# RobinBruneau/RNb-NeuS2

Hardware: AMD Instinct MI355X
Metric: training rays/s + ms/step, normals-only SDF 64x800^2 (higher is better)
Workload: dtype f16 storage / f32 accumulate

## Files before the change

include/rnb_neus2.h:

```cpp
#ifndef RNB_NEUS2_H
#define RNB_NEUS2_H

#include <stdint.h>

#ifdef __cplusplus
extern "C" {
#endif

#define RNB_ABI_VERSION 5

typedef enum rnb_status {
	RNB_OK = 0,
	RNB_ERR_INVALID = -1,
	RNB_ERR_DEVICE = -2,
	RNB_ERR_NOMEM = -3,
	RNB_ERR_NO_SAMPLES = -4
} rnb_status;

#define RNB_N_POS_DIMS 3
#define RNB_COORD_FLOATS 7
#define RNB_OUT_WIDTH 16
#define RNB_SDF_IN 32
#define RNB_SDF_HID 64
#define RNB_SDF_OUT 16
// ... 84 lines not shown
	RNB_BUF_DENSITY_BITFIELD = 8,
	RNB_BUF_DENSITY_MEAN = 9,
	RNB_BUF_RAY_INDICES = 10,
	RNB_BUF_RAYS = 11,
	RNB_BUF_NUMSTEPS = 12,
	RNB_BUF_COORDS = 13,
	RNB_BUF_MLP_OUT = 14,
	RNB_BUF_DLOSS_DOUT = 15,
	RNB_BUF_COORDS_COMPACTED = 16,
	RNB_BUF_LOSS = 17,
	RNB_BUF_EK_LOSS = 18,
	RNB_BUF_MASK_LOSS = 19,
	RNB_BUF_COUNTERS = 20,
	RNB_BUF_DENSITY_GRID_TMP = 21,
	RNB_BUF_GRID_SAMPLE_POS = 22,
	RNB_BUF_GRID_SAMPLE_IDX = 23,
	RNB_BUF_STEP_VECTOR = 24,
	RNB_BUF_GRID_SAMPLE_POS_EVAL = 25,
	RNB_BUF_GRID_SAMPLE_IDX_EVAL = 26,
	RNB_BUF_GRADS_FP16 = 27,
	RNB_BUF_COUNT
} rnb_buffer_id;
#define RNB_BUF_READONLY 0x100

typedef enum rnb_memcpy_kind { RNB_H2D = 0, RNB_D2H = 1, RNB_D2D = 2 } rnb_memcpy_kind;

const char* rnb_last_error(void);
uint32_t rnb_abi_version(void);
int rnb_default_config(rnb_config* cfg);
int rnb_create(const rnb_config* cfg, rnb_ctx** out);
int rnb_destroy(rnb_ctx* ctx);
int rnb_update_config(rnb_ctx* ctx, const rnb_config* cfg);

uint64_t rnb_n_params(const rnb_ctx* ctx);
int rnb_param_layout(const rnb_ctx* ctx, uint64_t offsets[5]);
int rnb_grid_tables(const rnb_ctx* ctx, uint32_t* offsets, uint32_t* resolution, float* scale);
int rnb_init_params(rnb_ctx* ctx, const float* sdf_mlp_weights_host);
int rnb_set_params(rnb_ctx* ctx, const float* params_host);
int rnb_buffer(rnb_ctx* ctx, int buffer_id, void** ptr, uint64_t* n_bytes);
int rnb_params_changed(rnb_ctx* ctx);
int rnb_bitfield_changed(rnb_ctx* ctx);
int rnb_device_malloc(rnb_ctx* ctx, uint64_t n_bytes, void** ptr);
int rnb_device_free(rnb_ctx* ctx, void* ptr);
int rnb_memcpy(rnb_ctx* ctx, void* dst, const void* src, uint64_t n_bytes, int kind);

int rnb_set_dataset(rnb_ctx* ctx, uint32_t n_views, const rnb_view* views,
                    const uint16_t* const* normals_host, const uint16_t* const* albedos_host);

int rnb_set_training_step(rnb_ctx* ctx, uint32_t step);
uint32_t rnb_valid_level(const rnb_ctx* ctx);
int rnb_update_density_grid(rnb_ctx* ctx, void* stream);
typedef int (*rnb_grid_exchange_fn)(void* user, void* grid_tmp, uint64_t n_elements, void* stream);
int rnb_set_grid_exchange(rnb_ctx* ctx, rnb_grid_exchange_fn fn, void* user);
int rnb_update_density_grid_begin(rnb_ctx* ctx, void* stream);
int rnb_update_density_grid_end(rnb_ctx* ctx, void* stream);
int rnb_update_density_bitfield(rnb_ctx* ctx, void* stream);
int rnb_density(rnb_ctx* ctx, void* stream, const float* xyz_dev, uint32_t n, uint16_t* out_dev, int use_inference_params);
int rnb_sdf(rnb_ctx* ctx, void* stream, const float* xyz_dev, uint32_t n, uint16_t* out_dev, int use_inference_params);
int rnb_forward_infer(rnb_ctx* ctx, void* stream, const float* coords_dev, uint32_t n, uint16_t* out_dev, int use_inference_params);
int rnb_sdf_lattice(rnb_ctx* ctx, void* stream, const uint32_t res[3], float lattice_min, float lattice_max, float* out, int inference);
int rnb_marching_cubes(rnb_ctx* ctx, void* stream, const float* density, const uint32_t res[3], const float aabb_min[3], const float aabb_max[3], float thresh,
                       float** verts, uint32_t** indices, uint32_t* n_verts, uint32_t* n_indices);
int rnb_generate_training_samples(rnb_ctx* ctx, void* stream, uint32_t n_rays, uint32_t n_rays_total, uint32_t max_samples);
int rnb_compute_loss(rnb_ctx* ctx, void* stream, uint32_t n_rays, uint32_t n_rays_total);
int rnb_forward_backward(rnb_ctx* ctx, void* stream);
int rnb_optimizer_step(rnb_ctx* ctx, void* stream);

int rnb_train_step(rnb_ctx* ctx, void* stream, rnb_step_stats* stats);
int rnb_train_step_begin(rnb_ctx* ctx, void* stream);
int rnb_train_step_end(rnb_ctx* ctx, void* stream, rnb_step_stats* stats);
int rnb_train_step_apply(rnb_ctx* ctx, void* stream);
int rnb_train_step_local(rnb_ctx* ctx, void* stream, uint64_t counters[4], double loss_sums[3]);
int rnb_train_step_finish(rnb_ctx* ctx, const uint64_t counters[4], const double loss_sums[3], rnb_step_stats* stats);
int rnb_profile_enable(rnb_ctx* ctx, int on);
int rnb_profile_count(const rnb_ctx* ctx);
int rnb_profile_get(const rnb_ctx* ctx, int idx, const char** name, double* total_ms, uint64_t* launches, double* units);
uint32_t rnb_training_step(const rnb_ctx* ctx);
uint32_t rnb_rays_per_batch(const rnb_ctx* ctx);
int rnb_set_optimizer_step(rnb_ctx* ctx, uint32_t step);
int rnb_set_controller(rnb_ctx* ctx, uint32_t training_step, uint32_t rays_per_batch,
                       uint32_t measured_batch_size_before_compaction, uint32_t n_rays_total);

typedef enum rnb_primitive { RNB_PRIM_PCG32 = 0, RNB_PRIM_MORTON = 1, RNB_PRIM_SRGB = 2, RNB_PRIM_RAY_BOX = 3, RNB_PRIM_MARCH = 4,
                             RNB_PRIM_ACTIVATION = 5, RNB_PRIM_WARP = 6, RNB_PRIM_LOSS = 7, RNB_PRIM_PIXEL = 8, RNB_PRIM_GRID = 9, RNB_PRIM_READ_RGBA = 10, RNB_PRIM_CAMERA_RAY = 11, RNB_PRIM_RAY_TARGETS = 12, RNB_PRIM_LOSS_SAMPLE = 13, RNB_PRIM_RAY_LOSS = 14, RNB_PRIM_ENCODE = 15, RNB_PRIM_MARCH_RAY = 16, RNB_PRIM_SDF_DENSITY = 17, RNB_PRIM_PREP_DUE = 18, RNB_PRIM_DW_SLICED = 19 } rnb_primitive;
int rnb_eval_primitives(rnb_ctx* ctx, int kind, const uint32_t* in_host, uint32_t n_items, uint32_t* out_host);

int rnb_gradient_parts(rnb_ctx* ctx, uint64_t ranges[3][2], uint32_t* n_parts);
int rnb_gradient_part_wait(rnb_ctx* ctx, uint32_t part, void* stream);
int rnb_train_step_apply_early(rnb_ctx* ctx, void* stream);

#define RNB_MAX_SHARD_PARTS 3
typedef struct rnb_shard_part { uint64_t lo, hi, own_lo, own_hi; } rnb_shard_part;
int rnb_shard_layout(rnb_ctx* ctx, rnb_shard_part parts[RNB_MAX_SHARD_PARTS], uint32_t* n_parts, uint64_t* capacity);
int rnb_train_step_apply_shard(rnb_ctx* ctx, uint32_t part, void* stream);
int rnb_train_step_apply_done(rnb_ctx* ctx, void* stream);

#ifdef __cplusplus
}
#endif
#endif
```

rnb-neus2_amd/_abi.py:

```python
import ctypes as C

ABI_VERSION = 5

OK, ERR_INVALID, ERR_DEVICE, ERR_NOMEM, ERR_NO_SAMPLES = 0, -1, -2, -3, -4

N_SDF_MLP_PARAMS = 3072
N_RGB_MLP_PARAMS = 8192
N_VARIANCE_PARAMS = 4
GRIDSIZE = 128
CASCADES = 8


class Config(C.Structure):
    _fields_ = [
        ("abi_version", C.c_uint32),
        ("n_levels", C.c_uint32),
        ("log2_hashmap_size", C.c_uint32),
        ("base_resolution", C.c_uint32),
        ("per_level_scale", C.c_float),
        ("valid_level_scale", C.c_float),
        ("base_valid_level_scale", C.c_float),
        ("base_training_step", C.c_uint32),
        ("sdf_bias", C.c_float),
        ("target_batch_size", C.c_uint32),
        ("initial_rays_per_batch", C.c_uint32),
        ("max_rays_per_batch", C.c_uint32),
        ("aabb_scale", C.c_uint32),
        ("seed", C.c_uint32),
        ("mask_loss_weight", C.c_float),
        ("ek_loss_weight", C.c_float),
        ("apply_L2", C.c_uint32),
        ("apply_rgbplus", C.c_uint32),
        ("apply_no_albedo", C.c_uint32),
        ("apply_light_opti", C.c_uint32),
        ("apply_supernormal", C.c_uint32),
        ("apply_relu", C.c_uint32),
        ("apply_bce", C.c_uint32),
        ("snap_to_pixel_centers", C.c_uint32),
        ("learning_rate", C.c_float),
        ("beta1", C.c_float),
        ("beta2", C.c_float),
        ("epsilon", C.c_float),
        ("l2_reg", C.c_float),
        ("ema_decay", C.c_float),
        ("lr_decay_start", C.c_uint32),
        ("lr_decay_interval", C.c_uint32),
        ("lr_decay_base", C.c_float),
        ("density_grid_decay", C.c_float),
        ("world_size", C.c_uint32),
        ("rank", C.c_uint32),
        ("only_sdf_training", C.c_uint32),
        ("overlap", C.c_uint32),
        ("accumulate", C.c_uint32),
        ("deterministic", C.c_uint32),
        ("reserved", C.c_uint32 * 4),
    ]


class View(C.Structure):
    _fields_ = [
        ("width", C.c_uint32),
        ("height", C.c_uint32),
        ("focal_length", C.c_float * 2),
        ("principal_point", C.c_float * 2),
        ("xform", C.c_float * 12),
    ]


class StepStats(C.Structure):
    _fields_ = [
        ("training_step", C.c_uint32),
        ("rays_per_batch", C.c_uint32),
        ("next_rays_per_batch", C.c_uint32),
        ("measured_batch_size", C.c_uint32),
        ("measured_batch_size_before_compaction", C.c_uint32),
        ("n_rays_kept", C.c_uint32),
        ("density_grid_updated", C.c_uint32),
        ("loss", C.c_float),
        ("ek_loss", C.c_float),
        ("mask_loss", C.c_float),
        ("prep_ms", C.c_float),
        ("step_ms", C.c_float),
    ]

    def as_dict(self):
        return {name: getattr(self, name) for name, _ in self._fields_}


BUF = dict(
    PARAMS_FP32=0, PARAMS_FP16=1, PARAMS_EMA=2, GRADS_FP32=3, ADAM_M=4, ADAM_V=5, ADAM_STEPS=6,
    DENSITY_GRID=7, DENSITY_BITFIELD=8, DENSITY_MEAN=9, RAY_INDICES=10, RAYS=11, NUMSTEPS=12,
    COORDS=13, MLP_OUT=14, DLOSS_DOUT=15, COORDS_COMPACTED=16, LOSS=17, EK_LOSS=18, MASK_LOSS=19,
    COUNTERS=20, DENSITY_GRID_TMP=21, GRID_SAMPLE_POS=22, GRID_SAMPLE_IDX=23, STEP_VECTOR=24, GRID_SAMPLE_POS_EVAL=25, GRID_SAMPLE_IDX_EVAL=26, GRADS_FP16=27,
)
BUF_DTYPE = dict(
    PARAMS_FP32="f4", PARAMS_FP16="f2", PARAMS_EMA="f2", GRADS_FP32="f4", ADAM_M="f4", ADAM_V="f4", ADAM_STEPS="u4",
    DENSITY_GRID="f4", DENSITY_BITFIELD="u1", DENSITY_MEAN="f4", RAY_INDICES="u4", RAYS="f4", NUMSTEPS="u4",
    COORDS="f4", MLP_OUT="f2", DLOSS_DOUT="f2", COORDS_COMPACTED="f4", LOSS="f4", EK_LOSS="f4", MASK_LOSS="f4",
    COUNTERS="u4", DENSITY_GRID_TMP="f4", GRID_SAMPLE_POS="f4", GRID_SAMPLE_IDX="u4", STEP_VECTOR="f8", GRID_SAMPLE_POS_EVAL="f4", GRID_SAMPLE_IDX_EVAL="u4", GRADS_FP16="f2",
)
ACCUM_FP32, ACCUM_HALF = 0, 1
BUF_READONLY = 0x100
GRID_EXCHANGE_FN = C.CFUNCTYPE(C.c_int, C.c_void_p, C.c_void_p, C.c_uint64, C.c_void_p)
PRIM = dict(PCG32=0, MORTON=1, SRGB=2, RAY_BOX=3, MARCH=4, ACTIVATION=5, WARP=6, LOSS=7, PIXEL=8, GRID=9, READ_RGBA=10, CAMERA_RAY=11, RAY_TARGETS=12, LOSS_SAMPLE=13, RAY_LOSS=14, ENCODE=15, MARCH_RAY=16, SDF_DENSITY=17, PREP_DUE=18, DW_SLICED=19)
PRIM_IN_WORDS, PRIM_OUT_WORDS = (6, 3, 1, 8, 9, 1, 9, 9, 9, 7, 32, 20, 35, 37, 16, 263, 10, 2, 1, 33028), (4, 4, 2, 3, 7, 3, 11, 5, 3, 3, 5, 9, 7, 28, 9, 16, 23, 1, 2, 16)
H2D, D2H, D2D = 0, 1, 2

_ctx = C.c_void_p
_stream = C.c_void_p
_u32, _u64, _i = C.c_uint32, C.c_uint64, C.c_int

PROTOTYPES = {
    "last_error": (C.c_char_p, []),
    "abi_version": (_u32, []),
    "default_config": (_i, [C.POINTER(Config)]),
    "create": (_i, [C.POINTER(Config), C.POINTER(_ctx)]),
    "destroy": (_i, [_ctx]),
    "update_config": (_i, [_ctx, C.POINTER(Config)]),
    "n_params": (_u64, [_ctx]),
    "param_layout": (_i, [_ctx, C.POINTER(_u64)]),
    "grid_tables": (_i, [_ctx, C.POINTER(_u32), C.POINTER(_u32), C.POINTER(C.c_float)]),
    "init_params": (_i, [_ctx, C.POINTER(C.c_float)]),
    "set_params": (_i, [_ctx, C.POINTER(C.c_float)]),
    "buffer": (_i, [_ctx, _i, C.POINTER(C.c_void_p), C.POINTER(_u64)]),
    "params_changed": (_i, [_ctx]),
    "bitfield_changed": (_i, [_ctx]),
    "memcpy": (_i, [_ctx, C.c_void_p, C.c_void_p, _u64, _i]),
    "device_malloc": (_i, [_ctx, _u64, C.POINTER(C.c_void_p)]),
    "device_free": (_i, [_ctx, C.c_void_p]),
    "set_dataset": (_i, [_ctx, _u32, C.POINTER(View), C.POINTER(C.c_void_p), C.POINTER(C.c_void_p)]),
    "set_training_step": (_i, [_ctx, _u32]),
    "valid_level": (_u32, [_ctx]),
    "update_density_grid": (_i, [_ctx, _stream]),
    "update_density_bitfield": (_i, [_ctx, _stream]),
    "update_density_grid_begin": (_i, [_ctx, _stream]),
    "update_density_grid_end": (_i, [_ctx, _stream]),
    "set_grid_exchange": (_i, [_ctx, C.c_void_p, C.c_void_p]),
    "density": (_i, [_ctx, _stream, C.c_void_p, _u32, C.c_void_p, _i]),
    "sdf": (_i, [_ctx, _stream, C.c_void_p, _u32, C.c_void_p, _i]),
    "forward_infer": (_i, [_ctx, _stream, C.c_void_p, _u32, C.c_void_p, _i]),
    "sdf_lattice": (_i, [_ctx, _stream, C.POINTER(_u32), C.c_float, C.c_float, C.c_void_p, _i]),
    "marching_cubes": (_i, [_ctx, _stream, C.c_void_p, C.POINTER(_u32), C.POINTER(C.c_float), C.POINTER(C.c_float), C.c_float,
                            C.POINTER(C.c_void_p), C.POINTER(C.c_void_p), C.POINTER(_u32), C.POINTER(_u32)]),
    "generate_training_samples": (_i, [_ctx, _stream, _u32, _u32, _u32]),
    "compute_loss": (_i, [_ctx, _stream, _u32, _u32]),
    "forward_backward": (_i, [_ctx, _stream]),
    "optimizer_step": (_i, [_ctx, _stream]),
    "train_step": (_i, [_ctx, _stream, C.POINTER(StepStats)]),
    "train_step_begin": (_i, [_ctx, _stream]),
    "train_step_end": (_i, [_ctx, _stream, C.POINTER(StepStats)]),
    "profile_enable": (_i, [_ctx, _i]),
    "profile_count": (_i, [_ctx]),
    "profile_get": (_i, [_ctx, _i, C.POINTER(C.c_char_p), C.POINTER(C.c_double), C.POINTER(_u64), C.POINTER(C.c_double)]),
    "train_step_apply": (_i, [_ctx, _stream]),
    "train_step_local": (_i, [_ctx, _stream, C.POINTER(_u64), C.POINTER(C.c_double)]),
    "train_step_finish": (_i, [_ctx, C.POINTER(_u64), C.POINTER(C.c_double), C.POINTER(StepStats)]),
    "training_step": (_u32, [_ctx]),
    "rays_per_batch": (_u32, [_ctx]),
    "set_controller": (_i, [_ctx, _u32, _u32, _u32, _u32]),
    "set_optimizer_step": (_i, [_ctx, _u32]),
    "eval_primitives": (_i, [_ctx, _i, C.c_void_p, _u32, C.c_void_p]),
    "gradient_parts": (_i, [_ctx, C.POINTER(_u64 * 2 * 3), C.POINTER(_u32)]),
    "gradient_part_wait": (_i, [_ctx, _u32, _stream]),
    "train_step_apply_early": (_i, [_ctx, _stream]),
    "shard_layout": (_i, [_ctx, C.POINTER(_u64 * 4 * 3), C.POINTER(_u32), C.POINTER(_u64)]),
    "train_step_apply_shard": (_i, [_ctx, _u32, _stream]),
    "train_step_apply_done": (_i, [_ctx, _stream]),
}


RENDER_ABI_VERSION = 1
RENDER_CHANNELS = 9


class RenderOptions(C.Structure):
    _fields_ = [
        ("abi_version", C.c_uint32),
        ("min_transmittance", C.c_float),
        ("near_distance", C.c_float),
        ("use_inference_params", C.c_uint32),
        ("use_occupancy", C.c_uint32),
        ("max_rays_in_flight", C.c_uint32),
        ("reserved", C.c_uint32 * 4),
    ]


class RenderStats(C.Structure):
    _fields_ = [
# ... 772 lines not shown
```

rnb-neus2_amd/api.py:

```python
import ctypes as C
import math
import os

import numpy as np

from . import _abi
from ._abi import Config, View, StepStats, BUF, BUF_DTYPE

__all__ = ["Context", "DeviceMesh", "Config", "View", "StepStats", "load_library", "default_config", "library_path",
           "load_sdf_init_weights", "RnbError", "BUF", "scaled_view", "RENDER_CHANNELS"]

RENDER_CHANNELS = _abi.RENDER_CHANNELS

_PKG_DIR = os.path.dirname(os.path.abspath(__file__))
_REPO_ROOT = os.path.dirname(_PKG_DIR)
_LIB_NAME = "librnb_neus2_hip.so"


class RnbError(RuntimeError):
    def __init__(self, code, message):
        super().__init__("rnb error %d: %s" % (code, message))
        self.code = code


# ... 224 lines not shown
        dt = np.dtype(BUF_DTYPE[name])
        total = nb // dt.itemsize
        if count is None:
            count = total - offset
        if offset + count > total:
            raise ValueError("%s: range [%d, %d) exceeds %d elements" % (name, offset, offset + count, total))
        out = np.empty(count, dtype=dt)
        if count:
            self._check(self.f.memcpy(self._h, out.ctypes.data_as(C.c_void_p), C.c_void_p(ptr + offset * dt.itemsize),
                                      count * dt.itemsize, _abi.D2H))
        return out

    def put(self, name, array, offset=0):
        ptr, nb = self.buffer(name)
        dt = np.dtype(BUF_DTYPE[name])
        a = np.ascontiguousarray(array, dtype=dt).ravel()
        if (offset + a.size) * dt.itemsize > nb:
            raise ValueError("%s: write of %d elements at %d exceeds buffer" % (name, a.size, offset))
        if a.size:
            self._check(self.f.memcpy(self._h, C.c_void_p(ptr + offset * dt.itemsize), a.ctypes.data_as(C.c_void_p),
                                      a.size * dt.itemsize, _abi.H2D))
            if name == "DENSITY_BITFIELD":
                self.bitfield_changed()
            elif name == "PARAMS_FP16":
                self.params_changed()

    def init_params(self, sdf_weights=None):
        w = load_sdf_init_weights() if sdf_weights is None else np.ascontiguousarray(sdf_weights, dtype=np.float32)
        self._check(self.f.init_params(self._h, w.ctypes.data_as(C.POINTER(C.c_float))))

    def set_params(self, params_fp32):
        p = np.ascontiguousarray(params_fp32, dtype=np.float32).ravel()
        if p.size != self.n_params:
            raise ValueError("expected %d params, got %d" % (self.n_params, p.size))
        self._check(self.f.set_params(self._h, p.ctypes.data_as(C.POINTER(C.c_float))))

    def set_dataset(self, views, normals, albedos):
        n = len(views)
        if n == 0 or len(normals) != n or len(albedos) != n:
            raise ValueError("views / normals / albedos must be non-empty and of equal length")
        arr = (View * n)()
        nptr = (C.c_void_p * n)()
        aptr = (C.c_void_p * n)()
        keep = []
        for i, v in enumerate(views):
            arr[i].width = int(v["width"])
            arr[i].height = int(v["height"])
            arr[i].focal_length[:] = [float(x) for x in v["focal_length"]]
            arr[i].principal_point[:] = [float(x) for x in v["principal_point"]]
            arr[i].xform[:] = [float(x) for x in np.asarray(v["xform"], dtype=np.float32).reshape(12)]
            nm = np.ascontiguousarray(normals[i], dtype=np.uint16)
            al = np.ascontiguousarray(albedos[i], dtype=np.uint16)
            if nm.size != arr[i].width * arr[i].height * 4 or al.size != nm.size:
                raise ValueError("view %d: image size does not match width*height*4" % i)
            keep += [nm, al]
            nptr[i] = nm.ctypes.data
            aptr[i] = al.ctypes.data
        self._check(self.f.set_dataset(self._h, n, arr, nptr, aptr))

    def set_training_step(self, step):
        self._check(self.f.set_training_step(self._h, int(step)))

    @property
    def valid_level(self):
        return int(self.f.valid_level(self._h))

    @property
    def training_step(self):
        return int(self.f.training_step(self._h))

    @property
    def rays_per_batch(self):
        return int(self.f.rays_per_batch(self._h))

    def set_controller(self, training_step, rays_per_batch, measured_before_compaction=0, n_rays_total=0):
        self._check(self.f.set_controller(self._h, int(training_step), int(rays_per_batch), int(measured_before_compaction), int(n_rays_total)))

    def eval_primitives(self, kind, items):
        k = _abi.PRIM[kind]
        a = np.ascontiguousarray(items, dtype=np.uint32).reshape(-1, _abi.PRIM_IN_WORDS[k])
        out = np.empty((a.shape[0], _abi.PRIM_OUT_WORDS[k]), dtype=np.uint32)
        self._check(self.f.eval_primitives(self._h, k, a.ctypes.data_as(C.c_void_p), a.shape[0], out.ctypes.data_as(C.c_void_p)))
        return out

    def training_state(self, last_stats=None):
        return dict(params=self.get("PARAMS_FP32").copy(), adam_m=self.get("ADAM_M").copy(), adam_v=self.get("ADAM_V").copy(), adam_steps=self.get("ADAM_STEPS").copy(),
                    ema=self.get("PARAMS_EMA").copy(), grid=self.get("DENSITY_GRID").copy(), step=self.training_step, rays=self.rays_per_batch,
                    before=int(last_stats.measured_batch_size_before_compaction) if last_stats is not None else 0)

    def load_training_state(self, state):
        self.set_params(state["params"])
        self.put("ADAM_M", state["adam_m"])
        self.put("ADAM_V", state["adam_v"])
        self.put("ADAM_STEPS", state["adam_steps"])
        self.put("PARAMS_EMA", state["ema"])
        self.set_optimizer_step(state["step"])
        self.put("DENSITY_GRID", state["grid"])
        self.update_density_bitfield()
        self.set_controller(state["step"], state["rays"], state["before"], 0)

    def set_optimizer_step(self, step):
        self._check(self.f.set_optimizer_step(self._h, int(step)))

    def gradient_parts(self):
        arr = (C.c_uint64 * 2 * 3)()
        n = C.c_uint32()
        self._check(self.f.gradient_parts(self._h, C.byref(arr), C.byref(n)))
        return [(int(arr[k][0]), int(arr[k][1])) for k in range(n.value)]

    def train_step_apply_early(self, stream_handle):
        self._check(self.f.train_step_apply_early(self._h, C.c_void_p(stream_handle)))

    def gradient_part_wait(self, part, stream_handle):
        self._check(self.f.gradient_part_wait(self._h, int(part), C.c_void_p(stream_handle)))

    def shard_layout(self):
        arr = (C.c_uint64 * 4 * 3)()
        n = C.c_uint32()
        cap = C.c_uint64()
        self._check(self.f.shard_layout(self._h, C.byref(arr), C.byref(n), C.byref(cap)))
        return [tuple(int(arr[k][j]) for j in range(4)) for k in range(n.value)], int(cap.value)

    def train_step_apply_shard(self, part, stream_handle=None):
        self._check(self.f.train_step_apply_shard(self._h, int(part), C.c_void_p(stream_handle)))

    def train_step_apply_done(self, stream_handle=None):
        self._check(self.f.train_step_apply_done(self._h, C.c_void_p(stream_handle)))

    def profile_enable(self, on=True):
        self._check(self.f.profile_enable(self._h, int(bool(on))))

    def profile(self):
        out = []
        for i in range(self.f.profile_count(self._h)):
            name, ms, n, units = C.c_char_p(), C.c_double(), C.c_uint64(), C.c_double()
            self._check(self.f.profile_get(self._h, i, C.byref(name), C.byref(ms), C.byref(n), C.byref(units)))
            out.append(dict(kernel=name.value.decode(), total_ms=ms.value, launches=n.value, units=units.value))
        return out

    def update_density_grid(self, stream=None):
        self._check(self.f.update_density_grid(self._h, _stream_handle(stream)))

    def update_density_grid_begin(self, stream=None):
        self._check(self.f.update_density_grid_begin(self._h, _stream_handle(stream)))

    def update_density_grid_end(self, stream=None):
        self._check(self.f.update_density_grid_end(self._h, _stream_handle(stream)))

    def set_grid_exchange(self, fn):
        if fn is None:
            self._grid_cb = None
            self._check(self.f.set_grid_exchange(self._h, None, None))
            return

        def trampoline(_user, ptr, n, stream):
            try:
                fn(ptr, int(n), stream)
                return 0
            except Exception:
                import traceback
                traceback.print_exc()
                return -1
        self._grid_cb = _abi.GRID_EXCHANGE_FN(trampoline)
        self._check(self.f.set_grid_exchange(self._h, C.cast(self._grid_cb, C.c_void_p), None))

    def update_density_bitfield(self, stream=None):
# ... 1012 lines not shown
```

rnb-neus2_amd/csrc/common.cuh:

```cuda
#pragma once
#include <hip/hip_runtime.h>
#include <stdint.h>
#include "../../include/rnb_neus2.h"

namespace rnb {

typedef _Float16 half_t;
typedef _Float16 h2 __attribute__((ext_vector_type(2)));
typedef _Float16 h4 __attribute__((ext_vector_type(4)));
typedef _Float16 h8 __attribute__((ext_vector_type(8)));
typedef float f4 __attribute__((ext_vector_type(4)));

constexpr uint32_t GRIDSIZE = RNB_GRIDSIZE;
constexpr uint32_t GRID_CELLS = GRIDSIZE * GRIDSIZE * GRIDSIZE;
constexpr uint32_t N_CASCADES = RNB_CASCADES;
constexpr float LOSS_SCALE = 128.f;
constexpr uint32_t N_MAX_RANDOM_SAMPLES_PER_RAY = 8;
constexpr float SQRT3 = 1.73205080757f;
constexpr float STEPSIZE = SQRT3 / 1024;
constexpr float MIN_CONE_STEPSIZE = STEPSIZE;
constexpr float MAX_CONE_STEPSIZE = STEPSIZE * (1 << (N_CASCADES - 1)) * 1024 / GRIDSIZE;
constexpr float MIN_OPTICAL_THICKNESS = 0.1f;

struct GridMeta {
// ... 213 lines not shown
__device__ __forceinline__ void encode_level_lm(const LevelMeta* __restrict__ lm, const uint32_t* __restrict__ grid, const uint32_t level,
                                                const float x, const float y, const float z,
                                                half_t& f0, half_t& f1, float dy0[3], float dy1[3]) {
	const uint4 raw = *reinterpret_cast<const uint4*>(lm + level);
	const uint32_t off = __builtin_amdgcn_readfirstlane(raw.x), size = __builtin_amdgcn_readfirstlane(raw.y), res = __builtin_amdgcn_readfirstlane(raw.z);
	const float scale = __uint_as_float(__builtin_amdgcn_readfirstlane(raw.w));
	encode_level_core<GRAD>(grid + off, size, res, scale, x, y, z, f0, f1, dy0, dy1);
}

__device__ __forceinline__ void level_issue(const LevelMeta* __restrict__ lm, const uint32_t* __restrict__ grid, const uint32_t level, const float x, const float y, const float z, uint32_t (&v)[8]) {
	const uint4 raw = reinterpret_cast<const uint4*>(lm + level)[0], raw2 = reinterpret_cast<const uint4*>(lm + level)[1];
	const uint32_t off = __builtin_amdgcn_readfirstlane(raw.x), hashmap_size = __builtin_amdgcn_readfirstlane(raw.y);
	const float scale = __uint_as_float(__builtin_amdgcn_readfirstlane(raw.w));
	const uint32_t my = __builtin_amdgcn_readfirstlane(raw2.x), mz = __builtin_amdgcn_readfirstlane(raw2.y);
	const bool dense = __builtin_amdgcn_readfirstlane(raw2.z) != 0u, pow2 = __builtin_amdgcn_readfirstlane(raw2.w) != 0u;
	const uint32_t* __restrict__ g = grid + off;
	float pos[3];
	uint32_t pg[3];
	pos_fract(x, scale, &pos[0], &pg[0]);
	pos_fract(y, scale, &pos[1], &pg[1]);
	pos_fract(z, scale, &pos[2], &pg[2]);
	const uint32_t ty0 = pg[1] * my, ty1 = ty0 + my, tz0 = pg[2] * mz, tz1 = tz0 + mz;
#pragma unroll
	for (uint32_t yz = 0; yz < 4; ++yz) {
		const uint32_t ty = (yz & 1u) ? ty1 : ty0, tz = (yz >> 1) ? tz1 : tz0;
		const uint32_t d0 = pg[0] + ty + tz, h = ty ^ tz;
		uint32_t e0 = dense ? d0 : (pg[0] ^ h), e1 = dense ? d0 + 1u : ((pg[0] + 1u) ^ h);
		const uint32_t w0 = e0 >= hashmap_size ? e0 - hashmap_size : e0, w1 = e1 >= hashmap_size ? e1 - hashmap_size : e1;
		e0 = pow2 ? (e0 & (hashmap_size - 1u)) : w0;
		e1 = pow2 ? (e1 & (hashmap_size - 1u)) : w1;
		v[yz * 2 + 0] = g[e0];
		v[yz * 2 + 1] = g[e1];
	}
}
template <bool GRAD>
__device__ __forceinline__ void level_consume(const LevelMeta* __restrict__ lm, const uint32_t level, const float x, const float y, const float z, const uint32_t (&v)[8],
                                              half_t& f0, half_t& f1, float dy0[3], float dy1[3]) {
	const float scale = __uint_as_float(__builtin_amdgcn_readfirstlane(reinterpret_cast<const uint32_t*>(lm + level)[3]));
	float pos[3];
	uint32_t pg[3];
	pos_fract(x, scale, &pos[0], &pg[0]);
	pos_fract(y, scale, &pos[1], &pg[1]);
	pos_fract(z, scale, &pos[2], &pg[2]);
	half_t r0 = (half_t)0.f, r1 = (half_t)0.f;
#pragma unroll
	for (uint32_t idx = 0; idx < 8; ++idx) {
		float weight = 1;
#pragma unroll
		for (uint32_t d = 0; d < 3; ++d) {
			if ((idx & (1u << d)) == 0) weight *= 1 - pos[d];
			else weight *= pos[d];
		}
		const h2 val = unpack_h2(v[idx]);
		r0 = r0 + f2h(weight * h2f(val[0]));
		r1 = r1 + f2h(weight * h2f(val[1]));
	}
	f0 = r0;
	f1 = r1;
	if (GRAD) {
#pragma unroll
		for (uint32_t gd = 0; gd < 3; ++gd) {
			float a0 = 0.f, a1 = 0.f;
#pragma unroll
			for (uint32_t idx = 0; idx < 4; ++idx) {
				float weight = scale;
				uint32_t corner = 0;
#pragma unroll
				for (uint32_t ngd = 0; ngd < 2; ++ngd) {
					const uint32_t d = ngd >= gd ? (ngd + 1) : ngd;
					if ((idx & (1u << ngd)) == 0) weight *= 1 - pos[d];
					else { weight *= pos[d]; corner |= (1u << d); }
				}
				const h2 vl = unpack_h2(v[corner]);
				const h2 vr = unpack_h2(v[corner | (1u << gd)]);
				a0 += weight * (h2f(vr[0]) - h2f(vl[0])) * 1.0f;
				a1 += weight * (h2f(vr[1]) - h2f(vl[1])) * 1.0f;
			}
			dy0[gd] = a0;
			dy1[gd] = a1;
		}
	}
}

struct Vec3 { float x, y, z; };
__device__ __forceinline__ Vec3 v3(float x, float y, float z) { return {x, y, z}; }
__device__ __forceinline__ Vec3 operator+(Vec3 a, Vec3 b) { return {a.x + b.x, a.y + b.y, a.z + b.z}; }
__device__ __forceinline__ Vec3 operator-(Vec3 a, Vec3 b) { return {a.x - b.x, a.y - b.y, a.z - b.z}; }
__device__ __forceinline__ Vec3 operator*(float s, Vec3 a) { return {s * a.x, s * a.y, s * a.z}; }
__device__ __forceinline__ float esum3(float x0, float x1, float x2) { return x0 + (x1 + x2); }
__device__ __forceinline__ float esum4(float x0, float x1, float x2, float x3) { return (x0 + x1) + (x2 + x3); }
__device__ __forceinline__ float dot(Vec3 a, Vec3 b) { return esum3(a.x * b.x, a.y * b.y, a.z * b.z); }
__device__ __forceinline__ Vec3 normalized(Vec3 a) { float n = sqrtf(dot(a, a)); return {a.x / n, a.y / n, a.z / n}; }

__device__ __forceinline__ int mip_from_pos(const Vec3& pos, uint32_t max_cascade = N_CASCADES - 1) {
	int exponent;
	float maxval = fmaxf(fmaxf(fabsf(pos.x - 0.5f), fabsf(pos.y - 0.5f)), fabsf(pos.z - 0.5f));
	frexpf(maxval, &exponent);
	return min((int)max_cascade, max(0, exponent + 1));
}
__device__ __forceinline__ int mip_from_dt(float dt, const Vec3& pos, uint32_t max_cascade = N_CASCADES - 1) {
	int mip = mip_from_pos(pos, max_cascade);
	dt *= 2 * GRIDSIZE;
	if (dt < 1.f) return mip;
	int exponent;
	frexpf(dt, &exponent);
	return min((int)max_cascade, max(exponent, mip));
}
__device__ __forceinline__ uint32_t cascaded_grid_idx_at(Vec3 pos, uint32_t mip) {
	float mip_scale = scalbnf(1.0f, -(int)mip);
	pos = pos - v3(0.5f, 0.5f, 0.5f);
	pos = mip_scale * pos;
	pos = pos + v3(0.5f, 0.5f, 0.5f);
	int ix = (int)(pos.x * GRIDSIZE), iy = (int)(pos.y * GRIDSIZE), iz = (int)(pos.z * GRIDSIZE);
	return morton3D((uint32_t)min(max(ix, 0), (int)GRIDSIZE - 1), (uint32_t)min(max(iy, 0), (int)GRIDSIZE - 1), (uint32_t)min(max(iz, 0), (int)GRIDSIZE - 1));
}
__device__ __forceinline__ bool density_grid_occupied_at(const Vec3& pos, const uint8_t* __restrict__ bitfield, uint32_t mip) {
	uint32_t idx = cascaded_grid_idx_at(pos, mip);
	return bitfield[idx / 8 + (GRID_CELLS * mip) / 8] & (1 << (idx % 8));
}
__device__ __forceinline__ float calc_dt(float t, float cone_angle) {
	return fminf(fmaxf(t * cone_angle, MIN_CONE_STEPSIZE), MAX_CONE_STEPSIZE);
}
__device__ __forceinline__ float warp_dt(float dt) {
	float max_stepsize = MIN_CONE_STEPSIZE * (1 << (N_CASCADES - 1));
	return (dt - MIN_CONE_STEPSIZE) / (max_stepsize - MIN_CONE_STEPSIZE);
}
__device__ __forceinline__ float unwarp_dt(float dt) {
	float max_stepsize = MIN_CONE_STEPSIZE * (1 << (N_CASCADES - 1));
	return dt * (max_stepsize - MIN_CONE_STEPSIZE) + MIN_CONE_STEPSIZE;
}
__device__ __forceinline__ float sign1(float x) { return copysignf(1.0f, x); }
__device__ __forceinline__ float distance_to_next_voxel(const Vec3& pos, const Vec3& dir, const Vec3& idir, uint32_t res) {
	Vec3 p = (float)res * pos;
	float tx = (floorf(p.x + 0.5f + 0.5f * sign1(dir.x)) - p.x) * idir.x;
	float ty = (floorf(p.y + 0.5f + 0.5f * sign1(dir.y)) - p.y) * idir.y;
	float tz = (floorf(p.z + 0.5f + 0.5f * sign1(dir.z)) - p.z) * idir.z;
	float t = fminf(fminf(tx, ty), tz);
	return fmaxf(t / res, 0.0f);
}
__device__ __forceinline__ float advance_to_next_voxel(float t, float cone_angle, const Vec3& pos, const Vec3& dir, const Vec3& idir, uint32_t res) {
	float t_target = t + distance_to_next_voxel(pos, dir, idir, res);
	do { t += calc_dt(t, cone_angle); } while (t < t_target);
	return t;
}

__device__ __forceinline__ float logistic(float x) { return 1.0f / (1.0f + expf(-x)); }
__device__ __forceinline__ float relu(float v) { return v > 0.0f ? v : 0.0f; }
__device__ __forceinline__ Vec3 warp_direction(const Vec3& d) { return {(d.x + 1.0f) * 0.5f, (d.y + 1.0f) * 0.5f, (d.z + 1.0f) * 0.5f}; }
__device__ __forceinline__ Vec3 unwarp_direction(const Vec3& d) { return {d.x * 2.0f - 1.0f, d.y * 2.0f - 1.0f, d.z * 2.0f - 1.0f}; }
__device__ __forceinline__ float loss_and_gradient(const bool l2, const float (&target)[4], const float (&prediction)[4], float (&grad)[4]) {
	float diff[4];
#pragma unroll
	for (int k = 0; k < 4; ++k) diff[k] = prediction[k] - target[k];
	if (l2) {
#pragma unroll
		for (int k = 0; k < 4; ++k) grad[k] = 2 * diff[k];
		return diff[0] * diff[0] + diff[1] * diff[1] + diff[2] * diff[2] + diff[3] * diff[3];
	}
#pragma unroll
	for (int k = 0; k < 4; ++k) grad[k] = copysignf(1.0f, diff[k]);
	return fabsf(diff[0]) + fabsf(diff[1]) + fabsf(diff[2]) + fabsf(diff[3]);
}

}
```

rnb-neus2_amd/csrc/kernels_net.cuh:

```cuda
#pragma once
#include "mlp.cuh"

namespace rnb {

constexpr int WG = 256;
constexpr int WAVES_PER_WG = 4;


__device__ __forceinline__ void write_sdf_in_row(half_t* __restrict__ tile, const int lane, const float x, const float y, const float z, const half_t (&feat)[28]) {
	half_t row[32];
	row[0] = f2h(x) - (half_t)0.5f;
	row[1] = f2h(y) - (half_t)0.5f;
	row[2] = f2h(z) - (half_t)0.5f;
#pragma unroll
	for (int k = 0; k < 28; ++k) row[3 + k] = feat[k];
	row[31] = (half_t)0.f;
#pragma unroll
	for (int q = 0; q < 4; ++q) {
		h8 v;
#pragma unroll
		for (int j = 0; j < 8; ++j) v[j] = row[q * 8 + j];
		*reinterpret_cast<h8*>(tile + lane * S32 + q * 8) = v;
	}
}

template <bool GRAD>
__device__ __forceinline__ void encode_all_lm(const LevelMeta* __restrict__ lm, const uint32_t n_levels, const uint32_t valid_level, const uint32_t* __restrict__ grid,
                                              const float x, const float y, const float z, half_t (&feat)[28], float (&dydx)[GRAD ? 28 : 1][3]) {
#pragma unroll
	for (uint32_t level = 0; level < 14; ++level) {
		half_t f0 = (half_t)0.f, f1 = (half_t)0.f;
		float d0[3] = {0.f, 0.f, 0.f}, d1[3] = {0.f, 0.f, 0.f};
		if (level < n_levels && level <= valid_level) {
			encode_level_lm<GRAD>(lm, grid, level, x, y, z, f0, f1, d0, d1);
		}
		feat[level * 2 + 0] = f0;
		feat[level * 2 + 1] = f1;
		if (GRAD) {
#pragma unroll
			for (int d = 0; d < 3; ++d) { dydx[GRAD ? level * 2 + 0 : 0][d] = d0[d]; dydx[GRAD ? level * 2 + 1 : 0][d] = d1[d]; }
		}
	}
}

template <bool GRAD, int DEPTH>
__device__ __forceinline__ void encode_all_pipelined(const LevelMeta* __restrict__ lm, const uint32_t n_levels, const uint32_t valid_level, const uint32_t* __restrict__ grid,
                                                     const float x, const float y, const float z, half_t (&feat)[28], float (&dydx)[GRAD ? 28 : 1][3]) {
	const uint32_t n_live = min(n_levels, valid_level + 1u);
	uint32_t v[DEPTH][8];
	const uint32_t last = n_live ? n_live - 1u : 0u;
#pragma unroll
	for (uint32_t l = 0; l < (uint32_t)DEPTH; ++l) level_issue(lm, grid, min(l, last), x, y, z, v[l]);
#pragma unroll
	for (uint32_t level = 0; level < 14; ++level) {
		half_t f0, f1;
		float d0[3], d1[3];
		const bool live = level < n_live;
		level_consume<GRAD>(lm, min(level, last), x, y, z, v[level % DEPTH], f0, f1, d0, d1);
		if (level + DEPTH < 14) level_issue(lm, grid, min(level + (uint32_t)DEPTH, last), x, y, z, v[level % DEPTH]);
		feat[level * 2 + 0] = live ? f0 : (half_t)0.f;
		feat[level * 2 + 1] = live ? f1 : (half_t)0.f;
		if (GRAD) {
#pragma unroll
			for (int d = 0; d < 3; ++d) { dydx[GRAD ? level * 2 + 0 : 0][d] = live ? d0[d] : 0.f; dydx[GRAD ? level * 2 + 1 : 0][d] = live ? d1[d] : 0.f; }
		}
	}
}

__device__ __forceinline__ half_t sdf_to_density(half_t sdf, half_t variance) {
	const half_t s = f2h(expf(h2f(variance * (half_t)10.0f)));
	const half_t sig = f2h(1.0f / (1.0f + expf(-h2f(sdf * s))));
	return (s * sig) * ((half_t)1.0f - sig);
}

struct PointArgs {
	const float* xyz;
	uint32_t n;
	half_t* out;
	const uint32_t* splat_idx;
	float* grid_tmp;
	int want_density;
	float sdf_bias;
	const uint32_t* range;
};

struct FwdArgs {
	const float* coords;
	const uint32_t* n_ptr;
	uint32_t n_max;
	half_t* out;
	float sdf_bias;
	const uint32_t* idx;
	const half_t* wimg;
	half_t* cin_out;
};

__device__ __forceinline__ void copy_weight_image(half_t* __restrict__ dst, const half_t* __restrict__ src, const int n_halfs, const int tid, const int nthreads) {
	for (int i = tid * 8; i < n_halfs; i += nthreads * 8) *reinterpret_cast<h8*>(dst + i) = *reinterpret_cast<const h8*>(src + i);
}

constexpr int PQ2_WAVE_HALFS = TILE * S32 + TILE;
constexpr size_t LDS_POINT2 = (size_t)(W_S0T + WAVES_PER_WG * PQ2_WAVE_HALFS) * sizeof(half_t);
__device__ __forceinline__ void poison_lds(char* smem_raw, const size_t bytes, const int tid, const int nthreads) {
#ifdef RNB_POISON_LDS
	uint32_t* w = reinterpret_cast<uint32_t*>(smem_raw);
	for (uint32_t q = (uint32_t)tid; q < (uint32_t)(bytes / 4); q += (uint32_t)nthreads) w[q] = 0x7e007e00u;
	__syncthreads();
#else
	(void)smem_raw; (void)bytes; (void)tid; (void)nthreads;
#endif
}

template <bool EMU, int DEPTH>
__device__ __forceinline__ void point_query_chained_body(const GridMeta& G, const NetW& net, const PointArgs& a, const half_t* __restrict__ wimg, char* smem_raw, LevelMeta* lm) {
	poison_lds(smem_raw, LDS_POINT2, threadIdx.x, WG);
	half_t* wts = reinterpret_cast<half_t*>(smem_raw);
	fill_level_meta(lm, G, threadIdx.x);
	const uint32_t n_levels = G.n_levels, valid_level = G.valid_level;
	if (wimg) copy_weight_image(wts, wimg, W_S0T, threadIdx.x, WG);
	else {
		for (int i = threadIdx.x; i < 64 * 32; i += WG) { int o = i >> 5, k = i & 31; wts[W_S0 + o * S32 + k] = net.sdf_w0[i]; }
		for (int i = threadIdx.x; i < 16 * 64; i += WG) { int o = i >> 6, q = i & 63; wts[W_S1 + o * S64 + q] = net.sdf_w1[o * 64 + chain_logical(q)]; }
	}
	__syncthreads();
	const int lane = threadIdx.x & 63, wave = threadIdx.x >> 6;
	half_t* X = wts + W_S0T + wave * PQ2_WAVE_HALFS;
	half_t* Z = X + TILE * S32;
	const half_t variance = net.variance[0];
	const half_t bias = f2h(a.sdf_bias);
	uint32_t s_first = 0, s_end = a.n;
	if (a.range) { s_first = a.range[0]; s_end = min(a.range[1], a.n); }
	const uint32_t n_tiles = (s_end - s_first + TILE - 1) / TILE;
	const int r16 = lane & 15, hq = lane >> 4;
	const bool by_xcd = (gridDim.x & 7u) == 0u;
	const uint32_t t8 = by_xcd ? (n_tiles + 7u) / 8u : n_tiles, t_base = by_xcd ? (blockIdx.x & 7u) * t8 : 0u, t_stop = min(n_tiles, t_base + t8);
	const uint32_t t_stride = (by_xcd ? gridDim.x / 8u : gridDim.x) * WAVES_PER_WG;
	for (uint32_t tile = t_base + (by_xcd ? blockIdx.x / 8u : blockIdx.x) * WAVES_PER_WG + wave; tile < t_stop; tile += t_stride) {
		const uint32_t s = s_first + tile * TILE + lane;
		const bool valid = s < s_end;
		float x = 0.5f, y = 0.5f, z = 0.5f;
		if (valid) { x = a.xyz[(size_t)s * 3 + 0]; y = a.xyz[(size_t)s * 3 + 1]; z = a.xyz[(size_t)s * 3 + 2]; }
		uint32_t cell = 0;
		if (valid && a.splat_idx) cell = a.splat_idx[s];
		half_t feat[28];
		float dummy[1][3];
		encode_all_pipelined<false, DEPTH>(lm, n_levels, valid_level, net.grid, x, y, z, feat, dummy);
		write_sdf_in_row(X, lane, x, y, z, feat);
		wave_lds_sync();
		h8 bz[4][2];
		{
			f4 acc[4][4];
			zero_acc<4>(acc);
			mfma_layer<4, 1, EMU ? EMU_NATURAL : EMU_OFF>(wts + W_S0, S32, X, S32, acc, lane);
			chain_pack<true>(acc, bz);
		}
		f4 acc_so[1][4];
		zero_acc<1>(acc_so);
		mfma_layer_regs<1, 2, EMU ? EMU_CHAINED : EMU_OFF>(wts + W_S1, S64, bz, acc_so, lane);
		if (hq == 0) {
#pragma unroll
			for (int nt = 0; nt < 4; ++nt) Z[16 * nt + r16] = f2h(acc_so[0][nt][0]);
		}
		wave_lds_sync();
		half_t v = Z[lane] + bias;
		if (a.want_density) v = sdf_to_density(v, variance);
		if (valid) {
			if (a.out) a.out[s] = v;
			if (a.splat_idx) atomicMax(reinterpret_cast<uint32_t*>(a.grid_tmp) + cell, __float_as_uint(h2f(v)));
		}
		wave_lds_sync();
	}
}
template <int DEPTH>
__global__ __launch_bounds__(WG, 3) void k_point_query_chained_pipe(const GridMeta G, const NetW net, const PointArgs a, const half_t* __restrict__ wimg) {
	extern __shared__ __attribute__((aligned(16))) char smem_raw[];
	__shared__ LevelMeta lm[RNB_MAX_LEVELS];
	point_query_chained_body<false, DEPTH>(G, net, a, wimg, smem_raw, lm);
}
template <int DEPTH>
__global__ __launch_bounds__(WG, 2) void k_point_query_chained_emul_pipe(const GridMeta G, const NetW net, const PointArgs a, const half_t* __restrict__ wimg) {
	extern __shared__ __attribute__((aligned(16))) char smem_raw[];
	__shared__ LevelMeta lm[RNB_MAX_LEVELS];
	point_query_chained_body<true, DEPTH>(G, net, a, wimg, smem_raw, lm);
}

constexpr int FWD2_WAVE_HALFS = TILE * S32 + TILE * 8 + TILE;
constexpr size_t LDS_FWD2 = (size_t)(W_FWD_END + WAVES_PER_WG * FWD2_WAVE_HALFS) * sizeof(half_t);

template <bool EMU, int DEPTH>
__device__ __forceinline__ void forward_chained_body(const GridMeta& G, const NetW& net, const FwdArgs& a, char* smem_raw, LevelMeta* lm) {
	poison_lds(smem_raw, LDS_FWD2, threadIdx.x, WG);
	half_t* wts = reinterpret_cast<half_t*>(smem_raw);
	fill_level_meta(lm, G, threadIdx.x);
	const uint32_t n_levels = G.n_levels, valid_level = G.valid_level;
	if (a.wimg) copy_weight_image(wts, a.wimg, W_FWD_END, threadIdx.x, WG);
	else load_weights_chained(wts, net, threadIdx.x, WG);
	__syncthreads();
	const int lane = threadIdx.x & 63, wave = threadIdx.x >> 6;
	half_t* X = wts + W_FWD_END + wave * FWD2_WAVE_HALFS;
	half_t* Y = X + TILE * S32;
	half_t* Z = Y + TILE * 8;
	const half_t variance = net.variance[0];
	const half_t bias = f2h(a.sdf_bias);
	uint32_t n = a.n_max;
	if (a.n_ptr) n = min(*a.n_ptr, a.n_max);
	const uint32_t n_tiles = (n + TILE - 1) / TILE;
	const int r16 = lane & 15, hq = lane >> 4;
	for (uint32_t tile = blockIdx.x * WAVES_PER_WG + wave; tile < n_tiles; tile += gridDim.x * WAVES_PER_WG) {
		const uint32_t q_in = tile * TILE + lane;
		const bool valid = q_in < n;
		uint32_t s = q_in;
		if (a.idx && valid) s = a.idx[q_in];
		float c[7] = {0.5f, 0.5f, 0.5f, 0.f, 0.f, 0.f, 0.f};
		if (valid) {
#pragma unroll
			for (int q = 0; q < 7; ++q) c[q] = a.coords[(size_t)s * 7 + q];
		}
		half_t feat[28];
		float dydx[28][3];
		encode_all_pipelined<true, DEPTH>(lm, n_levels, valid_level, net.grid, c[0], c[1], c[2], feat, dydx);
		write_sdf_in_row(X, lane, c[0], c[1], c[2], feat);
		wave_lds_sync();
		h8 bz[4][2];
		{
			f4 acc[4][4];
			zero_acc<4>(acc);
			mfma_layer<4, 1, EMU ? EMU_NATURAL : EMU_OFF>(wts + W_S0, S32, X, S32, acc, lane);
			chain_pack<true>(acc, bz);
		}
		f4 acc_so[1][4];
		zero_acc<1>(acc_so);
		mfma_layer_regs<1, 2, EMU ? EMU_CHAINED : EMU_OFF>(wts + W_S1, S64, bz, acc_so, lane);
		{
#pragma unroll
			for (int ks = 0; ks < 2; ++ks) {
				const h8 w1 = *reinterpret_cast<const h8*>(wts + W_S1 + 0 * S64 + 32 * ks + 8 * hq);
#pragma unroll
				for (int nt = 0; nt < 4; ++nt)
#pragma unroll
					for (int j = 0; j < 8; ++j) bz[nt][ks][j] = (bz[nt][ks][j] > (half_t)0.f) ? w1[j] : (half_t)0.f;
			}
		}
		wave_lds_sync();
		{
			f4 acc[2][4];
			zero_acc<2>(acc);
			mfma_layer_regs<2, 2, EMU ? EMU_CHAINED : EMU_OFF>(wts + W_S0T, S64, bz, acc, lane);
			store_acc<2, false>(acc, X, S32, 0, lane);
		}
		wave_lds_sync();
		float grad[3] = {0.f, 0.f, 0.f};
		{
			half_t din[32];
#pragma unroll
			for (int q = 0; q < 4; ++q) {
				const h8 v = *reinterpret_cast<const h8*>(X + lane * S32 + q * 8);
#pragma unroll
				for (int j = 0; j < 8; ++j) din[q * 8 + j] = v[j];
			}
#pragma unroll
			for (int k = 0; k < 28; ++k) {
				const float dl = h2f(din[3 + k]);
#pragma unroll
				for (int d = 0; d < 3; ++d) grad[d] += dl * dydx[k][d];
			}
#pragma unroll
			for (int d = 0; d < 3; ++d) grad[d] += h2f(din[d]);
		}
		{
			const h8 v = {f2h(c[0]), f2h(c[1]), f2h(c[2]), f2h(grad[0]), f2h(grad[1]), f2h(grad[2]), (half_t)0.f, (half_t)0.f};
			*reinterpret_cast<h8*>(Y + lane * 8) = v;
			if (hq == 0) {
#pragma unroll
				for (int nt = 0; nt < 4; ++nt) Z[16 * nt + r16] = f2h(acc_so[0][nt][0]);
			}
		}
		wave_lds_sync();
		const half_t sdf0 = Z[lane];
		if (a.cin_out) {
			if (valid) {
				h8* row = reinterpret_cast<h8*>(a.cin_out + (size_t)s * 32);
				row[2] = *reinterpret_cast<const h8*>(Y + lane * 8);
				row[3] = h8{(half_t)0.f, (half_t)0.f, (half_t)0.f, (half_t)0.f, (half_t)0.f, (half_t)0.f, (half_t)0.f, (half_t)0.f};
			}
#pragma unroll
			for (int nt = 0; nt < 4; ++nt) {
				const uint32_t s_nt = (uint32_t)__shfl((int)s, 16 * nt + r16, 64);
				const bool v_nt = __shfl((int)valid, 16 * nt + r16, 64) != 0;
				const h4 o = {f2h(acc_so[0][nt][0]), f2h(acc_so[0][nt][1]), f2h(acc_so[0][nt][2]), f2h(acc_so[0][nt][3])};
				if (v_nt) *reinterpret_cast<h4*>(a.cin_out + (size_t)s_nt * 32 + 4 * hq) = o;
			}
		}
		h8 bh[4][2];
		{
			h8 bin[4][1];
#pragma unroll
			for (int nt = 0; nt < 4; ++nt) {
				h4 o = {(half_t)0.f, (half_t)0.f, (half_t)0.f, (half_t)0.f};
				if (hq < 2) o = *reinterpret_cast<const h4*>(Y + (16 * nt + r16) * 8 + 4 * hq);
#pragma unroll
				for (int j = 0; j < 4; ++j) { bin[nt][0][j] = f2h(acc_so[0][nt][j]); bin[nt][0][4 + j] = o[j]; }
			}
			f4 acc[4][4];
			zero_acc<4>(acc);
			mfma_layer_regs<4, 1, EMU ? EMU_CHAINED : EMU_OFF>(wts + W_C0, S32, bin, acc, lane);
			chain_pack<true>(acc, bh);
		}
		{
			f4 acc[4][4];
			zero_acc<4>(acc);
			mfma_layer_regs<4, 2, EMU ? EMU_CHAINED : EMU_OFF>(wts + W_C1, S64, bh, acc, lane);
			chain_pack<true>(acc, bh);
		}
		{
			f4 acc[1][4];
			zero_acc<1>(acc);
			mfma_layer_regs<1, 2, EMU ? EMU_CHAINED : EMU_OFF>(wts + W_C2, S64, bh, acc, lane);
			store_acc<1, false>(acc, X, S32, 0, lane);
		}
		wave_lds_sync();
		{
			h8 o0 = *reinterpret_cast<const h8*>(X + lane * S32 + 0);
			h8 o1 = *reinterpret_cast<const h8*>(X + lane * S32 + 8);
			o0[3] = sdf0 + bias;
			o0[4] = f2h(grad[0]); o0[5] = f2h(grad[1]); o0[6] = f2h(grad[2]);
			o0[7] = variance;
			o1[0] = f2h(c[4]); o1[1] = f2h(c[5]); o1[2] = f2h(c[6]);
			if (valid) {
				h8* dst = reinterpret_cast<h8*>(a.out + (size_t)s * 16);
				dst[0] = o0;
				dst[1] = o1;
			}
		}
		wave_lds_sync();
	}
}
template <int DEPTH>
__global__ __launch_bounds__(WG, 2) void k_forward_chained_pipe(const GridMeta G, const NetW net, const FwdArgs a) {
	extern __shared__ __attribute__((aligned(16))) char smem_raw[];
	__shared__ LevelMeta lm[RNB_MAX_LEVELS];
	forward_chained_body<false, DEPTH>(G, net, a, smem_raw, lm);
}
template <int DEPTH>
__global__ __launch_bounds__(WG, 2) void k_forward_chained_emul_pipe(const GridMeta G, const NetW net, const FwdArgs a) {
	extern __shared__ __attribute__((aligned(16))) char smem_raw[];
	__shared__ LevelMeta lm[RNB_MAX_LEVELS];
	forward_chained_body<true, DEPTH>(G, net, a, smem_raw, lm);
}


struct TrainScratch {
	half_t *h2, *h1, *cin, *z1, *sdfin, *dz1;
	half_t *dr, *dh2, *dh1, *dso, *dz, *ddin, *front;
	uint32_t* g12;
	float* srec;
	float* var_partial;
};

struct TrainArgs {
	const float* coords;
	const half_t* dout;
	uint32_t B;
	uint32_t B_global;
	float sdf_bias;
	uint32_t skip_rgb;
	const half_t* wimg;
	float *dw_w0, *dw_w0b, *dw_w1, *dw_w1b;
	const half_t* dcin;
	TrainScratch t;
};

__device__ __forceinline__ void fm_store(const half_t* __restrict__ tile, const int stride, const int width, half_t* __restrict__ dst, const uint32_t B, const uint32_t s) {
	const half_t* row = tile + (s & 63) * stride;
	for (int f = 0; f < width; f += 8) {
		const h8 v = *reinterpret_cast<const h8*>(row + f);
#pragma unroll
		for (int j = 0; j < 8; ++j) dst[(size_t)(f + j) * B + s] = v[j];
	}
}

__global__ __launch_bounds__(WG, 1) void k_fwd_bwd(const GridMeta G, const NetW net, const TrainArgs a) {
	extern __shared__ __attribute__((aligned(16))) char smem_raw[];
	half_t* wts = reinterpret_cast<half_t*>(smem_raw);
	__shared__ LevelMeta lm[RNB_MAX_LEVELS];
	fill_level_meta(lm, G, threadIdx.x);
	const uint32_t n_levels = G.n_levels, valid_level = G.valid_level;
	if (a.wimg) copy_weight_image(wts, a.wimg, W_TRAIN_END, threadIdx.x, WG);
	else load_weights<true>(wts, net, threadIdx.x, WG);
	__syncthreads();
	const int lane = threadIdx.x & 63, wave = threadIdx.x >> 6;
	half_t* tA = wts + W_TRAIN_END + wave * 3 * ACT_TILE_HALFS;
	half_t* tB = tA + ACT_TILE_HALFS;
	half_t* tC = tB + ACT_TILE_HALFS;
	const int r16 = lane & 15, hq = lane >> 4;
	const uint32_t B = a.B;
	const uint32_t n_tiles = B / TILE;
	const TrainScratch& T = a.t;
	float var_sum = 0.f;
	for (uint32_t tile = blockIdx.x * WAVES_PER_WG + wave; tile < n_tiles; tile += gridDim.x * WAVES_PER_WG) {
		const uint32_t s = tile * TILE + lane;
		float c[7];
#pragma unroll
		for (int q = 0; q < 7; ++q) c[q] = a.coords[(size_t)s * 7 + q];
		half_t dout[16];
		{
			const h8* src = reinterpret_cast<const h8*>(a.dout + (size_t)s * 16);
			const h8 d0 = src[0], d1 = src[1];
#pragma unroll
			for (int j = 0; j < 8; ++j) { dout[j] = d0[j]; dout[8 + j] = d1[j]; }
		}
		half_t feat[28];
		float dydx[28][3];
		encode_all_lm<true>(lm, n_levels, valid_level, net.grid, c[0], c[1], c[2], feat, dydx);
		write_sdf_in_row(tA, lane, c[0], c[1], c[2], feat);
		wave_lds_sync();
		fm_store(tA, S32, 32, T.sdfin, B, s);
		uint64_t m_z1;
		{
			f4 acc[4][4];
			zero_acc<4>(acc);
			mfma_layer<4, 1>(wts + W_S0, S32, tA, S32, acc, lane);
			m_z1 = store_acc<4, true>(acc, tB, S64, 0, lane);
		}
		wave_lds_sync();
		fm_store(tB, S64, 64, T.z1, B, s);
		{
			f4 acc[1][4];
			zero_acc<1>(acc);
			mfma_layer<1, 2>(wts + W_S1, S64, tB, S64, acc, lane);
			store_acc<1, false>(acc, tC, S32, 0, lane);
// ... 174 lines not shown
			}
			dd[31] = (half_t)0.f;
#pragma unroll
			for (int q = 0; q < 4; ++q) {
				h8 v;
#pragma unroll
				for (int j = 0; j < 8; ++j) v[j] = dd[q * 8 + j];
				*reinterpret_cast<h8*>(tC + lane * S32 + q * 8) = v;
			}
		}
		wave_lds_sync();
		fm_store(tC, S32, 32, T.ddin, B, s);
		{
			f4 acc[4][4];
			zero_acc<4>(acc);
			mfma_layer<4, 1>(wts + W_S0, S32, tC, S32, acc, lane);
			wave_lds_sync();
			store_acc_masked<4>(acc, m_z1, tB, S64, 0, lane);
		}
		wave_lds_sync();
		fm_store(tB, S64, 64, T.front, B, s);
		wave_lds_sync();
		(void)m_h2;
	}
#pragma unroll
	for (int off = 32; off > 0; off >>= 1) var_sum += __shfl_down(var_sum, off, 64);
	if (lane == 0) T.var_partial[blockIdx.x * WAVES_PER_WG + wave] = var_sum;
}

constexpr int SW_S0 = 0;
constexpr int SW_S0T = SW_S0 + 64 * S32;
constexpr int SW_W1 = SW_S0T + 32 * S64;
constexpr int SW_W1N = SW_W1 + 64;
constexpr int SW_END = SW_W1N + 64;
constexpr int SW_END_PADDED = (SW_END + 7) / 8 * 8;
constexpr int FBS_WAVE_HALFS = 2 * TILE * S32 + TILE;
constexpr size_t LDS_FBS = (size_t)(SW_END + WAVES_PER_WG * FBS_WAVE_HALFS) * sizeof(half_t);
constexpr int SW_W1T = SW_END_PADDED;
constexpr int SWF_END = SW_W1T + 64 * S32;
constexpr int SO_STRIDE = 24;
constexpr int FBS_FULL_WAVE_HALFS = FBS_WAVE_HALFS + TILE * SO_STRIDE;
constexpr size_t LDS_FBS_FULL = (size_t)(SWF_END + WAVES_PER_WG * FBS_FULL_WAVE_HALFS) * sizeof(half_t);
__host__ __device__ constexpr int fbs_logical(int p) { return p < 28 ? 3 + p : (p < 31 ? p - 28 : 31); }
__host__ __device__ constexpr int fbs_logical_h(int p) { return p < 13 ? 3 + p : (p < 16 ? p - 13 : p); }
__host__ __device__ constexpr int fbs_feature_slot_h(int q) { return q < 13 ? q : q + 3; }

__device__ inline void load_weights_fbs(half_t* __restrict__ w, const NetW& net, const int tid, const int nthreads, const bool half_order = false) {
	for (int i = tid; i < 64 * 32; i += nthreads) { const int o = i >> 5, p = i & 31; w[SW_S0 + o * S32 + p] = net.sdf_w0[o * 32 + (half_order ? fbs_logical_h(p) : fbs_logical(p))]; }
	for (int i = tid; i < 32 * 64; i += nthreads) { const int q = i >> 6, p = i & 63; w[SW_S0T + q * S64 + p] = net.sdf_w0[chain_logical(p) * 32 + fbs_logical(q)]; }
	for (int i = tid; i < 64; i += nthreads) { w[SW_W1 + i] = net.sdf_w1[chain_logical(i)]; w[SW_W1N + i] = net.sdf_w1[i]; }
	for (int i = SW_END + tid; i < SW_END_PADDED; i += nthreads) w[i] = (half_t)0.f;
}
__device__ inline void load_weights_fbs_full(half_t* __restrict__ w, const NetW& net, const int tid, const int nthreads, const bool half_order = false) {
	load_weights_fbs(w, net, tid, nthreads, half_order);
	for (int i = tid; i < 64 * 32; i += nthreads) { const int u = i >> 5, o = i & 31; w[SW_W1T + u * S32 + o] = o < 16 ? net.sdf_w1[o * 64 + u] : (half_t)0.f; }
}

__device__ inline void load_weights_rgb(half_t* __restrict__ w, const NetW& net, const int tid, const int nthreads);
constexpr uint32_t WIMG_WGS = 16;
__global__ __launch_bounds__(WG) void k_prepare_weight_images(const NetW net, half_t* __restrict__ img_fwd, half_t* __restrict__ img_fbs, half_t* __restrict__ img_train, half_t* __restrict__ img_rgb, const int half_order) {
	const int tid = blockIdx.x * WG + threadIdx.x, nthreads = gridDim.x * WG;
	if (blockIdx.y == 0) load_weights_chained(img_fwd, net, tid, nthreads);
	else if (blockIdx.y == 1) load_weights_fbs_full(img_fbs, net, tid, nthreads, half_order != 0);
	else if (blockIdx.y == 2) load_weights<true>(img_train, net, tid, nthreads);
	else load_weights_rgb(img_rgb, net, tid, nthreads);
}

template <typename T>
__device__ __forceinline__ void st32(T* __restrict__ base, const uint32_t idx, const T v) { *reinterpret_cast<T*>(reinterpret_cast<char*>(base) + idx * (uint32_t)sizeof(T)) = v; }

__device__ __forceinline__ void export_frags(const h8 (&b)[4][2], half_t* __restrict__ dst, const uint32_t B, const uint32_t tile, const int lane) {
	const uint32_t r16 = lane & 15, hq = lane >> 4;
	const uint32_t lane_off = 4u * hq * B + tile * TILE + r16 * 4u;
#pragma unroll
	for (uint32_t ks = 0; ks < 2; ++ks)
#pragma unroll
		for (uint32_t j = 0; j < 8; ++j) {
			const uint32_t row_off = (16u * (2u * ks + (j >> 2)) + (j & 3u)) * B;
			const h4 v = {b[0][ks][j], b[1][ks][j], b[2][ks][j], b[3][ks][j]};
			*reinterpret_cast<h4*>(reinterpret_cast<char*>(dst) + (row_off + lane_off) * 2u) = v;
		}
}

template <bool FULL, bool EMU = false, bool SLICED = false>
__device__ __forceinline__ void fwd_bwd_sdf_body(const GridMeta& G, const NetW& net, const TrainArgs& a, char* smem_raw, LevelMeta* lm) {
	poison_lds(smem_raw, FULL ? LDS_FBS_FULL : LDS_FBS, threadIdx.x, WG);
	half_t* wts = reinterpret_cast<half_t*>(smem_raw);
	constexpr int W_END = FULL ? SWF_END : SW_END;
	fill_level_meta(lm, G, threadIdx.x);
	const uint32_t n_live = min(G.n_levels, G.valid_level + 1u);
	if (a.wimg) copy_weight_image(wts, a.wimg, W_END, threadIdx.x, WG);
	else if (FULL) load_weights_fbs_full(wts, net, threadIdx.x, WG, EMU);
	else load_weights_fbs(wts, net, threadIdx.x, WG, EMU);
	__syncthreads();
	const int lane = threadIdx.x & 63, wave = threadIdx.x >> 6;
	constexpr int WAVE_HALFS = FULL ? FBS_FULL_WAVE_HALFS : FBS_WAVE_HALFS;
	half_t* X = wts + W_END + wave * WAVE_HALFS;
	half_t* D = X + TILE * S32;
	half_t* Z = D + TILE * S32;
	half_t* SO = Z + TILE;
	const int r16 = lane & 15, hq = lane >> 4;
	const uint32_t B = a.B;
	const uint32_t n_tiles = B / TILE;
	const TrainScratch& T = a.t;
	float var_sum = 0.f;
	f4 acc_w0[4][2], acc_w0b[4][2];
	float acc_w1[4] = {0.f, 0.f, 0.f, 0.f}, acc_w1b[4] = {0.f, 0.f, 0.f, 0.f};
	f4 acc_w1f[FULL ? 4 : 1];
#pragma unroll
	for (int nt = 0; nt < (FULL ? 4 : 1); ++nt) acc_w1f[nt] = f4{0.f, 0.f, 0.f, 0.f};
#pragma unroll
	for (int mo = 0; mo < 4; ++mo)
#pragma unroll
		for (int ni = 0; ni < 2; ++ni) { acc_w0[mo][ni] = f4{0.f, 0.f, 0.f, 0.f}; acc_w0b[mo][ni] = f4{0.f, 0.f, 0.f, 0.f}; }
	for (uint32_t tile = blockIdx.x * WAVES_PER_WG + wave; tile < n_tiles; tile += gridDim.x * WAVES_PER_WG) {
		const uint32_t s = tile * TILE + lane;
		float c[3];
#pragma unroll
		for (int q = 0; q < 3; ++q) c[q] = a.coords[(size_t)s * 7 + q];
		half_t dout[16];
		{
			const h8* src = reinterpret_cast<const h8*>(a.dout + (size_t)s * 16);
			const h8 d0 = src[0], d1 = src[1];
#pragma unroll
			for (int j = 0; j < 8; ++j) { dout[j] = d0[j]; dout[8 + j] = d1[j]; }
		}
		float dn[3];
		{
			h8 a2 = {(half_t)0.f, (half_t)0.f, (half_t)0.f, (half_t)0.f, (half_t)0.f, (half_t)0.f, (half_t)0.f, (half_t)0.f};
			if (FULL) {
				const h8* row = reinterpret_cast<const h8*>(a.dcin + (size_t)s * 32);
				a2 = row[2];
				h8 o0 = row[0];
				o0[0] = o0[0] + dout[3];
				*reinterpret_cast<h8*>(SO + lane * SO_STRIDE) = o0;
				*reinterpret_cast<h8*>(SO + lane * SO_STRIDE + 8) = row[1];
			}
#pragma unroll
			for (int d = 0; d < 3; ++d) {
				float v = FULL ? h2f(a2[3 + d]) : 0.f;
				v += h2f(dout[4 + d]) / (float)a.B_global;
				v += h2f(dout[8 + d]);
				dn[d] = v;
			}
		}
		reinterpret_cast<f4*>(T.srec)[(size_t)s * 2 + 0] = f4{c[0], c[1], c[2], dn[0]};
		reinterpret_cast<f4*>(T.srec)[(size_t)s * 2 + 1] = f4{dn[1], dn[2], 0.f, 0.f};
		uint32_t* Xrow = reinterpret_cast<uint32_t*>(X + lane * S32);
		uint32_t* Drow = reinterpret_cast<uint32_t*>(D + lane * S32);
#pragma unroll 1
		for (uint32_t level = 0; level < 14; ++level) {
			half_t f0 = (half_t)0.f, f1 = (half_t)0.f;
			float d0[3] = {0.f, 0.f, 0.f}, d1[3] = {0.f, 0.f, 0.f};
			if (level < n_live) encode_level_lm<true>(lm, net.grid, level, c[0], c[1], c[2], f0, f1, d0, d1);
			float r0 = 0.f, r1 = 0.f;
#pragma unroll
			for (int d = 0; d < 3; ++d) { r0 += d0[d] * dn[d]; r1 += d1[d] * dn[d]; }
			const half_t e0 = f2h(r0), e1 = f2h(r1);
			if (EMU) {
				const uint32_t q0 = 2u * level, q1 = q0 + 1u, p0 = q0 < 13u ? q0 : q0 + 3u, p1 = q1 < 13u ? q1 : q1 + 3u;
				X[lane * S32 + p0] = f0; X[lane * S32 + p1] = f1;
				D[lane * S32 + p0] = e0; D[lane * S32 + p1] = e1;
			} else {
				Xrow[level] = pack_h2(f0, f1);
				Drow[level] = pack_h2(e0, e1);
			}
		}
		{
			const half_t px = f2h(c[0]) - (half_t)0.5f, py = f2h(c[1]) - (half_t)0.5f, pz = f2h(c[2]) - (half_t)0.5f;
			const half_t n0 = f2h(dn[0]), n1 = f2h(dn[1]), n2 = f2h(dn[2]);
			if (EMU) {
				half_t* xr = X + lane * S32; half_t* dr = D + lane * S32;
				xr[13] = px; xr[14] = py; xr[15] = pz; xr[31] = (half_t)0.f;
				dr[13] = n0; dr[14] = n1; dr[15] = n2; dr[31] = (half_t)0.f;
			} else {
				Xrow[14] = pack_h2(px, py); Xrow[15] = pack_h2(pz, (half_t)0.f);
				Drow[14] = pack_h2(n0, n1); Drow[15] = pack_h2(n2, (half_t)0.f);
			}
		}
		Z[lane] = dout[3];
		var_sum += h2f(dout[7]);
		wave_lds_sync();
		auto load_fso = [&](const int nt) {
			h8 v = {(half_t)0.f, (half_t)0.f, (half_t)0.f, (half_t)0.f, (half_t)0.f, (half_t)0.f, (half_t)0.f, (half_t)0.f};
			if (hq < 2) v = *reinterpret_cast<const h8*>(SO + (16 * nt + r16) * SO_STRIDE + 8 * hq);
			return v;
		};
		if (SLICED) {
			static_assert(!SLICED || EMU, "the sliced weight gradients belong to the half mode");
			if (!FULL) st32(T.dso, s, dout[3]);
		}
		{
			h8 fso[4];
			if (FULL) {
#pragma unroll
				for (int nt = 0; nt < 4; ++nt) fso[nt] = load_fso(nt);
			}
			h8 ain[4], add[4];
			h4 d3v[4];
#pragma unroll
			for (int mt = 0; mt < 4; ++mt) {
				ain[mt] = *reinterpret_cast<const h8*>(X + (16 * mt + r16) * S32 + 8 * hq);
				add[mt] = *reinterpret_cast<const h8*>(D + (16 * mt + r16) * S32 + 8 * hq);
				d3v[mt] = *reinterpret_cast<const h4*>(Z + 16 * mt + 4 * hq);
			}
			const f4 zero4 = {0.f, 0.f, 0.f, 0.f};
			h8 a_so[2];
			if (FULL) {
				h8 idf;
#pragma unroll
				for (int j = 0; j < 8; ++j) idf[j] = (8 * hq + j == r16) ? (half_t)1.f : (half_t)0.f;
#pragma unroll
				for (int ks = 0; ks < 2; ++ks)
#pragma unroll
					for (int h = 0; h < 2; ++h) {
						const f4 t = __builtin_amdgcn_mfma_f32_16x16x32_f16(fso[2 * ks + h], idf, zero4, 0, 0, 0);
#pragma unroll
						for (int r = 0; r < 4; ++r) a_so[ks][4 * h + r] = f2h(t[r]);
					}
				if (SLICED) {
#pragma unroll
					for (int ks = 0; ks < 2; ++ks)
#pragma unroll
						for (int h = 0; h < 2; ++h) {
							const uint32_t off = (uint32_t)r16 * B + tile * TILE + 16u * (2 * ks + h) + 4u * hq;
							st32(reinterpret_cast<h4*>(T.dso), off / 4u, h4{a_so[ks][4 * h], a_so[ks][4 * h + 1], a_so[ks][4 * h + 2], a_so[ks][4 * h + 3]});
						}
				}
			}
			h8 b_in[2][2], b_dd[2][2];
#pragma unroll
			for (int n2 = 0; n2 < 2; ++n2) {
				h8 idf;
#pragma unroll
				for (int j = 0; j < 8; ++j) idf[j] = (8 * hq + j == 16 * n2 + r16) ? (half_t)1.f : (half_t)0.f;
#pragma unroll
				for (int ks = 0; ks < 2; ++ks)
// ... 149 lines not shown
		{
			f4 acc[2][4];
			zero_acc<2>(acc);
			mfma_layer_regs<2, 2, EMU ? EMU_CHAINED : EMU_OFF>(wts + SW_S0T, S64, bdz, acc, lane);
			store_acc<2, false>(acc, X, S32, 0, lane);
		}
		wave_lds_sync();
#pragma unroll
		for (uint32_t l = 0; l < 14; ++l) st32(T.g12, (l * B + s) * 2u + 0u, Xrow[l]);
		wave_lds_sync();
	}
#pragma unroll
	for (int off = 32; off > 0; off >>= 1) var_sum += __shfl_down(var_sum, off, 64);
	if (lane == 0) T.var_partial[blockIdx.x * WAVES_PER_WG + wave] = var_sum;
	if (SLICED) return;
	float* red = reinterpret_cast<float*>(wts + W_END);
	static_assert((size_t)WAVES_PER_WG * FBS_WAVE_HALFS * sizeof(half_t) >= (size_t)WAVES_PER_WG * 64 * 32 * sizeof(float), "staging area of the weight-gradient partials");
	constexpr int N = 64 * 32;
	for (int pass = 0; pass < 2; ++pass) {
		__syncthreads();
#pragma unroll
		for (int mo = 0; mo < 4; ++mo)
#pragma unroll
			for (int ni = 0; ni < 2; ++ni)
#pragma unroll
				for (int r = 0; r < 4; ++r) red[wave * N + (16 * mo + 4 * hq + r) * 32 + (EMU ? fbs_logical_h(16 * ni + r16) : fbs_logical(16 * ni + r16))] = pass ? acc_w0b[mo][ni][r] : acc_w0[mo][ni][r];
		__syncthreads();
		float* dst = (pass ? a.dw_w0b : a.dw_w0) + (size_t)blockIdx.x * N;
		for (int q = threadIdx.x; q < N; q += WG) dst[q] = ((red[q] + red[N + q]) + red[2 * N + q]) + red[3 * N + q];
	}
	if (FULL) {
		__syncthreads();
#pragma unroll
		for (int nt = 0; nt < 4; ++nt)
#pragma unroll
			for (int r = 0; r < 4; ++r) red[wave * (16 * 64) + (4 * hq + r) * 64 + 16 * nt + r16] = acc_w1f[nt][r];
		__syncthreads();
		float* dst = a.dw_w1 + (size_t)blockIdx.x * (16 * 64);
		for (int q = threadIdx.x; q < 16 * 64; q += WG) dst[q] = ((red[q] + red[16 * 64 + q]) + red[2 * 16 * 64 + q]) + red[3 * 16 * 64 + q];
	}
	for (int pass = FULL ? 1 : 0; pass < 2; ++pass) {
		__syncthreads();
#pragma unroll
		for (int nt = 0; nt < 4; ++nt) red[(wave * 4 + hq) * 64 + 16 * nt + r16] = pass ? acc_w1b[nt] : acc_w1[nt];
		__syncthreads();
		float* dst = (pass ? a.dw_w1b : a.dw_w1) + (size_t)blockIdx.x * (16 * 64);
		for (int q = threadIdx.x; q < 16 * 64; q += WG) {
			float v = 0.f;
			if (q < 64) for (int g = 0; g < 16; ++g) v += red[g * 64 + q];
			dst[q] = v;
		}
	}
}

__global__ __launch_bounds__(WG, 2) void k_fwd_bwd_sdf(const GridMeta G, const NetW net, const TrainArgs a) {
	extern __shared__ __attribute__((aligned(16))) char smem_raw[];
	__shared__ LevelMeta lm[RNB_MAX_LEVELS];
	fwd_bwd_sdf_body<false>(G, net, a, smem_raw, lm);
}
__global__ __launch_bounds__(WG, 2) void k_fwd_bwd_sdf_full(const GridMeta G, const NetW net, const TrainArgs a) {
	extern __shared__ __attribute__((aligned(16))) char smem_raw[];
	__shared__ LevelMeta lm[RNB_MAX_LEVELS];
	fwd_bwd_sdf_body<true>(G, net, a, smem_raw, lm);
}
__global__ __launch_bounds__(WG, 2) void k_fwd_bwd_sdf_h(const GridMeta G, const NetW net, const TrainArgs a) {
	extern __shared__ __attribute__((aligned(16))) char smem_raw[];
	__shared__ LevelMeta lm[RNB_MAX_LEVELS];
	fwd_bwd_sdf_body<false, true>(G, net, a, smem_raw, lm);
}
__global__ __launch_bounds__(WG, 2) void k_fwd_bwd_sdf_hs(const GridMeta G, const NetW net, const TrainArgs a) {
	extern __shared__ __attribute__((aligned(16))) char smem_raw[];
	__shared__ LevelMeta lm[RNB_MAX_LEVELS];
	fwd_bwd_sdf_body<false, true, true>(G, net, a, smem_raw, lm);
}
__global__ __launch_bounds__(WG, 2) void k_fwd_bwd_sdf_full_hs(const GridMeta G, const NetW net, const TrainArgs a) {
	extern __shared__ __attribute__((aligned(16))) char smem_raw[];
	__shared__ LevelMeta lm[RNB_MAX_LEVELS];
	fwd_bwd_sdf_body<true, true, true>(G, net, a, smem_raw, lm);
}
__global__ __launch_bounds__(WG, 2) void k_fwd_bwd_sdf_full_h(const GridMeta G, const NetW net, const TrainArgs a) {
	extern __shared__ __attribute__((aligned(16))) char smem_raw[];
	__shared__ LevelMeta lm[RNB_MAX_LEVELS];
	fwd_bwd_sdf_body<true, true>(G, net, a, smem_raw, lm);
}

constexpr int RW_C0 = 0;
constexpr int RW_C1 = RW_C0 + 64 * S32;
constexpr int RW_C1T = RW_C1 + 64 * S64;
constexpr int RW_C0T = RW_C1T + 64 * S64;
constexpr int RW_C2T = RW_C0T + 32 * S64;
constexpr int RW_END = RW_C2T + 64 * S32;
static_assert(RW_END % 8 == 0, "16-byte copies of the image");
constexpr size_t LDS_RGB = std::max((size_t)RW_END * sizeof(half_t), (size_t)WAVES_PER_WG * 64 * 64 * sizeof(float));

__device__ inline void load_weights_rgb(half_t* __restrict__ w, const NetW& net, const int tid, const int nthreads) {
	auto col = [](int c) { return c < 16 ? c : c + 16; };
	for (int i = tid; i < 64 * 32; i += nthreads) {
		const int o = i >> 5, c = i & 31;
		w[RW_C0 + o * S32 + c] = net.rgb_w0[o * 48 + col(c)];
		w[RW_C2T + o * S32 + c] = c < 16 ? net.rgb_w2[c * 64 + o] : (half_t)0.f;
	}
	for (int i = tid; i < 64 * 64; i += nthreads) {
		const int o = i >> 6, p = i & 63;
		w[RW_C1 + o * S64 + p] = net.rgb_w1[o * 64 + chain_logical(p)];
		w[RW_C1T + o * S64 + p] = net.rgb_w1[chain_logical(p) * 64 + o];
	}
	for (int i = tid; i < 32 * 64; i += nthreads) { const int c = i >> 6, p = i & 63; w[RW_C0T + c * S64 + p] = net.rgb_w0[chain_logical(p) * 48 + col(c)]; }
}

struct RgbArgs {
	const half_t* cin;
	const uint32_t* src_slot;
	const half_t* dout;
	half_t* dcin;
	uint32_t B;
	const half_t* wimg;
	float *dw_c0, *dw_c1, *dw_c2;
	TrainScratch t;
};

template <int KS>
__device__ __forceinline__ void transpose_frags(const h8 (&in)[4][KS], h8 (&out)[2 * KS][2], const int r16, const int hq) {
	const f4 zero4 = {0.f, 0.f, 0.f, 0.f};
#pragma unroll
	for (int n2 = 0; n2 < 2; ++n2) {
		h8 idf;
#pragma unroll
		for (int j = 0; j < 8; ++j) idf[j] = (8 * hq + j == 16 * n2 + r16) ? (half_t)1.f : (half_t)0.f;
#pragma unroll
		for (int ks = 0; ks < KS; ++ks)
#pragma unroll
			for (int ms = 0; ms < 4; ++ms) {
				const f4 t = __builtin_amdgcn_mfma_f32_16x16x32_f16(in[ms][ks], idf, zero4, 0, 0, 0);
#pragma unroll
				for (int r = 0; r < 4; r += 2) {
					out[2 * ks + n2][ms >> 1][4 * (ms & 1) + r] = f2h(t[r]);
					out[2 * ks + n2][ms >> 1][4 * (ms & 1) + r + 1] = f2h(t[r + 1]);
				}
			}
	}
}

template <int NQ>
__device__ __forceinline__ void export_transposed(const h8 (&t)[NQ][2], const int n_q, half_t* __restrict__ dst, const uint32_t B, const uint32_t tile, const int r16, const int hq, const bool chained) {
#pragma unroll
	for (int q = 0; q < NQ; ++q) {
		if (q >= n_q) break;
		const uint32_t row = chained ? (uint32_t)chain_logical(16 * q + r16) : (uint32_t)(16 * q + r16);
#pragma unroll
		for (int ks = 0; ks < 2; ++ks)
#pragma unroll
			for (int h = 0; h < 2; ++h) {
				const uint32_t off = row * B + tile * TILE + 16u * (2 * ks + h) + 4u * hq;
				st32(reinterpret_cast<h4*>(dst), off / 4u, h4{t[q][ks][4 * h], t[q][ks][4 * h + 1], t[q][ks][4 * h + 2], t[q][ks][4 * h + 3]});
			}
	}
}

template <bool EMU, bool SLICED = false>
__device__ __forceinline__ void rgb_fwd_bwd_body(const NetW& net, const RgbArgs& a, char* smem_raw) {
	half_t* wts = reinterpret_cast<half_t*>(smem_raw);
	if (a.wimg) copy_weight_image(wts, a.wimg, RW_END, threadIdx.x, WG);
	else load_weights_rgb(wts, net, threadIdx.x, WG);
	__syncthreads();
	const int lane = threadIdx.x & 63, wave = threadIdx.x >> 6;
	const int r16 = lane & 15, hq = lane >> 4;
// ... 1163 lines not shown
```

rnb-neus2_amd/csrc/rnb_neus2_hip.hip:

```cpp
#include "kernels_net.cuh"
#include "kernels_ray.cuh"
#include "kernels_mesh.cuh"
#include "kernels_render.cuh"
#include "kernels_mesh_sparse.cuh"
#include "kernels_mesh_clean.cuh"
#include "kernels_mesh_simplify.cuh"
#include "kernels_mesh_distance.cuh"
#include "kernels_mesh_raster.cuh"
#include "kernels_mesh_texture.cuh"
#include "kernels_mesh_visibility.cuh"
#include "kernels_mesh_project.cuh"
#include "kernels_mesh_draw.cuh"
#include "kernels_mesh_topology.cuh"
#include "kernels_mesh_holes.cuh"
#include "../host/mesh.hpp"

#include <hip/hip_ext.h>

#include <algorithm>
#include <atomic>
#include <chrono>
#include <cmath>
#include <cstdio>
#include <cstdlib>
// ... 111 lines not shown
	int n_cus = 256;

	DevBuf<float> params_fp32, grads, adam_m, adam_v;
	DevBuf<half_t> params_fp16, params_ema;
	DevBuf<half_t> grads16;
	bool half_acc() const { return cfg.accumulate == RNB_ACCUM_HALF; }
	DevBuf<unsigned long long> grads_fixed;
	bool fixed_acc() const { return cfg.deterministic != 0; }
	size_t grad_elem() const { return half_acc() ? sizeof(half_t) : sizeof(float); }
	char* grad_ptr(uint64_t i) const { return half_acc() ? reinterpret_cast<char*>(grads16.p + i) : reinterpret_cast<char*>(grads.p + i); }
	DevBuf<uint32_t> adam_steps;
	DevBuf<float> opt_rec;
	bool opt_plain_current = true, opt_rec_current = false;
	DevBuf<float> adam_lr_table;
	float lr_table_beta1 = -1.f, lr_table_beta2 = -1.f;
	DevBuf<float> density_grid, density_grid_tmp, density_grid_tmp_alt, density_mean;
	bool tmp_alt_clear = false;
	rnb_grid_exchange_fn grid_exchange = nullptr;
	void* grid_exchange_user = nullptr;
	bool bitfield_foreign = false;
	DevBuf<double> mean_partial, loss_sums;
	DevBuf<uint8_t> bitfield;
	DevBuf<unsigned long long> march_stats;
	DevBuf<uint32_t> coarse_bits, coarse_count;
	bool coarse_valid = false;
	uint32_t* host_coarse = nullptr;
	uint32_t* host_coarse_dev = nullptr;
	DevBuf<float> grid_sample_pos;
	DevBuf<uint32_t> grid_sample_idx;
	uint32_t n_grid_samples = 0;
	struct { bool valid = false; uint32_t ema_step = 0, n_uniform = 0, n_nonuniform = 0; uint64_t rng_state = 0, rng_inc = 0; } gs_pre;
	bool last_update_sorted = false;
	struct { bool pending = false; uint32_t n_uniform = 0, n_nonuniform = 0; } gs_todo;
	DevBuf<float> gs_sorted_pos, gs_stage_pos, gs_eval_pos;
	DevBuf<uint32_t> gs_sorted_idx, gs_stage_idx, gs_eval_idx, gs_hist, gs_range;
	hipEvent_t ev_grid = nullptr, ev_gs = nullptr;

	uint32_t n_views = 0;
	DevBuf<ViewDev> views;
	DevBuf<uint16_t> pixels;
	float light_dirs[9];

	DevBuf<uint32_t> ray_indices, numsteps, counters;
	DevBuf<float> rays, coords, coords_compacted, loss;
	float *ek_loss = nullptr, *mask_loss = nullptr;
	DevBuf<half_t> mlp_out, dloss_dout;
	DevBuf<double> wg_partial;
	bool loss_reduced = false;
	DevBuf<float> ray_grad; DevBuf<uint32_t> ray_of, slot_of;
	DevBuf<float> chain_rec;
	DevBuf<float> ray_setup, ray_dunnorm, ray_t;
	DevBuf<double> loss_partial;
	DevBuf<uint32_t> ray_steps, ray_base, ray_slot, ncomp, cbase;
	DevBuf<uint32_t> ray_base1, idx1, idx2, fwd_counts;
	DevBuf<unsigned long long> scan_words;
	uint32_t scan_ticket = 0;
	DevBuf<half_t> wimg_fwd, wimg_fbs, wimg_train, wimg_rgb;
	DevBuf<half_t> cin_eval, dcin, rgb_out_scratch;
	DevBuf<uint32_t> src_slot;
	bool cin_flow = false;
	bool rgb_split() const { return !cfg.apply_no_albedo && !knobs.fwd_bwd_generic; }
	bool wimg_valid = false;
	DevBuf<float> ray_const;
	DevBuf<uint32_t> unfinished;
	uint32_t fwd_k1 = 48;
	bool fwd_k1_fixed = false;
	bool gen_split = false;
	uint32_t gen_k1 = 0, cur_k1 = 0;
	struct Knobs {
		bool march_narrow = false, fwd_bwd_generic = false, loss_wave_per_ray = false;
		uint32_t march_narrow_from = 18432;
		bool dp_order = false;
		bool loss_scan_fused_always = false;
		bool loss_scan_fused = true;
		bool loss_flat = true;
		bool loss_chain_records = true;
		bool scatter_plain = false;
		int march_skip = 1;
		bool march_skip_narrow = false;
		int march_bbox = 1;
		bool dw_sliced = true;
		bool grid_presort = true;
	} knobs;
	DevBuf<RayLoss> ray_loss;
	DevBuf<McTable> mc_table;
	RenderWorkspace render;
	DevBuf<half_t> fm;
	DevBuf<uint32_t> g12;
	DevBuf<float> srec, var_partial, dw_partial;
	TrainScratch ts;
	uint32_t dw_nwg = 0, dw_chunk = 0;
	uint32_t fwd_grid = 0;
	bool grads_clean = true;

	Pcg32 rng, density_grid_rng, trainer_rng;
	uint32_t density_grid_ema_step = 0;
	uint32_t training_step = 0, valid_level = 0, rays_per_batch = 0;
	uint32_t measured_batch_size = 0, measured_batch_size_before_compaction = 0, n_rays_total = 0;
	uint32_t optimizer_step_count = 0;
	float lr_factor = 1.f;
	uint32_t cur_n_rays = 0, cur_n_rays_total = 0, local_measured_before = 0, cur_step = 0;
	bool grid_updated = false;
	float prep_ms = 0.f;
	std::chrono::steady_clock::time_point step_start;

	hipStream_t s_march = nullptr, s_dw = nullptr, s_adam = nullptr;
	bool tail_pending = false;
	hipEvent_t ev_loss = nullptr, ev_march = nullptr, ev_fb = nullptr, ev_dw = nullptr, ev_adam = nullptr, ev_tail = nullptr, ev_march_rest = nullptr, ev_all = nullptr, ev_sc[3] = {nullptr, nullptr, nullptr};
	struct { bool valid = false, exchanged = false, dp = false, sharded = false, all_final_recorded = false, dw_joined = true; uint64_t split[2] = {0, 0}, split_mid = 0; int order = 0; } sc;
	struct ScatterGroups { uint32_t e_c = 0, l_fine = 0, Ks[RNB_MAX_LEVELS] = {}; uint64_t k_log2 = 0; } sg;
	hipStream_t backward_stream = nullptr;
	hipStream_t step_stream = nullptr;
	uint64_t dp_split = 0, dp_mid = 0;
	uint64_t param_capacity = 0;
	bool dp_order() const { return cfg.world_size > 1 || knobs.dp_order; }
	struct { bool begun = false, early_done = false; AdamArgs args; } opt;
	struct { bool valid = false, loss_cleared = false; uint32_t n_rays = 0, n_rays_total = 0, max_inference = 0, k1 = 0; bool split = false; } pre;
	struct Readback { double sums[3]; uint32_t counters[4]; uint32_t fwd[2]; uint32_t seq, pad; }* host_rb = nullptr;
	uint32_t rb_seq = 0;
	bool loss_polled = true;
	bool poll_loss() const { return overlap() && !dp_order(); }
	void* host_rb_dev = nullptr;
	bool overlap() const { return cfg.overlap != 0 && !prof.on && s_march != nullptr; }

	NetW net(bool inference) const {
		const half_t* p = inference ? params_ema.p : params_fp16.p;
		NetW n;
		n.sdf_w0 = p + off_sdf;
		n.sdf_w1 = n.sdf_w0 + 64 * 32;
		n.rgb_w0 = p + off_rgb;
		n.rgb_w1 = n.rgb_w0 + 64 * 48;
		n.rgb_w2 = n.rgb_w1 + 64 * 64;
		n.grid = reinterpret_cast<const uint32_t*>(p + off_grid);
		n.variance = p + off_var;
		return n;
	}
	GridMeta meta() const { GridMeta g = grid; g.valid_level = valid_level; return g; }
};

static void discard_premarch(rnb_ctx* c);
static bool prep_due(uint32_t step) {
	const uint32_t n_prep_to_skip = std::min(std::max(step / 16u, 1u), 16u);
	return step % n_prep_to_skip == 0;
}
static void join_tail_host(rnb_ctx* c) {
	if (c->tail_pending) { (void)hipEventSynchronize(c->ev_tail); c->tail_pending = false; }
}

static int check_scan_errors(rnb_ctx* c) {
	const bool rays = c->host_coarse[5] != 0, compact = c->host_coarse[6] != 0;
	if (!rays && !compact) return RNB_OK;
	c->host_coarse[5] = 0; c->host_coarse[6] = 0;
	g_err = std::string(rays ? "k_scan_rays_chain" : "k_scan_compact_chain") + ": a tile's sums did not arrive (workgroup not scheduled); the launch reported zero counters";
	return RNB_ERR_DEVICE;
}

namespace {

constexpr size_t LDS_TRAIN = (size_t)(W_TRAIN_END + WAVES_PER_WG * 3 * ACT_TILE_HALFS) * sizeof(half_t);
static_assert(LDS_TRAIN <= 160 * 1024, "training kernel LDS exceeds 160 KiB");

void build_grid_tables(rnb_ctx* c) {
	const rnb_config& cfg = c->cfg;
	std::memset(&c->grid, 0, sizeof(c->grid));
	c->grid.n_levels = cfg.n_levels;
	uint32_t offset = 0;
// ... 25 lines not shown
	if (c->cfg.apply_supernormal) {
		for (int r = 0; r < 3; ++r) for (int k = 0; k < 3; ++k) c->light_dirs[r * 3 + k] = (r == k) ? 1.f : 0.f;
	}
}

int derive_half_params(rnb_ctx* c, hipStream_t s) {
	hipLaunchKernelGGL(k_fp32_to_half, dim3(2048), dim3(256), 0, s, c->params_fp32.p, c->params_fp16.p, c->n_params);
	HIP_TRY(hipGetLastError());
	return RNB_OK;
}

static int ensure_opt_records(rnb_ctx* c) {
	if (c->opt_rec_current) return RNB_OK;
	HIP_TRY(hipDeviceSynchronize());
	hipLaunchKernelGGL(k_opt_records_pack, dim3(4096), dim3(256), 0, 0, c->param_capacity / 4, c->params_fp32.p, c->adam_m.p, c->adam_v.p, c->adam_steps.p, c->opt_rec.p);
	HIP_TRY(hipGetLastError());
	HIP_TRY(hipDeviceSynchronize());
	c->opt_rec_current = true;
	return RNB_OK;
}
static int ensure_opt_views(rnb_ctx* c) {
	if (c->opt_plain_current) return RNB_OK;
	HIP_TRY(hipDeviceSynchronize());
	hipLaunchKernelGGL(k_opt_records_unpack, dim3(4096), dim3(256), 0, 0, c->param_capacity / 4, c->opt_rec.p, c->params_fp32.p, c->adam_m.p, c->adam_v.p, c->adam_steps.p);
	HIP_TRY(hipGetLastError());
	HIP_TRY(hipDeviceSynchronize());
	c->opt_plain_current = true;
	return RNB_OK;
}

int reset_optimizer_state(rnb_ctx* c) {
	HIP_TRY(hipMemset(c->adam_m.p, 0, c->adam_m.bytes()));
	HIP_TRY(hipMemset(c->adam_v.p, 0, c->adam_v.bytes()));
	HIP_TRY(hipMemset(c->adam_steps.p, 0, c->adam_steps.bytes()));
	HIP_TRY(hipMemset(c->grad_ptr(0), 0, c->param_capacity * c->grad_elem()));
	c->grads_clean = true;
	c->optimizer_step_count = 0;
	c->opt_plain_current = true; c->opt_rec_current = false;
	return RNB_OK;
}

static int rebuild_coarse(rnb_ctx* c, hipStream_t s, bool wait = true) {
	LAUNCH_EV(k_coarse_bitfield, dim3(1), dim3(1024), 0, s, (c->overlap() && !wait) ? c->ev_grid : nullptr, c->bitfield.p, c->coarse_bits.p, c->coarse_count.p, c->host_coarse_dev);
	HIP_TRY(hipGetLastError());
	c->coarse_valid = true;
	if (wait || *c->host_coarse == 0xffffffffu) HIP_TRY(hipStreamSynchronize(s));
	return RNB_OK;
}

int update_bitfield(rnb_ctx* c, hipStream_t s, bool wait = true, bool have_partials = false) {
	const uint32_t n_blocks = 1024;
	if (!have_partials) hipLaunchKernelGGL(k_mean_partial, dim3(n_blocks), dim3(256), 0, s, c->density_grid.p, c->mean_partial.p);
	const uint32_t n_bytes_per_mip = GRID_CELLS / 8;
	if (c->aabb.max_cascade == 0 && !c->bitfield_foreign) {
		hipLaunchKernelGGL(k_bitfield_sc, dim3(n_bytes_per_mip / 256), dim3(256), 0, s, c->density_grid.p, c->bitfield.p, c->mean_partial.p, c->density_mean.p);
		LAUNCH_EV(k_pool_tail_coarse, dim3(2), dim3(1024), 0, s, (c->overlap() && !wait) ? c->ev_grid : nullptr, 2u, c->bitfield.p, c->coarse_bits.p, c->coarse_count.p, c->host_coarse_dev);
		HIP_TRY(hipGetLastError());
		c->coarse_valid = true;
		if (wait || *c->host_coarse == 0xffffffffu) HIP_TRY(hipStreamSynchronize(s));
		return RNB_OK;
	}
	hipLaunchKernelGGL(k_mean_final, dim3(1), dim3(64), 0, s, c->mean_partial.p, n_blocks, c->density_mean.p);
	const uint32_t n_el = n_bytes_per_mip * N_CASCADES;
	hipLaunchKernelGGL(k_grid_to_bitfield, dim3((n_el + 127) / 128), dim3(128), 0, s, n_el, n_bytes_per_mip * (c->aabb.max_cascade + 1), c->density_grid.p, c->bitfield.p, c->density_mean.p);
	const uint32_t first_tail = std::min<uint32_t>(c->aabb.max_cascade + 2, N_CASCADES);
	for (uint32_t level = 1; level < first_tail; ++level) {
		hipLaunchKernelGGL(k_bitfield_max_pool, dim3((GRID_CELLS / 64 + 127) / 128), dim3(128), 0, s, GRID_CELLS / 64,
		                   c->bitfield.p + (size_t)n_bytes_per_mip * (level - 1), c->bitfield.p + (size_t)n_bytes_per_mip * level);
	}
	if (first_tail < N_CASCADES) hipLaunchKernelGGL(k_bitfield_max_pool_tail, dim3(1), dim3(1024), 0, s, first_tail, c->bitfield.p);
	HIP_TRY(hipGetLastError());
	c->bitfield_foreign = false;
	return rebuild_coarse(c, s, wait);
}

int launch_point_query(rnb_ctx* c, hipStream_t s, const float* xyz, uint32_t n, half_t* out, const uint32_t* splat_idx, float* grid_tmp, int want_density, bool inference, const uint32_t* range = nullptr) {
	if (n == 0) return RNB_OK;
	join_tail_host(c);
	PointArgs a;
	a.xyz = xyz; a.n = n; a.out = out; a.splat_idx = splat_idx; a.grid_tmp = grid_tmp; a.want_density = want_density; a.sdf_bias = c->cfg.sdf_bias; a.range = range;
	const uint32_t n_tiles = (n + TILE - 1) / TILE;
	const uint32_t grid = std::min<uint32_t>((n_tiles + WAVES_PER_WG - 1) / WAVES_PER_WG, (uint32_t)c->n_cus * 5);
	const half_t* wimg = (!inference && c->wimg_valid) ? c->wimg_fwd.p : nullptr;
	if (c->half_acc()) hipLaunchKernelGGL(k_point_query_chained_emul_pipe<4>, dim3(grid), dim3(WG), LDS_POINT2, s, c->meta(), c->net(inference), a, wimg);
	else hipLaunchKernelGGL(k_point_query_chained_pipe<4>, dim3(grid), dim3(WG), LDS_POINT2, s, c->meta(), c->net(inference), a, wimg);
	HIP_TRY(hipGetLastError());
	return RNB_OK;
}

static int launch_grid_samples(rnb_ctx* c, hipStream_t s, Pcg32& rng, uint32_t ema_step, uint32_t n_uniform, uint32_t n_nonuniform, float* pos, uint32_t* idx, uint32_t* hist, uint32_t key_shift) {
	if (n_uniform) hipLaunchKernelGGL(k_grid_samples, dim3((n_uniform + 127) / 128), dim3(128), 0, s, n_uniform, rng, ema_step, c->aabb, c->density_grid.p,
	                                  pos, idx, -0.01f, hist, key_shift);
	rng.advance();
	if (n_nonuniform) hipLaunchKernelGGL(k_grid_samples, dim3((n_nonuniform + 127) / 128), dim3(128), 0, s, n_nonuniform, rng, ema_step, c->aabb, c->density_grid.p,
	                                     pos + (size_t)n_uniform * 3, idx + n_uniform, MIN_OPTICAL_THICKNESS, hist, key_shift);
	rng.advance();
	HIP_TRY(hipGetLastError());
	return RNB_OK;
}

static int pregenerate_grid_samples(rnb_ctx* c, hipStream_t s_main) {
	if (!c->gs_todo.pending) return RNB_OK;
	c->gs_todo.pending = false;
	c->gs_pre.valid = false;
	const uint32_t n_uniform = c->gs_todo.n_uniform, n_nonuniform = c->gs_todo.n_nonuniform;
	if (!c->knobs.grid_presort || c->training_step < 256 || n_nonuniform == 0) return RNB_OK;
	const uint32_t n_elements = GRID_CELLS * (c->aabb.max_cascade + 1);
	const uint32_t n = n_uniform + n_nonuniform;
	uint32_t shift = 3;
	while ((n_elements >> shift) > (1u << 20)) ++shift;
	const uint32_t n_keys = n_elements >> shift;
	if (!c->gs_sorted_pos.p) {
		if (c->gs_range.alloc(2) != hipSuccess || c->gs_sorted_pos.alloc((size_t)n * 3) != hipSuccess || c->gs_sorted_idx.alloc(n) != hipSuccess || c->gs_hist.alloc((size_t)(1u << 20) + 2048) != hipSuccess ||
		    c->gs_stage_pos.alloc(c->grid_sample_pos.n) != hipSuccess || c->gs_stage_idx.alloc(c->grid_sample_idx.n) != hipSuccess ||
		    c->gs_eval_pos.alloc((size_t)n * 3) != hipSuccess || c->gs_eval_idx.alloc(n) != hipSuccess) {
			if (c->cfg.world_size > 1 && c->grid_exchange) return fail(RNB_ERR_NOMEM, "hipMalloc failed for the cell-ordered occupancy samples (data parallel: every rank must evaluate the same order)");
			c->knobs.grid_presort = false;
			return RNB_OK;
		}
	}
	hipStream_t s = s_main;
	if (c->overlap()) {
		s = c->s_dw;
		HIP_TRY(hipStreamWaitEvent(s, c->ev_grid, 0));
	}
	HIP_TRY(hipMemsetAsync(c->gs_hist.p, 0, sizeof(uint32_t) * n_keys, s));
	if (c->density_grid_tmp_alt.p) {
		HIP_TRY(hipMemsetAsync(c->density_grid_tmp_alt.p, 0, sizeof(float) * n_elements, s));
		c->tmp_alt_clear = true;
	}
	Pcg32 rng = c->density_grid_rng;
	c->gs_pre.rng_state = rng.state; c->gs_pre.rng_inc = rng.inc;
	int rc = launch_grid_samples(c, s, rng, c->density_grid_ema_step, n_uniform, n_nonuniform, c->gs_stage_pos.p, c->gs_stage_idx.p, c->gs_hist.p, shift);
	if (rc != RNB_OK) return rc;
	const uint32_t nb = (n_keys + 1023) / 1024;
	uint32_t* sums = c->gs_hist.p + (1u << 20);
	hipLaunchKernelGGL(k_scan_blocks, dim3(nb), dim3(1024), 0, s, c->gs_hist.p, (uint64_t)n_keys, sums);
	hipLaunchKernelGGL(k_scan_blocks, dim3(1), dim3(1024), 0, s, sums, (uint64_t)nb, sums + 1024);
	hipLaunchKernelGGL(k_scan_add, dim3(nb), dim3(1024), 0, s, c->gs_hist.p, (uint64_t)n_keys, sums);
	hipLaunchKernelGGL(k_grid_samples_place, dim3((n + 127) / 128), dim3(128), 0, s, n, c->gs_stage_pos.p, c->gs_stage_idx.p, c->gs_hist.p, shift, c->gs_sorted_pos.p, c->gs_sorted_idx.p);
	if (c->cfg.world_size > 1) hipLaunchKernelGGL(k_shard_range, dim3(1), dim3(64), 0, s, c->gs_hist.p, n_keys, n, c->cfg.world_size, c->cfg.rank, c->gs_range.p);
	HIP_TRY(hipGetLastError());
	HIP_TRY(hipEventRecord(c->ev_gs, s));
	c->gs_pre.valid = true; c->gs_pre.ema_step = c->density_grid_ema_step; c->gs_pre.n_uniform = n_uniform; c->gs_pre.n_nonuniform = n_nonuniform;
	return RNB_OK;
}

int update_density_grid_front(rnb_ctx* c, hipStream_t s, uint32_t n_uniform, uint32_t n_nonuniform, bool shard) {
	const uint32_t n_elements = GRID_CELLS * (c->aabb.max_cascade + 1);
	const uint32_t n_samples = n_uniform + n_nonuniform;
	c->prof.mark(s, P_NONE);
	if (c->training_step == 0) {
		c->density_grid_ema_step = 0;
		HIP_TRY(hipMemsetAsync(c->density_grid.p, 0, sizeof(float) * n_elements, s));
		c->gs_pre.valid = false;
	}
	const bool sorted = c->gs_pre.valid && c->gs_pre.ema_step == c->density_grid_ema_step && c->gs_pre.n_uniform == n_uniform && c->gs_pre.n_nonuniform == n_nonuniform &&
	                    c->gs_pre.rng_state == c->density_grid_rng.state && c->gs_pre.rng_inc == c->density_grid_rng.inc;
	c->gs_pre.valid = false;
	c->last_update_sorted = sorted;
	if (sorted && c->tmp_alt_clear) c->density_grid_tmp.swap(c->density_grid_tmp_alt);
	else HIP_TRY(hipMemsetAsync(c->density_grid_tmp.p, 0, sizeof(float) * n_elements, s));
	c->tmp_alt_clear = false;
	if (sorted) {
		HIP_TRY(hipStreamWaitEvent(s, c->ev_gs, 0));
		c->grid_sample_pos.swap(c->gs_stage_pos);
		c->grid_sample_idx.swap(c->gs_stage_idx);
		c->gs_sorted_pos.swap(c->gs_eval_pos);
		c->gs_sorted_idx.swap(c->gs_eval_idx);
		c->density_grid_rng.advance();
		c->density_grid_rng.advance();
	} else {
		int rc = launch_grid_samples(c, s, c->density_grid_rng, c->density_grid_ema_step, n_uniform, n_nonuniform, c->grid_sample_pos.p, c->grid_sample_idx.p, nullptr, 0);
		if (rc != RNB_OK) return rc;
	}
	c->prof.mark(s, P_GRID_SAMPLES);
	c->n_grid_samples = n_samples;
	int rc;
	const uint64_t W = shard ? c->cfg.world_size : 1u, r = shard ? c->cfg.rank : 0u;
	if (sorted) {
		rc = launch_point_query(c, s, c->gs_eval_pos.p, n_samples, nullptr, c->gs_eval_idx.p, c->density_grid_tmp.p, 1, false, W > 1 ? c->gs_range.p : nullptr);
	} else {
		const uint32_t lo = (uint32_t)((uint64_t)n_samples * r / W), hi = (uint32_t)((uint64_t)n_samples * (r + 1) / W);
		rc = launch_point_query(c, s, c->grid_sample_pos.p + (size_t)lo * 3, hi - lo, nullptr, c->grid_sample_idx.p + lo, c->density_grid_tmp.p, 1, false);
	}
	if (rc != RNB_OK) return rc;
	c->prof.mark(s, P_POINT_QUERY);
	c->prof.units[P_POINT_QUERY] += n_samples / W;
	c->gs_todo.n_uniform = n_uniform; c->gs_todo.n_nonuniform = n_nonuniform;
	return RNB_OK;
}

int update_density_grid_back(rnb_ctx* c, hipStream_t s) {
	const uint32_t n_elements = GRID_CELLS * (c->aabb.max_cascade + 1);
	int rc;
	hipLaunchKernelGGL(k_ema_mean, dim3(n_elements / 2048), dim3(256), 0, s, n_elements, c->cfg.density_grid_decay, c->density_grid.p, c->density_grid_tmp.p, c->mean_partial.p);
	HIP_TRY(hipGetLastError());
	++c->density_grid_ema_step;
	rc = update_bitfield(c, s, !c->overlap(), true);
	c->prof.mark(s, P_EMA_BITFIELD);
	c->gs_todo.pending = true;
	return rc;
}

int training_prep_front(rnb_ctx* c, hipStream_t s, bool shard) {
	const uint32_t n_cascades = c->aabb.max_cascade + 1;
	if (c->training_step < 256) return update_density_grid_front(c, s, GRID_CELLS * n_cascades, 0, shard);
	return update_density_grid_front(c, s, GRID_CELLS / 4 * n_cascades, GRID_CELLS / 4 * n_cascades, shard);
}
int training_prep(rnb_ctx* c, hipStream_t s) {
	const bool shard = c->grid_exchange != nullptr && c->dp_order();
	int rc = training_prep_front(c, s, shard);
	if (rc != RNB_OK) return rc;
	if (shard) {
		const int xrc = c->grid_exchange(c->grid_exchange_user, c->density_grid_tmp.p, (uint64_t)GRID_CELLS * (c->aabb.max_cascade + 1), (void*)s);
		if (xrc != 0) return fail(RNB_ERR_INVALID, "the occupancy grid exchange (rnb_set_grid_exchange) failed");
	}
	return update_density_grid_back(c, s);
}

static int ensure_rgb_buffers(rnb_ctx* c) {
	if (c->cin_eval.p) return RNB_OK;
	const size_t B = c->cfg.target_batch_size;
	if (c->cin_eval.alloc(B * 16 * 32) != hipSuccess || c->dcin.alloc(B * 32) != hipSuccess || c->rgb_out_scratch.alloc(B * 16) != hipSuccess || c->src_slot.alloc(B) != hipSuccess)
		return fail(RNB_ERR_NOMEM, "hipMalloc failed for the colour-MLP training buffers");
	return RNB_OK;
}

int launch_forward(rnb_ctx* c, hipStream_t s, const float* coords, const uint32_t* n_ptr, uint32_t n_max, half_t* out, bool inference, const uint32_t* idx = nullptr, half_t* cin_out = nullptr) {
	if (n_max == 0) return RNB_OK;
	join_tail_host(c);
	FwdArgs a;
	a.coords = coords; a.n_ptr = n_ptr; a.n_max = n_max; a.out = out; a.sdf_bias = c->cfg.sdf_bias; a.idx = idx; a.cin_out = cin_out;
	a.wimg = (!inference && c->wimg_valid) ? c->wimg_fwd.p : nullptr;
	const uint32_t n_tiles = (n_max + TILE - 1) / TILE;
	const uint32_t grid = std::min<uint32_t>((n_tiles + WAVES_PER_WG - 1) / WAVES_PER_WG, (uint32_t)c->n_cus * 2);
	if (c->half_acc()) hipLaunchKernelGGL(k_forward_chained_emul_pipe<4>, dim3(grid), dim3(WG), LDS_FWD2, s, c->meta(), c->net(inference), a);
	else hipLaunchKernelGGL(k_forward_chained_pipe<4>, dim3(grid), dim3(WG), LDS_FWD2, s, c->meta(), c->net(inference), a);
	HIP_TRY(hipGetLastError());
	return RNB_OK;
}

static LossFlags loss_flags(const rnb_ctx* c) {
	LossFlags F;
	F.apply_L2 = c->cfg.apply_L2; F.apply_rgbplus = c->cfg.apply_rgbplus; F.apply_no_albedo = c->cfg.apply_no_albedo; F.apply_light_opti = c->cfg.apply_light_opti;
	F.apply_relu = c->cfg.apply_relu; F.apply_bce = c->cfg.apply_bce; F.snap = c->cfg.snap_to_pixel_centers;
	F.mask_loss_weight = c->cfg.mask_loss_weight; F.ek_loss_weight = c->cfg.ek_loss_weight;
	return F;
}

static bool large_batch(const rnb_ctx* c, uint32_t n_rays) { return n_rays >= c->knobs.march_narrow_from; }
static uint32_t scan_tiles_of(uint32_t n_rays) { return (n_rays + SCAN_TILE - 1) / SCAN_TILE; }

static uint32_t k1_for(const rnb_ctx* c, uint32_t n_rays) {
	if (c->fwd_k1 == 0 || c->fwd_k1_fixed) return c->fwd_k1;
	const float k = 8.f + 3.f * (float)c->cfg.target_batch_size / (float)std::max(1u, n_rays);
	const uint32_t k8 = (uint32_t)std::min(48.f, std::max(16.f, k) + 4.f) / 8u * 8u;
	return std::min(c->fwd_k1, std::max(16u, k8));
}

static bool lattice_is_linear() {
	const volatile float C = STEPSIZE;
	for (int e = -1; e <= 3; ++e) {
		const float base = std::ldexp(0.5f, e), ulp = std::ldexp(1.0f, e - 1 - 23);
		const volatile float d0 = (base + C) - base;
		for (const float t : {base, base + ulp, base + 2 * ulp, base + 3 * ulp, std::ldexp(1.0f, e) - 64 * d0, std::ldexp(1.0f, e) - 64 * d0 + ulp}) {
			const volatile float sum = t + C;
			if (sum - t != d0) return false;
		}
	}
	return true;
}

constexpr uint32_t MARCH_WAVE_PER_RAY_BELOW = 4096;

MarchArgs march_args(rnb_ctx* c, uint32_t n_rays, uint32_t n_rays_total, uint32_t max_samples) {
	MarchArgs a;
	static const bool linear = lattice_is_linear();
	a.lattice_ok = linear ? 1u : 0u;
	a.n_rays = n_rays;
	a.n_rays_global = n_rays * c->cfg.world_size;
	a.ray_offset = c->cfg.rank * n_rays;
	a.n_rays_total = n_rays_total;
	a.max_samples = max_samples;
	a.n_images = c->n_views;
	a.snap = c->cfg.snap_to_pixel_centers;
	a.rng = c->rng;
	a.A = c->aabb;
	a.views = c->views.p;
	a.bitfield = c->bitfield.p; a.coarse = c->coarse_bits.p;
	{
		const uint32_t seen = *reinterpret_cast<volatile uint32_t*>(c->host_coarse);
		const uint32_t budget = seen == 0xffffffffu ? 0u : (seen + seen / 8 + 64 + 63) / 64 * 64;
		a.n_blocks_lds = seen <= COARSE_MAX_BLOCKS ? std::min(budget, COARSE_MAX_BLOCKS) : 0u;
	}
	a.setup = c->ray_setup.p; a.ray_t = c->ray_t.p; a.d_unnorm = c->ray_dunnorm.p; a.steps = c->ray_steps.p; a.base = c->ray_base.p; a.slot = c->ray_slot.p;
	a.ray_indices = c->ray_indices.p; a.rays = c->rays.p; a.numsteps = c->numsteps.p; a.coords = c->coords.p; a.counters = c->counters.p;
	a.base1 = c->ray_base1.p; a.idx1 = c->idx1.p; a.k1 = k1_for(c, n_rays);
	a.F = loss_flags(c);
	for (int k = 0; k < 9; ++k) a.light_dirs[k] = c->light_dirs[k];
	a.part = 0;
	a.stats = c->march_stats.p;
	a.use_bbox = (uint32_t)c->knobs.march_bbox;
	return a;
}

int generate_training_samples(rnb_ctx* c, hipStream_t s, uint32_t n_rays, uint32_t n_rays_total, uint32_t max_samples, hipEvent_t done = nullptr, hipEvent_t wait_before_write = nullptr, hipEvent_t rest_done = nullptr, hipEvent_t wait_before_scans = nullptr) {
	if (!c->coarse_valid) { const int rc0 = rebuild_coarse(c, s); if (rc0 != RNB_OK) return rc0; }
	MarchArgs a = march_args(c, n_rays, n_rays_total, max_samples);
	c->gen_k1 = a.k1;
	const uint32_t blocks = (n_rays + 127) / 128;
	c->prof.mark(s, P_NONE);
	const bool sc = c->aabb.cone_angle == 0.f && c->aabb.max_cascade == 0;
	const size_t march_lds = sc ? (size_t)(2 * COARSE_WORDS + 2 * a.n_blocks_lds) * sizeof(uint32_t) : 0;
	MarchArgs ar = a;
	if (c->knobs.march_skip == 2) ar.lattice_ok |= LATTICE_REFUSE_REENTRY;
	if (c->knobs.march_narrow || large_batch(c, n_rays)) {
		if (sc && c->knobs.march_skip && c->knobs.march_skip_narrow && a.lattice_ok) {
			hipLaunchKernelGGL(k_march_count_skip_narrow, dim3(blocks), dim3(128), march_lds + COARSE_WORDS * sizeof(uint32_t), s, ar);
		} else if (sc && c->knobs.march_bbox >= 2 && a.lattice_ok) {
// ... 47 lines not shown
	a.src_slot = c->cin_flow ? c->src_slot.p : nullptr;
	a.chain_rec = c->knobs.loss_chain_records ? c->chain_rec.p : nullptr;
	a.ray_grad = c->ray_grad.p; a.ray_of = c->ray_of.p; a.slot_of = c->slot_of.p;
	a.scan_words = nullptr; a.scan_ticket = 0; a.scan_error = nullptr; a.scan_total = nullptr;
	a.wg_partial = c->wg_partial.p; a.red_out = nullptr; a.red_host_out = nullptr; a.red_host_seq = 0;
	c->loss_reduced = false;
	if (!c->pre.loss_cleared && !defer_rollover) HIP_TRY(hipMemsetAsync(c->loss.p, 0, c->loss.bytes(), s));
	c->pre.loss_cleared = false;
	const uint32_t blocks = (n_rays + 3) / 4;
	const bool rows = large_batch(c, n_rays) && !c->knobs.loss_wave_per_ray;
	const uint32_t blocks_heads = rows ? (n_rays + LOSS1_WG / 16 - 1) / (LOSS1_WG / 16) : (n_rays + LOSS1_WG / 64 - 1) / (LOSS1_WG / 64);
	auto launch_heads = [&]() {
		if (rows) hipLaunchKernelGGL(k_loss_pass1_heads<16>, dim3(blocks_heads), dim3(LOSS1_WG), 0, s, a);
		else hipLaunchKernelGGL(k_loss_pass1_heads<64>, dim3(blocks_heads), dim3(LOSS1_WG), 0, s, a);
	};
	a.cap = 0xffffffffu; a.phase = 0; a.unfinished = c->unfinished.p; a.idx2 = c->idx2.p; a.fwd_counts = c->fwd_counts.p;
	c->prof.mark(s, P_NONE);
	if (two_round_n_max) {
		a.cap = c->cur_k1;
		launch_heads();
		c->prof.mark(s, P_LOSS_PASS1);
		int rc = launch_forward(c, s, c->coords.p, c->fwd_counts.p + 2, two_round_n_max, c->mlp_out.p, false, c->idx2.p, c->cin_flow ? c->cin_eval.p : nullptr);
		if (rc != RNB_OK) return rc;
		c->prof.mark(s, P_FORWARD);
		a.phase = 1;
	}
	if (a.phase) hipLaunchKernelGGL(k_loss_pass1, dim3(std::min(blocks, 1024u)), dim3(256), 0, s, a);
	else launch_heads();
	c->prof.mark(s, P_LOSS_PASS1);
	const bool flat = a.chain_rec && c->knobs.loss_flat;
	if (flat && c->knobs.loss_scan_fused && scan_tiles_of(n_rays) <= (c->knobs.loss_scan_fused_always ? SCAN_MAX_TILES : 8u)) {
		a.scan_words = c->scan_words.p + 64 * 4; a.scan_ticket = ++c->scan_ticket; a.scan_error = c->host_coarse_dev + 6; a.scan_total = c->counters.p + 1;
	} else if (large_batch(c, n_rays)) {
		hipLaunchKernelGGL(k_scan_compact_chain, dim3(scan_tiles_of(n_rays)), dim3(SCAN_WG), 0, s, n_rays, c->ncomp.p, c->cbase.p, c->counters.p,
		                   c->scan_words.p + 64 * 4, ++c->scan_ticket, c->host_coarse_dev + 6);
	} else
		hipLaunchKernelGGL(k_scan_compact, dim3(1), dim3(1024), 0, s, n_rays, c->ncomp.p, c->cbase.p, c->counters.p);
	c->prof.mark(s, P_SCAN_COMPACT);
	if (flat) {
		hipLaunchKernelGGL(k_loss_pass2_rays<16>, dim3((n_rays + 15) / 16), dim3(256), 0, s, a);
		hipEvent_t ev = nullptr;
		if (reduce_too) {
			const bool poll = c->poll_loss();
			if (poll) { if (++c->rb_seq == 0) ++c->rb_seq; c->loss_polled = false; }
			a.red_out = c->loss_sums.p; a.red_host_out = reinterpret_cast<double*>(c->host_rb_dev); a.red_host_seq = poll ? c->rb_seq : 0u;
			ev = poll ? nullptr : c->ev_loss;
			c->loss_reduced = true;
		}
		LAUNCH_EV(k_loss_pass2_samples, dim3(1 + (a.B + 255) / 256), dim3(256), 0, s, ev, a);
		c->prof.mark(s, P_LOSS_PASS2);
		HIP_TRY(hipGetLastError());
		return RNB_OK;
	} else if (a.chain_rec) {
		if (rows) hipLaunchKernelGGL((k_loss_pass2<16, true>), dim3((n_rays + 15) / 16), dim3(256), 0, s, a);
		else hipLaunchKernelGGL((k_loss_pass2<64, true>), dim3(blocks), dim3(256), 0, s, a);
	} else {
		if (rows) hipLaunchKernelGGL((k_loss_pass2<16, false>), dim3((n_rays + 15) / 16), dim3(256), 0, s, a);
		else hipLaunchKernelGGL((k_loss_pass2<64, false>), dim3(blocks), dim3(256), 0, s, a);
	}
	if (!defer_rollover) hipLaunchKernelGGL(k_rollover, dim3(1024), dim3(256), 0, s, c->cfg.target_batch_size, c->counters.p, c->dloss_dout.p, c->coords_compacted.p, a.src_slot);
	c->prof.mark(s, P_LOSS_PASS2);
	HIP_TRY(hipGetLastError());
	return RNB_OK;
}

int forward_backward(rnb_ctx* c, hipStream_t s, bool join_dw = true) {
	const uint32_t B = c->cfg.target_batch_size;
	const rnb_ctx::ScatterGroups& sg = c->sg;
	const uint32_t L = c->cfg.n_levels;
	const uint32_t e_c = sg.e_c, l_fine = sg.l_fine;
	join_tail_host(c);
	const bool half = c->half_acc();
	if (!c->grads_clean) HIP_TRY(hipMemsetAsync(c->grad_ptr(0), 0, c->n_params * c->grad_elem(), s));
	c->grads_clean = false;
	c->sc.valid = false; c->sc.exchanged = false; c->sc.sharded = false; c->sc.all_final_recorded = false; c->sc.dw_joined = true;
	TrainArgs a;
	a.coords = c->coords_compacted.p; a.dout = c->dloss_dout.p; a.B = B; a.B_global = B * c->cfg.world_size; a.sdf_bias = c->cfg.sdf_bias; a.t = c->ts; a.skip_rgb = c->cfg.apply_no_albedo ? 1u : 0u;
	const bool split = c->rgb_split();
	a.wimg = !c->wimg_valid ? nullptr : (!c->knobs.fwd_bwd_generic) ? c->wimg_fbs.p : c->wimg_train.p;
	const bool sdf_only = (a.skip_rgb && !c->knobs.fwd_bwd_generic) || split;
	const uint32_t fb_grid = sdf_only ? std::min<uint32_t>((B / TILE + WAVES_PER_WG - 1) / WAVES_PER_WG, (uint32_t)c->n_cus * 2) : c->fwd_grid;
	const bool sliced = half && sdf_only && c->knobs.dw_sliced;
	const uint32_t n_slices = (B + DW_SLICE - 1) / DW_SLICE;
	const size_t slab = sliced ? (size_t)n_slices : sdf_only ? (size_t)fb_grid : (size_t)c->dw_nwg;
	float* p_rgb2; float* p_rgb1; float* p_rgb0; float* p_sdf1; float* p_sdf0; float* p_sdf0b; float* p_sdf1b;
	{
		float* p = c->dw_partial.p;
		p_rgb2 = p;  p += slab * 16 * 64;
		p_rgb1 = p;  p += slab * 64 * 64;
		p_rgb0 = p;  p += slab * 64 * 32;
		p_sdf1 = p;  p += slab * 16 * 64;
		p_sdf0 = p;  p += slab * 64 * 32;
		p_sdf0b = p; p += slab * 64 * 32;
		p_sdf1b = p; p += slab * 16 * 64;
	}
	a.dw_w0 = p_sdf0; a.dw_w0b = p_sdf0b; a.dw_w1 = p_sdf1; a.dw_w1b = p_sdf1b;
	const bool side_streams = c->overlap();
	c->prof.mark(s, P_NONE);
	hipEvent_t ev_fb = side_streams ? c->ev_fb : nullptr;
	if (split) {
		int rc = ensure_rgb_buffers(c);
		if (rc != RNB_OK) return rc;
		const bool flow = c->cin_flow;
		c->cin_flow = false;
		if (!flow) {
			rc = launch_forward(c, s, c->coords_compacted.p, nullptr, B, c->rgb_out_scratch.p, false, nullptr, c->cin_eval.p);
			if (rc != RNB_OK) return rc;
		}
		RgbArgs r;
		r.cin = c->cin_eval.p; r.src_slot = flow ? c->src_slot.p : nullptr; r.dout = c->dloss_dout.p; r.dcin = c->dcin.p; r.B = B;
		r.wimg = c->wimg_valid ? c->wimg_rgb.p : nullptr;
		r.dw_c0 = p_rgb0; r.dw_c1 = p_rgb1; r.dw_c2 = p_rgb2;
		r.t = c->ts;
		if (half && sliced) hipLaunchKernelGGL(k_rgb_fwd_bwd_hs, dim3(fb_grid), dim3(WG), LDS_RGB, s, c->net(false), r);
		else if (half) hipLaunchKernelGGL(k_rgb_fwd_bwd_h, dim3(fb_grid), dim3(WG), LDS_RGB, s, c->net(false), r);
		else hipLaunchKernelGGL(k_rgb_fwd_bwd, dim3(fb_grid), dim3(WG), LDS_RGB, s, c->net(false), r);
		a.dcin = c->dcin.p;
		if (half && sliced) LAUNCH_EV(k_fwd_bwd_sdf_full_hs, dim3(fb_grid), dim3(WG), LDS_FBS_FULL, s, ev_fb, c->meta(), c->net(false), a);
		else if (half) LAUNCH_EV(k_fwd_bwd_sdf_full_h, dim3(fb_grid), dim3(WG), LDS_FBS_FULL, s, ev_fb, c->meta(), c->net(false), a);
		else LAUNCH_EV(k_fwd_bwd_sdf_full, dim3(fb_grid), dim3(WG), LDS_FBS_FULL, s, ev_fb, c->meta(), c->net(false), a);
	} else if (sdf_only && half && sliced) LAUNCH_EV(k_fwd_bwd_sdf_hs, dim3(fb_grid), dim3(WG), LDS_FBS, s, ev_fb, c->meta(), c->net(false), a);
	else if (sdf_only && half) LAUNCH_EV(k_fwd_bwd_sdf_h, dim3(fb_grid), dim3(WG), LDS_FBS, s, ev_fb, c->meta(), c->net(false), a);
	else if (sdf_only) LAUNCH_EV(k_fwd_bwd_sdf, dim3(fb_grid), dim3(WG), LDS_FBS, s, ev_fb, c->meta(), c->net(false), a);
	else LAUNCH_EV(k_fwd_bwd, dim3(fb_grid), dim3(WG), LDS_TRAIN, s, ev_fb, c->meta(), c->net(false), a);
	c->prof.mark(s, P_FWD_BWD);
	c->prof.units[P_FWD_BWD] += B;
	const TrainScratch& T = c->ts;

	auto launch_dw = [&](hipStream_t sd, hipEvent_t done) {
		const uint32_t nwg = c->dw_nwg, chunk = c->dw_chunk;
		DwAllArgs d;
		d.n = 0; d.nwg = nwg; d.B = B; d.chunk = chunk;
		auto add = [&](uint32_t kind, const half_t* yt, const half_t* xt, float* part) { d.kind[d.n] = kind; d.YT[d.n] = yt; d.XT[d.n] = xt; d.partial[d.n] = part; ++d.n; };
		if (!a.skip_rgb) {
			add(DW_4x4, T.dh2, T.h1, p_rgb1);
			add(DW_4x2, T.dh1, T.cin, p_rgb0);
			add(DW_1x4, T.dr, T.h2, p_rgb2);
		}
		add(DW_4x2, T.dz, T.sdfin, p_sdf0);
		add(DW_4x2, T.dz1, T.ddin, p_sdf0b);
		add(DW_1x4, T.dso, T.z1, p_sdf1);
		add(DW_1x4_ONES, nullptr, T.front, p_sdf1b);
		for (uint32_t q = d.n; q < 7; ++q) { d.kind[q] = DW_1x4; d.YT[q] = nullptr; d.XT[q] = nullptr; d.partial[q] = nullptr; }
		if (!sdf_only) hipLaunchKernelGGL(k_dw_all, dim3(nwg * d.n), dim3(WG), 0, sd, d);
		if (sliced) {
			DwSlicedArgs q;
			q.n = 0; q.B = B; q.n_slices = n_slices;
			uint32_t wgs = 0;
			auto add_sliced = [&](const half_t* yt, const half_t* xt, float* out, uint32_t n_out, uint32_t n_live, uint32_t n_in, uint32_t ones) {
				q.YT[q.n] = yt; q.XT[q.n] = xt; q.out[q.n] = out; q.n_out[q.n] = n_out; q.n_out_live[q.n] = n_live; q.n_in[q.n] = n_in; q.ones[q.n] = ones;
				q.first_wg[q.n] = wgs; wgs += n_slices * ((n_out * n_in / 4 + 255) / 256); ++q.n;
			};
			if (!a.skip_rgb) {
				add_sliced(T.dh2, T.h1, p_rgb1, 64, 64, 64, 0);
				add_sliced(T.dh1, T.cin, p_rgb0, 64, 64, 32, 0);
				add_sliced(T.dr, T.h2, p_rgb2, 16, 3, 64, 0);
			}
			add_sliced(T.dz, T.sdfin, p_sdf0, 64, 64, 32, 0);
			add_sliced(T.dz1, T.ddin, p_sdf0b, 64, 64, 32, 0);
			add_sliced(T.dso, T.z1, p_sdf1, 16, split ? 16 : 1, 64, 0);
			add_sliced(nullptr, T.front, p_sdf1b, 16, 1, 64, 1);
			for (uint32_t g = q.n; g < 7; ++g) { q.YT[g] = nullptr; q.XT[g] = nullptr; q.out[g] = nullptr; q.n_out[g] = 0; q.n_out_live[g] = 0; q.n_in[g] = 4; q.ones[g] = 0; }
			for (uint32_t g = q.n; g < 8; ++g) q.first_wg[g] = wgs;
			hipLaunchKernelGGL(k_dw_sliced, dim3(wgs), dim3(256), 0, sd, q);
		}
		DwFinishArgs f;
		f.partial[0] = p_rgb2; f.partial[1] = p_rgb1; f.partial[2] = p_rgb0; f.partial[3] = p_sdf1; f.partial[4] = p_sdf0; f.partial[5] = p_sdf0b; f.partial[6] = p_sdf1b;
		f.n_partials = (uint32_t)slab; f.sliced = sliced ? 1u : 0u;
		f.var_partial = c->var_partial.p; f.n_var_partials = fb_grid * WAVES_PER_WG;
		f.grads = c->grads.p; f.grads16 = half ? c->grads16.p : nullptr; f.off_sdf = (uint32_t)c->off_sdf; f.off_rgb = (uint32_t)c->off_rgb; f.off_var = (uint32_t)c->off_var; f.skip_rgb = a.skip_rgb;
		const uint32_t n_fin_blocks = (RNB_N_SDF_MLP_PARAMS + (a.skip_rgb ? 0 : RNB_N_RGB_MLP_PARAMS)) / DWF_PARAMS + 1;
		LAUNCH_EV(k_dw_finish, dim3(n_fin_blocks), dim3(DWF_WG), 0, sd, done, f);
	};

	const uint32_t scatter_cap = (sdf_only && !split) ? 0u : 2u;
	ScatterArgs sa;
	sa.g12 = T.g12; sa.srec = T.srec; sa.B = B; sa.grid_grad = half ? nullptr : c->grads.p + c->off_grid;
	sa.grid_grad16 = half ? reinterpret_cast<uint32_t*>(c->grads16.p + c->off_grid) : nullptr;
	const bool fixed = c->fixed_acc();
	sa.grid_fixed = fixed ? c->grads_fixed.p : nullptr;
	auto narrow = [&](hipStream_t st, hipEvent_t done, uint32_t l0, uint32_t l1) {
		const uint64_t lo = (uint64_t)c->grid.offsets[l0] * 2, hi = (uint64_t)c->grid.offsets[l1] * 2;
		if (hi <= lo) { if (done) (void)hipEventRecord(done, st); return; }
		const uint32_t blocks = (uint32_t)std::min<uint64_t>(2048, ((hi - lo) / 2 + 255) / 256);
		LAUNCH_EV(k_fixed_narrow, dim3(blocks), dim3(256), 0, st, done, c->grads_fixed.p, half ? nullptr : c->grads.p + c->off_grid, half ? c->grads16.p + c->off_grid : nullptr, lo, hi);
	};
	bool sc_first = true;
	auto sc_flags = [&]() -> uint32_t { const bool any = side_streams && !sc_first; sc_first = false; return any ? (uint32_t)hipExtAnyOrderLaunch : 0u; };
	auto launch_a = [&](hipStream_t st, hipEvent_t done, uint32_t l0, uint32_t l1) {
		const uint32_t n_vb = (B * 4 + 255) / 256, cap = scatter_cap ? std::max(1u, (uint32_t)c->n_cus * scatter_cap / std::max(1u, l1 - l0)) : n_vb;
		if (l1 > l0 && fixed) {
			LAUNCH_EVF(k_grid_scatter_quad_fixed, dim3(std::min(n_vb, cap), l1 - l0), dim3(256), 0, st, nullptr, sc_flags(), c->meta(), sa, l0, n_vb);
			narrow(st, done, l0, l1);
		} else if (l1 > l0 && half && c->knobs.scatter_plain) LAUNCH_EVF(k_grid_scatter_quad_h_per_addend, dim3(std::min(n_vb, cap), l1 - l0), dim3(256), 0, st, done, sc_flags(), c->meta(), sa, l0, n_vb);
		else if (l1 > l0 && half) LAUNCH_EVF(k_grid_scatter_quad_h, dim3(std::min(n_vb, cap), l1 - l0), dim3(256), 0, st, done, sc_flags(), c->meta(), sa, l0, n_vb);
		else if (l1 > l0) LAUNCH_EVF(k_grid_scatter_quad, dim3(std::min(n_vb, cap), l1 - l0), dim3(256), 0, st, done, sc_flags(), c->meta(), sa, l0, n_vb);
		else if (done) (void)hipEventRecord(done, st);
	};
	auto launch_b = [&](hipStream_t st, hipEvent_t done) {
		if (l_fine <= e_c) { if (done) (void)hipEventRecord(done, st); return; }
		ScatterRlPlan plan;
		plan.n = l_fine - e_c; plan.k_log2 = sg.k_log2;
		uint32_t wg = 0;
		for (uint32_t q = 0; q < plan.n; ++q) { plan.wg_start[q] = wg; wg += (((B + sg.Ks[e_c + q] - 1) / sg.Ks[e_c + q]) * 4 + 255) / 256; }
		plan.wg_start[plan.n] = wg;
		const uint32_t cap_rl = scatter_cap ? (uint32_t)c->n_cus * scatter_cap : wg;
		const bool staged = c->cur_n_rays != 0 && !large_batch(c, c->cur_n_rays);
// ... 331 lines not shown
	const uint32_t n_grid = GRID_CELLS * (c->aabb.max_cascade + 1);
#define ALLOC(buf, count)                                                                                              \
	do {                                                                                                               \
		if ((buf).alloc(count) != hipSuccess) { rnb_destroy(c); return fail(RNB_ERR_NOMEM, "hipMalloc failed for " #buf); } \
	} while (0)
	{
		const uint64_t q = 4ull * std::max(1u, cfg->world_size);
		c->param_capacity = (c->n_params + q - 1) / q * q;
	}
#define ALLOC_P(buf)                                                                                                   \
	do {                                                                                                               \
		if ((buf).alloc_padded(c->n_params, c->param_capacity) != hipSuccess) { rnb_destroy(c); return fail(RNB_ERR_NOMEM, "hipMalloc failed for " #buf); } \
	} while (0)
	if (getenv("RNB_MARCH_STATS")) { if (c->march_stats.alloc_padded(8, 8) != hipSuccess) { rnb_destroy(c); return fail(RNB_ERR_NOMEM, "hipMalloc failed"); } }
	ALLOC(c->adam_lr_table, ADAM_LR_TABLE_N);
	ALLOC(c->opt_rec, c->param_capacity * 4);
	if (cfg->accumulate == RNB_ACCUM_HALF) ALLOC_P(c->grads16); else ALLOC_P(c->grads);
	if (c->cfg.deterministic) {
		if (c->grads_fixed.alloc_padded(c->n_grid_params, c->n_grid_params) != hipSuccess) { rnb_destroy(c); return fail(RNB_ERR_NOMEM, "hipMalloc failed for the fixed-point gradient accumulators"); }
	}
	ALLOC_P(c->params_fp32); ALLOC_P(c->adam_m); ALLOC_P(c->adam_v); ALLOC_P(c->params_fp16); ALLOC_P(c->params_ema); ALLOC_P(c->adam_steps);
#undef ALLOC_P
	ALLOC(c->density_grid, n_grid); ALLOC(c->density_grid_tmp, n_grid); ALLOC(c->density_grid_tmp_alt, n_grid); ALLOC(c->density_mean, 1); ALLOC(c->mean_partial, 1024); ALLOC(c->loss_sums, 16);
	ALLOC(c->bitfield, (size_t)GRID_CELLS / 8 * N_CASCADES); ALLOC(c->coarse_bits, COARSE_BUF_WORDS); ALLOC(c->coarse_count, 1);
	ALLOC(c->grid_sample_pos, (size_t)n_grid * 3); ALLOC(c->grid_sample_idx, n_grid);
	ALLOC(c->ray_indices, maxr); ALLOC(c->numsteps, (size_t)maxr * 2); ALLOC(c->counters, 4); ALLOC(c->rays, (size_t)maxr * 6);
	ALLOC(c->coords, (size_t)B * 16 * 7); ALLOC(c->mlp_out, (size_t)B * 16 * 16); ALLOC(c->chain_rec, (size_t)B * 16 * CHAIN_REC_FLOATS); ALLOC(c->ray_grad, (size_t)maxr * 16); ALLOC(c->ray_of, B); ALLOC(c->slot_of, B); ALLOC(c->wg_partial, ((size_t)maxr + 15) / 16 * 3); ALLOC(c->dloss_dout, (size_t)B * 16); ALLOC(c->coords_compacted, (size_t)B * 7);
	ALLOC(c->loss, (size_t)maxr * 3); c->ek_loss = c->loss.p + maxr; c->mask_loss = c->loss.p + (size_t)maxr * 2;
	ALLOC(c->ray_setup, (size_t)maxr * 8); ALLOC(c->ray_t, (size_t)maxr * RNB_MAX_STEPS); ALLOC(c->ray_dunnorm, (size_t)maxr * 3); ALLOC(c->ray_steps, maxr); ALLOC(c->ray_base, maxr); ALLOC(c->ray_slot, maxr);
	ALLOC(c->loss_partial, 64 * 3);
	ALLOC(c->ncomp, maxr); ALLOC(c->cbase, maxr); ALLOC(c->ray_loss, maxr);
	ALLOC(c->wimg_fwd, W_FWD_END); ALLOC(c->wimg_fbs, SWF_END); ALLOC(c->wimg_train, W_TRAIN_END); ALLOC(c->wimg_rgb, RW_END);
	ALLOC(c->ray_const, (size_t)maxr * RAY_CONST_FLOATS); ALLOC(c->ray_base1, maxr); ALLOC(c->scan_words, 3 * 64 * 4); ALLOC(c->unfinished, maxr); ALLOC(c->fwd_counts, 4); ALLOC(c->idx1, (size_t)B * 16); ALLOC(c->idx2, (size_t)B * 16);
	ALLOC(c->fm, (size_t)B * (8 * 64 + 3 * 32 + 2 * 16));
	ALLOC(c->g12, (size_t)B * 14 * 2); ALLOC(c->srec, (size_t)B * 8);
	{
		half_t* q = c->fm.p;
		TrainScratch& T = c->ts;
		T.h2 = q; q += (size_t)B * 64; T.h1 = q; q += (size_t)B * 64; T.z1 = q; q += (size_t)B * 64; T.dz1 = q; q += (size_t)B * 64;
		T.dh2 = q; q += (size_t)B * 64; T.dh1 = q; q += (size_t)B * 64; T.dz = q; q += (size_t)B * 64; T.front = q; q += (size_t)B * 64;
		T.cin = q; q += (size_t)B * 32; T.sdfin = q; q += (size_t)B * 32; T.ddin = q; q += (size_t)B * 32;
		T.dr = q; q += (size_t)B * 16; T.dso = q; q += (size_t)B * 16;
		T.g12 = c->g12.p; T.srec = c->srec.p;
	}
	c->fwd_grid = std::min<uint32_t>((B / TILE + WAVES_PER_WG - 1) / WAVES_PER_WG, (uint32_t)c->n_cus);
	ALLOC(c->var_partial, (size_t)c->n_cus * 3 * WAVES_PER_WG);
	c->ts.var_partial = c->var_partial.p;
	{
		const uint32_t units = B / 128;
		uint32_t nwg = 1;
		for (uint32_t d = 1; d <= std::min<uint32_t>(units, 256u); ++d) if (units % d == 0) nwg = d;
		c->dw_nwg = nwg;
		c->dw_chunk = B / nwg;
		const size_t per_wave = (size_t)16 * 64 * 3 + 64 * 64 + (size_t)64 * 32 * 3;
		ALLOC(c->dw_partial, (size_t)std::max<uint32_t>(nwg * WAVES_PER_WG, (uint32_t)c->n_cus * 2) * per_wave);
	}
#undef ALLOC
	HIP_TRY_C(hipMemset(c->params_fp32.p, 0, c->params_fp32.bytes()));
	HIP_TRY_C(hipMemset(c->params_fp16.p, 0, c->params_fp16.bytes()));
	HIP_TRY_C(hipMemset(c->params_ema.p, 0, c->params_ema.bytes()));
	HIP_TRY_C(hipMemset(c->density_grid.p, 0, c->density_grid.bytes()));
	HIP_TRY_C(hipMemset(c->density_grid_tmp.p, 0, c->density_grid_tmp.bytes()));
	HIP_TRY_C(hipMemset(c->bitfield.p, 0, c->bitfield.bytes()));
	HIP_TRY_C(hipMemset(c->counters.p, 0, c->counters.bytes()));
	HIP_TRY_C(hipMemset(c->density_mean.p, 0, 4));
	HIP_TRY_C(hipMemset(c->coords.p, 0, c->coords.bytes()));
	HIP_TRY_C(hipMemset(c->coords_compacted.p, 0, c->coords_compacted.bytes()));
	HIP_TRY_C(hipMemset(c->dloss_dout.p, 0, c->dloss_dout.bytes()));
	HIP_TRY_C(hipMemset(c->mlp_out.p, 0, c->mlp_out.bytes()));
	int rc = reset_optimizer_state(c);
	if (rc != RNB_OK) { rnb_destroy(c); return rc; }
	HIP_TRY_C(hipFuncSetAttribute(reinterpret_cast<const void*>(k_forward_chained_emul_pipe<4>), hipFuncAttributeMaxDynamicSharedMemorySize, (int)LDS_FWD2));
	HIP_TRY_C(hipFuncSetAttribute(reinterpret_cast<const void*>(k_forward_chained_pipe<4>), hipFuncAttributeMaxDynamicSharedMemorySize, (int)LDS_FWD2));
	HIP_TRY_C(hipFuncSetAttribute(reinterpret_cast<const void*>(k_fwd_bwd), hipFuncAttributeMaxDynamicSharedMemorySize, (int)LDS_TRAIN));
	HIP_TRY_C(hipFuncSetAttribute(reinterpret_cast<const void*>(k_fwd_bwd_sdf), hipFuncAttributeMaxDynamicSharedMemorySize, (int)LDS_FBS));
	HIP_TRY_C(hipFuncSetAttribute(reinterpret_cast<const void*>(k_fwd_bwd_sdf_full), hipFuncAttributeMaxDynamicSharedMemorySize, (int)LDS_FBS_FULL));
	HIP_TRY_C(hipFuncSetAttribute(reinterpret_cast<const void*>(k_rgb_fwd_bwd), hipFuncAttributeMaxDynamicSharedMemorySize, (int)LDS_RGB));
	HIP_TRY_C(hipFuncSetAttribute(reinterpret_cast<const void*>(k_fwd_bwd_sdf_h), hipFuncAttributeMaxDynamicSharedMemorySize, (int)LDS_FBS));
	HIP_TRY_C(hipFuncSetAttribute(reinterpret_cast<const void*>(k_fwd_bwd_sdf_hs), hipFuncAttributeMaxDynamicSharedMemorySize, (int)LDS_FBS));
	HIP_TRY_C(hipFuncSetAttribute(reinterpret_cast<const void*>(k_fwd_bwd_sdf_full_hs), hipFuncAttributeMaxDynamicSharedMemorySize, (int)LDS_FBS_FULL));
	HIP_TRY_C(hipFuncSetAttribute(reinterpret_cast<const void*>(k_rgb_fwd_bwd_hs), hipFuncAttributeMaxDynamicSharedMemorySize, (int)LDS_RGB));
	HIP_TRY_C(hipFuncSetAttribute(reinterpret_cast<const void*>(k_fwd_bwd_sdf_full_h), hipFuncAttributeMaxDynamicSharedMemorySize, (int)LDS_FBS_FULL));
	HIP_TRY_C(hipFuncSetAttribute(reinterpret_cast<const void*>(k_rgb_fwd_bwd_h), hipFuncAttributeMaxDynamicSharedMemorySize, (int)LDS_RGB));
	HIP_TRY_C(hipFuncSetAttribute(reinterpret_cast<const void*>(k_grid_scatter_lds_h), hipFuncAttributeMaxDynamicSharedMemorySize, 150 * 1024));
	{
		const int march_lds_max = (int)((2 * COARSE_WORDS + 2 * COARSE_MAX_BLOCKS) * sizeof(uint32_t));
		HIP_TRY_C(hipFuncSetAttribute(reinterpret_cast<const void*>(k_march_count<true>), hipFuncAttributeMaxDynamicSharedMemorySize, march_lds_max));
		HIP_TRY_C(hipFuncSetAttribute(reinterpret_cast<const void*>(k_march_count_wide<16, true>), hipFuncAttributeMaxDynamicSharedMemorySize, march_lds_max));
		HIP_TRY_C(hipFuncSetAttribute(reinterpret_cast<const void*>(k_march_count_wide<64, true, 256>), hipFuncAttributeMaxDynamicSharedMemorySize, march_lds_max));
		HIP_TRY_C(hipFuncSetAttribute(reinterpret_cast<const void*>(k_march_count_skip<1024>), hipFuncAttributeMaxDynamicSharedMemorySize, march_lds_max + (int)(COARSE_WORDS * sizeof(uint32_t))));
		HIP_TRY_C(hipFuncSetAttribute(reinterpret_cast<const void*>(k_march_count_skip_narrow), hipFuncAttributeMaxDynamicSharedMemorySize, march_lds_max + (int)(COARSE_WORDS * sizeof(uint32_t))));
		HIP_TRY_C(hipFuncSetAttribute(reinterpret_cast<const void*>(k_march_count_bbox), hipFuncAttributeMaxDynamicSharedMemorySize, march_lds_max));
	}
HIP_TRY_C(hipFuncSetAttribute(reinterpret_cast<const void*>(k_grid_scatter_lds), hipFuncAttributeMaxDynamicSharedMemorySize, 150 * 1024));
	HIP_TRY_C(hipFuncSetAttribute(reinterpret_cast<const void*>(k_grid_scatter_lds_fixed), hipFuncAttributeMaxDynamicSharedMemorySize, 150 * 1024));
	c->rng = Pcg32{cfg->seed};
	c->density_grid_rng = Pcg32{c->rng.next_uint()};
	(void)c->rng.next_uint();
	c->rays_per_batch = std::min(cfg->initial_rays_per_batch, cfg->max_rays_per_batch);
	c->training_step = 0;
	c->valid_level = compute_valid_level(c->cfg, 0);
	build_light_dirs(c);
	if (const char* e = getenv("RNB_FWD_K1")) { c->fwd_k1 = (uint32_t)atoi(e); c->fwd_k1_fixed = true; }
	{
		rnb_ctx::Knobs& k = c->knobs;
		k.march_narrow = getenv("RNB_MARCH_NARROW") != nullptr; k.fwd_bwd_generic = getenv("RNB_FWD_BWD_GENERIC") != nullptr;
		k.loss_wave_per_ray = getenv("RNB_LOSS_WAVE_PER_RAY") != nullptr;
		k.dp_order = getenv("RNB_DP_FORCE_COLLECTIVES") != nullptr;
		if (const char* e = getenv("RNB_MARCH_NARROW_FROM")) k.march_narrow_from = (uint32_t)atoi(e);
		if (const char* e = getenv("RNB_GRID_PRESORT")) k.grid_presort = atoi(e) != 0;
		if (const char* e = getenv("RNB_LOSS_SCAN_FUSED")) { k.loss_scan_fused = atoi(e) != 0; k.loss_scan_fused_always = atoi(e) == 2; }
		if (const char* e = getenv("RNB_LOSS_FLAT")) k.loss_flat = atoi(e) != 0;
		if (const char* e = getenv("RNB_LOSS_CHAIN_RECORDS")) k.loss_chain_records = atoi(e) != 0;
		if (const char* e = getenv("RNB_SCATTER_PLAIN")) k.scatter_plain = atoi(e) != 0;
		if (const char* e = getenv("RNB_DW_SLICED")) k.dw_sliced = atoi(e) != 0;
		if (const char* e = getenv("RNB_MARCH_SKIP")) k.march_skip = std::max(0, std::min(2, atoi(e)));
		if (const char* e = getenv("RNB_MARCH_SKIP_NARROW")) k.march_skip_narrow = atoi(e) != 0;
		if (const char* e = getenv("RNB_MARCH_BBOX")) k.march_bbox = std::max(0, std::min(2, atoi(e)));
	}
	plan_scatter_groups(c);
	for (hipStream_t* st : {&c->s_march, &c->s_dw, &c->s_adam}) HIP_TRY_C(hipStreamCreateWithFlags(st, hipStreamNonBlocking));
	HIP_TRY_C(hipEventCreateWithFlags(&c->ev_loss, hipEventDisableTiming));
	const unsigned dev_flags = hipEventDisableTiming | (unsigned)hipEventDisableSystemFence;
	for (hipEvent_t* e : {&c->ev_march, &c->ev_fb, &c->ev_dw, &c->ev_adam, &c->ev_tail, &c->ev_march_rest, &c->ev_all, &c->ev_grid, &c->ev_gs, &c->ev_sc[0], &c->ev_sc[1], &c->ev_sc[2]}) HIP_TRY_C(hipEventCreateWithFlags(e, dev_flags));
	HIP_TRY_C(hipHostMalloc(reinterpret_cast<void**>(&c->host_rb), sizeof(*c->host_rb), hipHostMallocMapped));
	std::memset(c->host_rb, 0, sizeof(*c->host_rb));
	HIP_TRY_C(hipHostGetDevicePointer(&c->host_rb_dev, c->host_rb, 0));
	HIP_TRY_C(hipHostMalloc(reinterpret_cast<void**>(&c->host_coarse), 64, hipHostMallocMapped));
	std::memset(c->host_coarse, 0, 64);
	*c->host_coarse = 0xffffffffu;
	HIP_TRY_C(hipMemset(c->scan_words.p, 0, c->scan_words.bytes()));
	HIP_TRY_C(hipHostGetDevicePointer(reinterpret_cast<void**>(&c->host_coarse_dev), c->host_coarse, 0));
	*out = c;
	return RNB_OK;
#undef HIP_TRY_C
} RNB_GUARD

int rnb_update_config(rnb_ctx* c, const rnb_config* cfg) try {
	if (!c || !cfg) return fail(RNB_ERR_INVALID, "null argument");
	discard_premarch(c);
	int rc = update_config_common(c->cfg, cfg);
	if (rc != RNB_OK) return rc;
	build_light_dirs(c);
	return RNB_OK;
} RNB_GUARD

uint64_t rnb_n_params(const rnb_ctx* c) { return c ? c->n_params : 0; }

int rnb_param_layout(const rnb_ctx* c, uint64_t offsets[5]) try {
	if (!c || !offsets) return fail(RNB_ERR_INVALID, "null argument");
	offsets[0] = c->off_sdf; offsets[1] = c->off_rgb; offsets[2] = c->off_grid; offsets[3] = c->off_var; offsets[4] = c->n_params;
	return RNB_OK;
} RNB_GUARD

int rnb_grid_tables(const rnb_ctx* c, uint32_t* offsets, uint32_t* resolution, float* scale) try {
	if (!c) return fail(RNB_ERR_INVALID, "null ctx");
	for (uint32_t i = 0; i <= c->cfg.n_levels; ++i) if (offsets) offsets[i] = c->grid.offsets[i];
	for (uint32_t i = 0; i < c->cfg.n_levels; ++i) { if (resolution) resolution[i] = c->grid.resolution[i]; if (scale) scale[i] = c->grid.scale[i]; }
	return RNB_OK;
} RNB_GUARD

int rnb_init_params(rnb_ctx* c, const float* sdf_w) try {
	if (!c || !sdf_w) return fail(RNB_ERR_INVALID, "null argument");
	discard_premarch(c);
	HIP_TRY(hipDeviceSynchronize());
	std::seed_seq seq{c->cfg.seed};
// ... 422 lines not shown
	const uint64_t Bg = (uint64_t)c->cfg.target_batch_size * c->cfg.world_size;
	const uint32_t n_rays = c->cur_n_rays;
	c->measured_batch_size = 0;
	c->measured_batch_size_before_compaction = 0;
	float loss_scalar = 0.f, ek_scalar = 0.f, mask_scalar = 0.f;
	uint32_t next_rays = c->rays_per_batch;
	int rc = RNB_OK;
	if (counters[0] == 0 || counters[1] == 0) {
		rc = RNB_ERR_NO_SAMPLES;
		g_err = "Nerf training generated 0 samples.";
	} else {
		c->measured_batch_size_before_compaction = c->local_measured_before;
		c->measured_batch_size = (uint32_t)(counters[1] / c->cfg.world_size);
		const float measured = (float)counters[1], target = (float)Bg;
		loss_scalar = (float)sums[0] * measured / target;
		ek_scalar = (float)sums[1] * measured / target;
		mask_scalar = (float)sums[2] * measured / target;
		next_rays = (uint32_t)((float)c->rays_per_batch * target / measured);
		next_rays = std::min(next_multiple_u32(next_rays, 128u), c->cfg.max_rays_per_batch);
	}
	if (stats) {
		stats->training_step = c->cur_step + 1;
		stats->rays_per_batch = n_rays;
		stats->next_rays_per_batch = next_rays;
		stats->measured_batch_size = (uint32_t)(counters[1] / c->cfg.world_size);
		stats->measured_batch_size_before_compaction = (uint32_t)(counters[0] / c->cfg.world_size);
		stats->n_rays_kept = (uint32_t)(counters[2] / c->cfg.world_size);
		stats->density_grid_updated = c->grid_updated ? 1 : 0;
		stats->loss = loss_scalar; stats->ek_loss = ek_scalar; stats->mask_loss = mask_scalar;
		stats->prep_ms = c->prep_ms;
		stats->step_ms = std::chrono::duration<float, std::milli>(std::chrono::steady_clock::now() - c->step_start).count();
	}
	c->rays_per_batch = next_rays;
	if (rc != RNB_OK) return rc;
	return launch_premarch(c);
} RNB_GUARD

int rnb_train_step_end(rnb_ctx* c, void* stream, rnb_step_stats* stats) try {
	if (c && c->overlap()) {
		uint64_t counters[4];
		double sums[3];
		int rc = rnb_train_step_local(c, stream, counters, sums);
		if (rc != RNB_OK) return rc;
		const int rc_finish = rnb_train_step_finish(c, counters, sums, stats);
		rc = rnb_train_step_apply(c, stream);
		return rc != RNB_OK ? rc : rc_finish;
	}
	int rc = rnb_train_step_apply(c, stream);
	if (rc != RNB_OK) return rc;
	uint64_t counters[4];
	double sums[3];
	rc = rnb_train_step_local(c, stream, counters, sums);
	if (rc != RNB_OK) return rc;
	return rnb_train_step_finish(c, counters, sums, stats);
} RNB_GUARD

int rnb_train_step(rnb_ctx* c, void* stream, rnb_step_stats* stats) try {
	int rc = rnb_train_step_begin(c, stream);
	if (rc != RNB_OK) return rc;
	return rnb_train_step_end(c, stream, stats);
} RNB_GUARD

int rnb_profile_enable(rnb_ctx* c, int on) try {
	if (!c) return fail(RNB_ERR_INVALID, "null ctx");
	c->prof.on = on != 0;
	c->prof.reset();
	return RNB_OK;
} RNB_GUARD
int rnb_profile_count(const rnb_ctx*) { return P_COUNT; }
int rnb_profile_get(const rnb_ctx* c, int idx, const char** name, double* total_ms, uint64_t* launches, double* units) try {
	if (!c || idx < 0 || idx >= P_COUNT) return fail(RNB_ERR_INVALID, "bad profile index");
	if (name) *name = PROF_NAMES[idx];
	if (total_ms) *total_ms = c->prof.total_ms[idx];
	if (launches) *launches = c->prof.launches[idx];
	if (units) *units = c->prof.units[idx];
	return RNB_OK;
} RNB_GUARD

uint32_t rnb_training_step(const rnb_ctx* c) { return c ? c->training_step : 0; }
uint32_t rnb_rays_per_batch(const rnb_ctx* c) { return c ? c->rays_per_batch : 0; }

int rnb_eval_primitives(rnb_ctx* c, int kind, const uint32_t* in_host, uint32_t n_items, uint32_t* out_host) try {
	if (!c || (!in_host && n_items) || (!out_host && n_items)) return fail(RNB_ERR_INVALID, "null argument");
	if (kind < 0 || kind > RNB_PRIM_DW_SLICED) return fail(RNB_ERR_INVALID, "unknown primitive kind");
	if (n_items == 0) return RNB_OK;
	if (kind == RNB_PRIM_PREP_DUE) {
		for (uint32_t i = 0; i < n_items; ++i) { out_host[2 * i] = prep_due(in_host[i]) ? 1u : 0u; out_host[2 * i + 1] = std::min(std::max(in_host[i] / 16u, 1u), 16u); }
		return RNB_OK;
	}
	const size_t n_in = (size_t)n_items * PRIM_IN_WORDS[kind], n_out = (size_t)n_items * PRIM_OUT_WORDS[kind], n_bf = (size_t)GRID_CELLS / 8 * N_CASCADES;
	uint32_t *in = nullptr, *out = nullptr;
	uint8_t* bf = nullptr;
	int rc = RNB_OK;
	if (hipMalloc((void**)&in, n_in * 4) != hipSuccess || hipMalloc((void**)&out, n_out * 4) != hipSuccess || ((kind == RNB_PRIM_MARCH || kind == RNB_PRIM_MARCH_RAY) && hipMalloc((void**)&bf, n_bf) != hipSuccess))
		rc = fail(RNB_ERR_NOMEM, "hipMalloc failed for the primitive self-test");
	std::vector<uint32_t> own;
	if (kind == RNB_PRIM_RAY_TARGETS) {
		own.assign(in_host, in_host + n_in);
		for (uint32_t i = 0; i < n_items; ++i) {
			uint32_t* ld = own.data() + (size_t)i * PRIM_IN_WORDS[kind] + 26;
			bool all = true;
			for (int k = 0; k < 9; ++k) all = all && ld[k] == 0xffffffffu;
			if (all) std::memcpy(ld, c->light_dirs, 36);
		}
		in_host = own.data();
	}
	if (rc == RNB_OK && hipMemcpy(in, in_host, n_in * 4, hipMemcpyHostToDevice) != hipSuccess) rc = fail(RNB_ERR_DEVICE, "rnb_eval_primitives: copy in failed");
	if (rc == RNB_OK) {
		if (bf) hipLaunchKernelGGL(k_prim_bitfield, dim3((uint32_t)((n_bf + 255) / 256)), dim3(256), 0, 0, bf, (uint32_t)n_bf);
		if (kind == RNB_PRIM_DW_SLICED) {
			const uint32_t S = PRIM_DW_SAMPLES, n_sl = (S + DW_SLICE - 1) / DW_SLICE;
			float* tmp = nullptr;
			if (hipMalloc((void**)&tmp, (size_t)n_sl * 16 * 4) != hipSuccess) rc = fail(RNB_ERR_NOMEM, "hipMalloc failed for the primitive self-test");
			for (uint32_t i = 0; i < n_items && rc == RNB_OK; ++i) {
				const uint32_t* item = in + (size_t)i * PRIM_IN_WORDS[kind];
				DwSlicedArgs q;
				for (uint32_t g = 0; g < 7; ++g) { q.YT[g] = nullptr; q.XT[g] = nullptr; q.out[g] = nullptr; q.n_out[g] = 0; q.n_out_live[g] = 0; q.n_in[g] = 4; q.ones[g] = 0; }
				const bool ones = (in_host[(size_t)i * PRIM_IN_WORDS[kind]] & 1u) != 0u;
				q.YT[0] = reinterpret_cast<const half_t*>(item + 4); q.XT[0] = q.YT[0] + (size_t)4 * S; q.out[0] = tmp;
				q.n_out[0] = 4; q.n_out_live[0] = ones ? 1u : 4u; q.n_in[0] = 4; q.ones[0] = ones ? 1u : 0u;
				q.n = 1; q.B = S; q.n_slices = n_sl; q.first_wg[0] = 0;
				for (uint32_t g = 1; g < 8; ++g) q.first_wg[g] = n_sl;
				hipLaunchKernelGGL(k_dw_sliced, dim3(n_sl), dim3(256), 0, 0, q);
				hipLaunchKernelGGL(k_prim_dw_sliced_total, dim3(1), dim3(64), 0, 0, tmp, 16u, n_sl, reinterpret_cast<float*>(out + (size_t)i * 16));
			}
			(void)hipDeviceSynchronize();
			if (tmp) (void)hipFree(tmp);
		} else if (kind == RNB_PRIM_ENCODE) hipLaunchKernelGGL(k_prim_encode, dim3(n_items), dim3(64), 0, 0, in, n_items, out);
		else hipLaunchKernelGGL(k_primitives, dim3((n_items + 127) / 128), dim3(128), 0, 0, kind, in, n_items, out, bf);
		if (hipGetLastError() != hipSuccess || hipDeviceSynchronize() != hipSuccess || hipMemcpy(out_host, out, n_out * 4, hipMemcpyDeviceToHost) != hipSuccess)
			rc = fail(RNB_ERR_DEVICE, "rnb_eval_primitives: kernel or copy out failed");
	}
	if (in) (void)hipFree(in);
	if (out) (void)hipFree(out);
	if (bf) (void)hipFree(bf);
	return rc;
} RNB_GUARD

int rnb_set_optimizer_step(rnb_ctx* c, uint32_t step) try {
	if (!c) return fail(RNB_ERR_INVALID, "null ctx");
	HIP_TRY(hipDeviceSynchronize());
	c->opt.begun = false;
	c->optimizer_step_count = step;
	c->lr_factor = 1.0f;
	for (uint64_t s0 = c->cfg.lr_decay_start; s0 < step && s0 <= 10000000u; s0 += std::max(1u, c->cfg.lr_decay_interval)) c->lr_factor *= c->cfg.lr_decay_base;
	return RNB_OK;
} RNB_GUARD

int rnb_set_controller(rnb_ctx* c, uint32_t training_step, uint32_t rays_per_batch, uint32_t measured_before, uint32_t n_rays_total) try {
	if (!c) return fail(RNB_ERR_INVALID, "null ctx");
	if (rays_per_batch == 0 || rays_per_batch > c->cfg.max_rays_per_batch) return fail(RNB_ERR_INVALID, "rays_per_batch out of range");
	discard_premarch(c);
	c->training_step = training_step;
	c->valid_level = compute_valid_level(c->cfg, (int)training_step);
	c->rays_per_batch = rays_per_batch;
	c->measured_batch_size_before_compaction = measured_before;
	c->n_rays_total = n_rays_total;
	return RNB_OK;
} RNB_GUARD

int rnb_gradient_parts(rnb_ctx* c, uint64_t ranges[3][2], uint32_t* n_parts) try {
	if (!c || !ranges || !n_parts) return fail(RNB_ERR_INVALID, "null argument");
	c->sc.exchanged = true;
	if (c->sc.valid && c->sc.dp) {
		const bool mid = c->sc.split_mid > c->sc.split[0] && c->sc.split_mid < c->off_var;
		ranges[0][0] = 0;              ranges[0][1] = c->sc.split[0];
		ranges[1][0] = c->sc.split[0]; ranges[1][1] = mid ? c->sc.split_mid : c->n_params;
		if (mid) { ranges[2][0] = c->sc.split_mid; ranges[2][1] = c->n_params; }
// ... 62 lines not shown
```

Baseline: 52.05 million.

## Gather hash-grid corners cooperatively across lanes via LDS transpose

```diff
diff --git a/include/rnb_neus2.h b/include/rnb_neus2.h
--- a/include/rnb_neus2.h
+++ b/include/rnb_neus2.h
@@ -190,7 +190,7 @@
                        uint32_t measured_batch_size_before_compaction, uint32_t n_rays_total);
 
 typedef enum rnb_primitive { RNB_PRIM_PCG32 = 0, RNB_PRIM_MORTON = 1, RNB_PRIM_SRGB = 2, RNB_PRIM_RAY_BOX = 3, RNB_PRIM_MARCH = 4,
-                             RNB_PRIM_ACTIVATION = 5, RNB_PRIM_WARP = 6, RNB_PRIM_LOSS = 7, RNB_PRIM_PIXEL = 8, RNB_PRIM_GRID = 9, RNB_PRIM_READ_RGBA = 10, RNB_PRIM_CAMERA_RAY = 11, RNB_PRIM_RAY_TARGETS = 12, RNB_PRIM_LOSS_SAMPLE = 13, RNB_PRIM_RAY_LOSS = 14, RNB_PRIM_ENCODE = 15, RNB_PRIM_MARCH_RAY = 16, RNB_PRIM_SDF_DENSITY = 17, RNB_PRIM_PREP_DUE = 18, RNB_PRIM_DW_SLICED = 19 } rnb_primitive;
+                             RNB_PRIM_ACTIVATION = 5, RNB_PRIM_WARP = 6, RNB_PRIM_LOSS = 7, RNB_PRIM_PIXEL = 8, RNB_PRIM_GRID = 9, RNB_PRIM_READ_RGBA = 10, RNB_PRIM_CAMERA_RAY = 11, RNB_PRIM_RAY_TARGETS = 12, RNB_PRIM_LOSS_SAMPLE = 13, RNB_PRIM_RAY_LOSS = 14, RNB_PRIM_ENCODE = 15, RNB_PRIM_MARCH_RAY = 16, RNB_PRIM_SDF_DENSITY = 17, RNB_PRIM_PREP_DUE = 18, RNB_PRIM_DW_SLICED = 19, RNB_PRIM_ENCODE_FORM = 20 } rnb_primitive;
 int rnb_eval_primitives(rnb_ctx* ctx, int kind, const uint32_t* in_host, uint32_t n_items, uint32_t* out_host);
 
 int rnb_gradient_parts(rnb_ctx* ctx, uint64_t ranges[3][2], uint32_t* n_parts);
diff --git a/rnb-neus2_amd/_abi.py b/rnb-neus2_amd/_abi.py
--- a/rnb-neus2_amd/_abi.py
+++ b/rnb-neus2_amd/_abi.py
@@ -102,8 +102,8 @@
 ACCUM_FP32, ACCUM_HALF = 0, 1
 BUF_READONLY = 0x100
 GRID_EXCHANGE_FN = C.CFUNCTYPE(C.c_int, C.c_void_p, C.c_void_p, C.c_uint64, C.c_void_p)
-PRIM = dict(PCG32=0, MORTON=1, SRGB=2, RAY_BOX=3, MARCH=4, ACTIVATION=5, WARP=6, LOSS=7, PIXEL=8, GRID=9, READ_RGBA=10, CAMERA_RAY=11, RAY_TARGETS=12, LOSS_SAMPLE=13, RAY_LOSS=14, ENCODE=15, MARCH_RAY=16, SDF_DENSITY=17, PREP_DUE=18, DW_SLICED=19)
-PRIM_IN_WORDS, PRIM_OUT_WORDS = (6, 3, 1, 8, 9, 1, 9, 9, 9, 7, 32, 20, 35, 37, 16, 263, 10, 2, 1, 33028), (4, 4, 2, 3, 7, 3, 11, 5, 3, 3, 5, 9, 7, 28, 9, 16, 23, 1, 2, 16)
+PRIM = dict(PCG32=0, MORTON=1, SRGB=2, RAY_BOX=3, MARCH=4, ACTIVATION=5, WARP=6, LOSS=7, PIXEL=8, GRID=9, READ_RGBA=10, CAMERA_RAY=11, RAY_TARGETS=12, LOSS_SAMPLE=13, RAY_LOSS=14, ENCODE=15, MARCH_RAY=16, SDF_DENSITY=17, PREP_DUE=18, DW_SLICED=19, ENCODE_FORM=20)
+PRIM_IN_WORDS, PRIM_OUT_WORDS = (6, 3, 1, 8, 9, 1, 9, 9, 9, 7, 32, 20, 35, 37, 16, 263, 10, 2, 1, 33028, 1), (4, 4, 2, 3, 7, 3, 11, 5, 3, 3, 5, 9, 7, 28, 9, 16, 23, 1, 2, 16, 1)
 H2D, D2H, D2D = 0, 1, 2
 
 _ctx = C.c_void_p
diff --git a/rnb-neus2_amd/api.py b/rnb-neus2_amd/api.py
--- a/rnb-neus2_amd/api.py
+++ b/rnb-neus2_amd/api.py
@@ -330,6 +330,9 @@
         out = np.empty((a.shape[0], _abi.PRIM_OUT_WORDS[k]), dtype=np.uint32)
         self._check(self.f.eval_primitives(self._h, k, a.ctypes.data_as(C.c_void_p), a.shape[0], out.ctypes.data_as(C.c_void_p)))
         return out
+
+    def set_encode_corners(self, mask):
+        return int(self.eval_primitives("ENCODE_FORM", [int(mask)])[0, 0])
 
     def training_state(self, last_stats=None):
         return dict(params=self.get("PARAMS_FP32").copy(), adam_m=self.get("ADAM_M").copy(), adam_v=self.get("ADAM_V").copy(), adam_steps=self.get("ADAM_STEPS").copy(),
diff --git a/rnb-neus2_amd/csrc/common.cuh b/rnb-neus2_amd/csrc/common.cuh
--- a/rnb-neus2_amd/csrc/common.cuh
+++ b/rnb-neus2_amd/csrc/common.cuh
@@ -319,6 +319,44 @@
 	}
 }
 
+struct __attribute__((aligned(16))) CornerSlab { uint4 cell[64]; uint32_t val[64 * 8]; };
+__device__ __forceinline__ void level_issue_corners(const LevelMeta* __restrict__ lm, const uint32_t* __restrict__ grid, const uint32_t level, const float x, const float y, const float z,
+                                                    CornerSlab* __restrict__ cs, const int lane, uint32_t (&r)[8]) {
+	const uint4 raw = reinterpret_cast<const uint4*>(lm + level)[0], raw2 = reinterpret_cast<const uint4*>(lm + level)[1];
+	const uint32_t off = __builtin_amdgcn_readfirstlane(raw.x), hashmap_size = __builtin_amdgcn_readfirstlane(raw.y);
+	const float scale = __uint_as_float(__builtin_amdgcn_readfirstlane(raw.w));
+	const uint32_t my = __builtin_amdgcn_readfirstlane(raw2.x), mz = __builtin_amdgcn_readfirstlane(raw2.y);
+	const bool dense = __builtin_amdgcn_readfirstlane(raw2.z) != 0u, pow2 = __builtin_amdgcn_readfirstlane(raw2.w) != 0u;
+	const uint32_t* __restrict__ g = grid + off;
+	float pos[3];
+	uint32_t pg[3];
+	pos_fract(x, scale, &pos[0], &pg[0]);
+	pos_fract(y, scale, &pos[1], &pg[1]);
+	pos_fract(z, scale, &pos[2], &pg[2]);
+	cs->cell[lane] = uint4{pg[0], pg[1] * my, pg[2] * mz, 0u};
+	wave_lds_sync();
+	const uint32_t cx = (uint32_t)lane & 1u, cy = ((uint32_t)lane & 2u) ? my : 0u, cz = ((uint32_t)lane & 4u) ? mz : 0u;
+#pragma unroll
+	for (uint32_t i = 0; i < 8; ++i) {
+		const uint4 b = cs->cell[8u * i + ((uint32_t)lane >> 3)];
+		const uint32_t px = b.x + cx, ty = b.y + cy, tz = b.z + cz;
+		uint32_t e = dense ? px + ty + tz : (px ^ (ty ^ tz));
+		const uint32_t w = e >= hashmap_size ? e - hashmap_size : e;
+		e = pow2 ? (e & (hashmap_size - 1u)) : w;
+		r[i] = g[e];
+	}
+}
+__device__ __forceinline__ void level_collect_corners(CornerSlab* __restrict__ cs, const int lane, const uint32_t (&r)[8], uint32_t (&v)[8]) {
+#pragma unroll
+	for (uint32_t i = 0; i < 8; ++i) cs->val[64u * i + ((uint32_t)lane ^ ((i & 1u) ? 4u : 0u))] = r[i];
+	wave_lds_sync();
+	const uint32_t swap = ((uint32_t)lane >> 3) & 1u;
+	const uint4 lo = *reinterpret_cast<const uint4*>(cs->val + 8u * (uint32_t)lane + 4u * swap), hi = *reinterpret_cast<const uint4*>(cs->val + 8u * (uint32_t)lane + 4u * (swap ^ 1u));
+	v[0] = lo.x; v[1] = lo.y; v[2] = lo.z; v[3] = lo.w;
+	v[4] = hi.x; v[5] = hi.y; v[6] = hi.z; v[7] = hi.w;
+	wave_lds_sync();
+}
+
 struct Vec3 { float x, y, z; };
 __device__ __forceinline__ Vec3 v3(float x, float y, float z) { return {x, y, z}; }
 __device__ __forceinline__ Vec3 operator+(Vec3 a, Vec3 b) { return {a.x + b.x, a.y + b.y, a.z + b.z}; }
diff --git a/rnb-neus2_amd/csrc/kernels_net.cuh b/rnb-neus2_amd/csrc/kernels_net.cuh
--- a/rnb-neus2_amd/csrc/kernels_net.cuh
+++ b/rnb-neus2_amd/csrc/kernels_net.cuh
@@ -43,21 +43,37 @@
 	}
 }
 
-template <bool GRAD, int DEPTH>
+__device__ __forceinline__ int tile_local(int lane) { asm volatile("" : "+v"(lane)); return lane; }
+
+template <bool GRAD, int DEPTH, bool CORNERS = false>
 __device__ __forceinline__ void encode_all_pipelined(const LevelMeta* __restrict__ lm, const uint32_t n_levels, const uint32_t valid_level, const uint32_t* __restrict__ grid,
-                                                     const float x, const float y, const float z, half_t (&feat)[28], float (&dydx)[GRAD ? 28 : 1][3]) {
+                                                     const float x, const float y, const float z, half_t (&feat)[28], float (&dydx)[GRAD ? 28 : 1][3],
+                                                     CornerSlab* __restrict__ cs = nullptr, const int lane = 0) {
 	const uint32_t n_live = min(n_levels, valid_level + 1u);
 	uint32_t v[DEPTH][8];
-	const uint32_t last = n_live ? n_live - 1u : 0u;
-#pragma unroll
-	for (uint32_t l = 0; l < (uint32_t)DEPTH; ++l) level_issue(lm, grid, min(l, last), x, y, z, v[l]);
+	uint32_t last = n_live ? n_live - 1u : 0u;
+	const int cl = CORNERS ? tile_local(lane) : 0;
+	if constexpr (CORNERS) last = __builtin_amdgcn_readfirstlane((uint32_t)tile_local((int)last));
+#pragma unroll
+	for (uint32_t l = 0; l < (uint32_t)DEPTH; ++l) {
+		if constexpr (CORNERS) level_issue_corners(lm, grid, min(l, last), x, y, z, cs, cl, v[l]);
+		else level_issue(lm, grid, min(l, last), x, y, z, v[l]);
+	}
 #pragma unroll
 	for (uint32_t level = 0; level < 14; ++level) {
 		half_t f0, f1;
 		float d0[3], d1[3];
 		const bool live = level < n_live;
-		level_consume<GRAD>(lm, min(level, last), x, y, z, v[level % DEPTH], f0, f1, d0, d1);
-		if (level + DEPTH < 14) level_issue(lm, grid, min(level + (uint32_t)DEPTH, last), x, y, z, v[level % DEPTH]);
+		if constexpr (CORNERS) {
+			uint32_t w[8];
+			level_collect_corners(cs, cl, v[level % DEPTH], w);
+			level_consume<GRAD>(lm, min(level, last), x, y, z, w, f0, f1, d0, d1);
+			if (level + DEPTH < 14) level_issue_corners(lm, grid, min(level + (uint32_t)DEPTH, last), x, y, z, cs, cl, v[level % DEPTH]);
+			__builtin_amdgcn_sched_barrier(0);
+		} else {
+			level_consume<GRAD>(lm, min(level, last), x, y, z, v[level % DEPTH], f0, f1, d0, d1);
+			if (level + DEPTH < 14) level_issue(lm, grid, min(level + (uint32_t)DEPTH, last), x, y, z, v[level % DEPTH]);
+		}
 		feat[level * 2 + 0] = live ? f0 : (half_t)0.f;
 		feat[level * 2 + 1] = live ? f1 : (half_t)0.f;
 		if (GRAD) {
@@ -111,8 +127,8 @@
 #endif
 }
 
-template <bool EMU, int DEPTH>
-__device__ __forceinline__ void point_query_chained_body(const GridMeta& G, const NetW& net, const PointArgs& a, const half_t* __restrict__ wimg, char* smem_raw, LevelMeta* lm) {
+template <bool EMU, int DEPTH, bool CORNERS = false>
+__device__ __forceinline__ void point_query_chained_body(const GridMeta& G, const NetW& net, const PointArgs& a, const half_t* __restrict__ wimg, char* smem_raw, LevelMeta* lm, CornerSlab* cs = nullptr) {
 	poison_lds(smem_raw, LDS_POINT2, threadIdx.x, WG);
 	half_t* wts = reinterpret_cast<half_t*>(smem_raw);
 	fill_level_meta(lm, G, threadIdx.x);
@@ -144,7 +160,7 @@
 		if (valid && a.splat_idx) cell = a.splat_idx[s];
 		half_t feat[28];
 		float dummy[1][3];
-		encode_all_pipelined<false, DEPTH>(lm, n_levels, valid_level, net.grid, x, y, z, feat, dummy);
+		encode_all_pipelined<false, DEPTH, CORNERS>(lm, n_levels, valid_level, net.grid, x, y, z, feat, dummy, CORNERS ? cs + wave : nullptr, lane);
 		write_sdf_in_row(X, lane, x, y, z, feat);
 		wave_lds_sync();
 		h8 bz[4][2];
@@ -183,12 +199,26 @@
 	__shared__ LevelMeta lm[RNB_MAX_LEVELS];
 	point_query_chained_body<true, DEPTH>(G, net, a, wimg, smem_raw, lm);
 }
+template <int DEPTH>
+__global__ __launch_bounds__(WG, 3) void k_point_query_chained_corners(const GridMeta G, const NetW net, const PointArgs a, const half_t* __restrict__ wimg) {
+	extern __shared__ __attribute__((aligned(16))) char smem_raw[];
+	__shared__ LevelMeta lm[RNB_MAX_LEVELS];
+	__shared__ CornerSlab cs[WAVES_PER_WG];
+	point_query_chained_body<false, DEPTH, true>(G, net, a, wimg, smem_raw, lm, cs);
+}
+template <int DEPTH>
+__global__ __launch_bounds__(WG, 2) void k_point_query_chained_emul_corners(const GridMeta G, const NetW net, const PointArgs a, const half_t* __restrict__ wimg) {
+	extern __shared__ __attribute__((aligned(16))) char smem_raw[];
+	__shared__ LevelMeta lm[RNB_MAX_LEVELS];
+	__shared__ CornerSlab cs[WAVES_PER_WG];
+	point_query_chained_body<true, DEPTH, true>(G, net, a, wimg, smem_raw, lm, cs);
+}
 
 constexpr int FWD2_WAVE_HALFS = TILE * S32 + TILE * 8 + TILE;
 constexpr size_t LDS_FWD2 = (size_t)(W_FWD_END + WAVES_PER_WG * FWD2_WAVE_HALFS) * sizeof(half_t);
 
-template <bool EMU, int DEPTH>
-__device__ __forceinline__ void forward_chained_body(const GridMeta& G, const NetW& net, const FwdArgs& a, char* smem_raw, LevelMeta* lm) {
+template <bool EMU, int DEPTH, bool CORNERS = false>
+__device__ __forceinline__ void forward_chained_body(const GridMeta& G, const NetW& net, const FwdArgs& a, char* smem_raw, LevelMeta* lm, CornerSlab* cs = nullptr) {
 	poison_lds(smem_raw, LDS_FWD2, threadIdx.x, WG);
 	half_t* wts = reinterpret_cast<half_t*>(smem_raw);
 	fill_level_meta(lm, G, threadIdx.x);
@@ -218,7 +248,7 @@
 		}
 		half_t feat[28];
 		float dydx[28][3];
-		encode_all_pipelined<true, DEPTH>(lm, n_levels, valid_level, net.grid, c[0], c[1], c[2], feat, dydx);
+		encode_all_pipelined<true, DEPTH, CORNERS>(lm, n_levels, valid_level, net.grid, c[0], c[1], c[2], feat, dydx, CORNERS ? cs + wave : nullptr, lane);
 		write_sdf_in_row(X, lane, c[0], c[1], c[2], feat);
 		wave_lds_sync();
 		h8 bz[4][2];
@@ -346,6 +376,20 @@
 	extern __shared__ __attribute__((aligned(16))) char smem_raw[];
 	__shared__ LevelMeta lm[RNB_MAX_LEVELS];
 	forward_chained_body<true, DEPTH>(G, net, a, smem_raw, lm);
+}
+template <int DEPTH>
+__global__ __launch_bounds__(WG, 2) void k_forward_chained_corners(const GridMeta G, const NetW net, const FwdArgs a) {
+	extern __shared__ __attribute__((aligned(16))) char smem_raw[];
+	__shared__ LevelMeta lm[RNB_MAX_LEVELS];
+	__shared__ CornerSlab cs[WAVES_PER_WG];
+	forward_chained_body<false, DEPTH, true>(G, net, a, smem_raw, lm, cs);
+}
+template <int DEPTH>
+__global__ __launch_bounds__(WG, 2) void k_forward_chained_emul_corners(const GridMeta G, const NetW net, const FwdArgs a) {
+	extern __shared__ __attribute__((aligned(16))) char smem_raw[];
+	__shared__ LevelMeta lm[RNB_MAX_LEVELS];
+	__shared__ CornerSlab cs[WAVES_PER_WG];
+	forward_chained_body<true, DEPTH, true>(G, net, a, smem_raw, lm, cs);
 }
 
 
@@ -686,8 +730,8 @@
 		}
 }
 
-template <bool FULL, bool EMU = false, bool SLICED = false>
-__device__ __forceinline__ void fwd_bwd_sdf_body(const GridMeta& G, const NetW& net, const TrainArgs& a, char* smem_raw, LevelMeta* lm) {
+template <bool FULL, bool EMU = false, bool SLICED = false, bool CORNERS = false>
+__device__ __forceinline__ void fwd_bwd_sdf_body(const GridMeta& G, const NetW& net, const TrainArgs& a, char* smem_raw, LevelMeta* lm, CornerSlab* cs = nullptr) {
 	poison_lds(smem_raw, FULL ? LDS_FBS_FULL : LDS_FBS, threadIdx.x, WG);
 	half_t* wts = reinterpret_cast<half_t*>(smem_raw);
 	constexpr int W_END = FULL ? SWF_END : SW_END;
@@ -752,11 +796,19 @@
 		reinterpret_cast<f4*>(T.srec)[(size_t)s * 2 + 1] = f4{dn[1], dn[2], 0.f, 0.f};
 		uint32_t* Xrow = reinterpret_cast<uint32_t*>(X + lane * S32);
 		uint32_t* Drow = reinterpret_cast<uint32_t*>(D + lane * S32);
+		const int cl = CORNERS ? tile_local(lane) : 0;
 #pragma unroll 1
 		for (uint32_t level = 0; level < 14; ++level) {
 			half_t f0 = (half_t)0.f, f1 = (half_t)0.f;
 			float d0[3] = {0.f, 0.f, 0.f}, d1[3] = {0.f, 0.f, 0.f};
-			if (level < n_live) encode_level_lm<true>(lm, net.grid, level, c[0], c[1], c[2], f0, f1, d0, d1);
+			if constexpr (CORNERS) {
+				if (level < n_live) {
+					uint32_t gr[8], gv[8];
+					level_issue_corners(lm, net.grid, level, c[0], c[1], c[2], cs + wave, cl, gr);
+					level_collect_corners(cs + wave, cl, gr, gv);
+					level_consume<true>(lm, level, c[0], c[1], c[2], gv, f0, f1, d0, d1);
+				}
+			} else if (level < n_live) encode_level_lm<true>(lm, net.grid, level, c[0], c[1], c[2], f0, f1, d0, d1);
 			float r0 = 0.f, r1 = 0.f;
 #pragma unroll
 			for (int d = 0; d < 3; ++d) { r0 += d0[d] * dn[d]; r1 += d1[d] * dn[d]; }
@@ -1072,6 +1124,13 @@
 	extern __shared__ __attribute__((aligned(16))) char smem_raw[];
 	__shared__ LevelMeta lm[RNB_MAX_LEVELS];
 	fwd_bwd_sdf_body<true, true>(G, net, a, smem_raw, lm);
+}
+template <bool FULL, bool EMU, bool SLICED>
+__global__ __launch_bounds__(WG, 2) void k_fwd_bwd_sdf_corners(const GridMeta G, const NetW net, const TrainArgs a) {
+	extern __shared__ __attribute__((aligned(16))) char smem_raw[];
+	__shared__ LevelMeta lm[RNB_MAX_LEVELS];
+	__shared__ CornerSlab cs[WAVES_PER_WG];
+	fwd_bwd_sdf_body<FULL, EMU, SLICED, true>(G, net, a, smem_raw, lm, cs);
 }
 
 constexpr int RW_C0 = 0;
diff --git a/rnb-neus2_amd/csrc/rnb_neus2_hip.hip b/rnb-neus2_amd/csrc/rnb_neus2_hip.hip
--- a/rnb-neus2_amd/csrc/rnb_neus2_hip.hip
+++ b/rnb-neus2_amd/csrc/rnb_neus2_hip.hip
@@ -217,6 +217,7 @@
 		bool dw_sliced = true;
 		bool grid_presort = true;
 	} knobs;
+	uint32_t encode_corners = 5;
 	DevBuf<RayLoss> ray_loss;
 	DevBuf<McTable> mc_table;
 	RenderWorkspace render;
@@ -408,7 +409,10 @@
 	const uint32_t n_tiles = (n + TILE - 1) / TILE;
 	const uint32_t grid = std::min<uint32_t>((n_tiles + WAVES_PER_WG - 1) / WAVES_PER_WG, (uint32_t)c->n_cus * 5);
 	const half_t* wimg = (!inference && c->wimg_valid) ? c->wimg_fwd.p : nullptr;
-	if (c->half_acc()) hipLaunchKernelGGL(k_point_query_chained_emul_pipe<4>, dim3(grid), dim3(WG), LDS_POINT2, s, c->meta(), c->net(inference), a, wimg);
+	if (c->encode_corners & 2u) {
+		if (c->half_acc()) hipLaunchKernelGGL(k_point_query_chained_emul_corners<4>, dim3(grid), dim3(WG), LDS_POINT2, s, c->meta(), c->net(inference), a, wimg);
+		else hipLaunchKernelGGL(k_point_query_chained_corners<4>, dim3(grid), dim3(WG), LDS_POINT2, s, c->meta(), c->net(inference), a, wimg);
+	} else if (c->half_acc()) hipLaunchKernelGGL(k_point_query_chained_emul_pipe<4>, dim3(grid), dim3(WG), LDS_POINT2, s, c->meta(), c->net(inference), a, wimg);
 	else hipLaunchKernelGGL(k_point_query_chained_pipe<4>, dim3(grid), dim3(WG), LDS_POINT2, s, c->meta(), c->net(inference), a, wimg);
 	HIP_TRY(hipGetLastError());
 	return RNB_OK;
@@ -561,7 +565,10 @@
 	a.wimg = (!inference && c->wimg_valid) ? c->wimg_fwd.p : nullptr;
 	const uint32_t n_tiles = (n_max + TILE - 1) / TILE;
 	const uint32_t grid = std::min<uint32_t>((n_tiles + WAVES_PER_WG - 1) / WAVES_PER_WG, (uint32_t)c->n_cus * 2);
-	if (c->half_acc()) hipLaunchKernelGGL(k_forward_chained_emul_pipe<4>, dim3(grid), dim3(WG), LDS_FWD2, s, c->meta(), c->net(inference), a);
+	if (c->encode_corners & 1u) {
+		if (c->half_acc()) hipLaunchKernelGGL(k_forward_chained_emul_corners<4>, dim3(grid), dim3(WG), LDS_FWD2, s, c->meta(), c->net(inference), a);
+		else hipLaunchKernelGGL(k_forward_chained_corners<4>, dim3(grid), dim3(WG), LDS_FWD2, s, c->meta(), c->net(inference), a);
+	} else if (c->half_acc()) hipLaunchKernelGGL(k_forward_chained_emul_pipe<4>, dim3(grid), dim3(WG), LDS_FWD2, s, c->meta(), c->net(inference), a);
 	else hipLaunchKernelGGL(k_forward_chained_pipe<4>, dim3(grid), dim3(WG), LDS_FWD2, s, c->meta(), c->net(inference), a);
 	HIP_TRY(hipGetLastError());
 	return RNB_OK;
@@ -775,6 +782,8 @@
 	const uint32_t fb_grid = sdf_only ? std::min<uint32_t>((B / TILE + WAVES_PER_WG - 1) / WAVES_PER_WG, (uint32_t)c->n_cus * 2) : c->fwd_grid;
 	const bool sliced = half && sdf_only && c->knobs.dw_sliced;
 	const uint32_t n_slices = (B + DW_SLICE - 1) / DW_SLICE;
+	const bool corners = (c->encode_corners & 4u) != 0u;
+#define FBS_CORNERS(FULL, EMU, SLICED) (k_fwd_bwd_sdf_corners<FULL, EMU, SLICED>)
 	const size_t slab = sliced ? (size_t)n_slices : sdf_only ? (size_t)fb_grid : (size_t)c->dw_nwg;
 	float* p_rgb2; float* p_rgb1; float* p_rgb0; float* p_sdf1; float* p_sdf0; float* p_sdf0b; float* p_sdf1b;
 	{
@@ -809,13 +818,20 @@
 		else if (half) hipLaunchKernelGGL(k_rgb_fwd_bwd_h, dim3(fb_grid), dim3(WG), LDS_RGB, s, c->net(false), r);
 		else hipLaunchKernelGGL(k_rgb_fwd_bwd, dim3(fb_grid), dim3(WG), LDS_RGB, s, c->net(false), r);
 		a.dcin = c->dcin.p;
-		if (half && sliced) LAUNCH_EV(k_fwd_bwd_sdf_full_hs, dim3(fb_grid), dim3(WG), LDS_FBS_FULL, s, ev_fb, c->meta(), c->net(false), a);
+		if (corners && half && sliced) LAUNCH_EV(FBS_CORNERS(true, true, true), dim3(fb_grid), dim3(WG), LDS_FBS_FULL, s, ev_fb, c->meta(), c->net(false), a);
+		else if (corners && half) LAUNCH_EV(FBS_CORNERS(true, true, false), dim3(fb_grid), dim3(WG), LDS_FBS_FULL, s, ev_fb, c->meta(), c->net(false), a);
+		else if (corners) LAUNCH_EV(FBS_CORNERS(true, false, false), dim3(fb_grid), dim3(WG), LDS_FBS_FULL, s, ev_fb, c->meta(), c->net(false), a);
+		else if (half && sliced) LAUNCH_EV(k_fwd_bwd_sdf_full_hs, dim3(fb_grid), dim3(WG), LDS_FBS_FULL, s, ev_fb, c->meta(), c->net(false), a);
 		else if (half) LAUNCH_EV(k_fwd_bwd_sdf_full_h, dim3(fb_grid), dim3(WG), LDS_FBS_FULL, s, ev_fb, c->meta(), c->net(false), a);
 		else LAUNCH_EV(k_fwd_bwd_sdf_full, dim3(fb_grid), dim3(WG), LDS_FBS_FULL, s, ev_fb, c->meta(), c->net(false), a);
-	} else if (sdf_only && half && sliced) LAUNCH_EV(k_fwd_bwd_sdf_hs, dim3(fb_grid), dim3(WG), LDS_FBS, s, ev_fb, c->meta(), c->net(false), a);
+	} else if (sdf_only && corners && half && sliced) LAUNCH_EV(FBS_CORNERS(false, true, true), dim3(fb_grid), dim3(WG), LDS_FBS, s, ev_fb, c->meta(), c->net(false), a);
+	else if (sdf_only && corners && half) LAUNCH_EV(FBS_CORNERS(false, true, false), dim3(fb_grid), dim3(WG), LDS_FBS, s, ev_fb, c->meta(), c->net(false), a);
+	else if (sdf_only && corners) LAUNCH_EV(FBS_CORNERS(false, false, false), dim3(fb_grid), dim3(WG), LDS_FBS, s, ev_fb, c->meta(), c->net(false), a);
+	else if (sdf_only && half && sliced) LAUNCH_EV(k_fwd_bwd_sdf_hs, dim3(fb_grid), dim3(WG), LDS_FBS, s, ev_fb, c->meta(), c->net(false), a);
 	else if (sdf_only && half) LAUNCH_EV(k_fwd_bwd_sdf_h, dim3(fb_grid), dim3(WG), LDS_FBS, s, ev_fb, c->meta(), c->net(false), a);
 	else if (sdf_only) LAUNCH_EV(k_fwd_bwd_sdf, dim3(fb_grid), dim3(WG), LDS_FBS, s, ev_fb, c->meta(), c->net(false), a);
 	else LAUNCH_EV(k_fwd_bwd, dim3(fb_grid), dim3(WG), LDS_TRAIN, s, ev_fb, c->meta(), c->net(false), a);
+#undef FBS_CORNERS
 	c->prof.mark(s, P_FWD_BWD);
 	c->prof.units[P_FWD_BWD] += B;
 	const TrainScratch& T = c->ts;
@@ -1313,6 +1329,14 @@
 	HIP_TRY_C(hipFuncSetAttribute(reinterpret_cast<const void*>(k_rgb_fwd_bwd_hs), hipFuncAttributeMaxDynamicSharedMemorySize, (int)LDS_RGB));
 	HIP_TRY_C(hipFuncSetAttribute(reinterpret_cast<const void*>(k_fwd_bwd_sdf_full_h), hipFuncAttributeMaxDynamicSharedMemorySize, (int)LDS_FBS_FULL));
 	HIP_TRY_C(hipFuncSetAttribute(reinterpret_cast<const void*>(k_rgb_fwd_bwd_h), hipFuncAttributeMaxDynamicSharedMemorySize, (int)LDS_RGB));
+	HIP_TRY_C(hipFuncSetAttribute(reinterpret_cast<const void*>(k_forward_chained_corners<4>), hipFuncAttributeMaxDynamicSharedMemorySize, (int)LDS_FWD2));
+	HIP_TRY_C(hipFuncSetAttribute(reinterpret_cast<const void*>(k_forward_chained_emul_corners<4>), hipFuncAttributeMaxDynamicSharedMemorySize, (int)LDS_FWD2));
+	HIP_TRY_C(hipFuncSetAttribute(reinterpret_cast<const void*>(k_fwd_bwd_sdf_corners<false, false, false>), hipFuncAttributeMaxDynamicSharedMemorySize, (int)LDS_FBS));
+	HIP_TRY_C(hipFuncSetAttribute(reinterpret_cast<const void*>(k_fwd_bwd_sdf_corners<false, true, false>), hipFuncAttributeMaxDynamicSharedMemorySize, (int)LDS_FBS));
+	HIP_TRY_C(hipFuncSetAttribute(reinterpret_cast<const void*>(k_fwd_bwd_sdf_corners<false, true, true>), hipFuncAttributeMaxDynamicSharedMemorySize, (int)LDS_FBS));
+	HIP_TRY_C(hipFuncSetAttribute(reinterpret_cast<const void*>(k_fwd_bwd_sdf_corners<true, false, false>), hipFuncAttributeMaxDynamicSharedMemorySize, (int)LDS_FBS_FULL));
+	HIP_TRY_C(hipFuncSetAttribute(reinterpret_cast<const void*>(k_fwd_bwd_sdf_corners<true, true, false>), hipFuncAttributeMaxDynamicSharedMemorySize, (int)LDS_FBS_FULL));
+	HIP_TRY_C(hipFuncSetAttribute(reinterpret_cast<const void*>(k_fwd_bwd_sdf_corners<true, true, true>), hipFuncAttributeMaxDynamicSharedMemorySize, (int)LDS_FBS_FULL));
 	HIP_TRY_C(hipFuncSetAttribute(reinterpret_cast<const void*>(k_grid_scatter_lds_h), hipFuncAttributeMaxDynamicSharedMemorySize, 150 * 1024));
 	{
 		const int march_lds_max = (int)((2 * COARSE_WORDS + 2 * COARSE_MAX_BLOCKS) * sizeof(uint32_t));
@@ -1901,8 +1925,12 @@
 
 int rnb_eval_primitives(rnb_ctx* c, int kind, const uint32_t* in_host, uint32_t n_items, uint32_t* out_host) try {
 	if (!c || (!in_host && n_items) || (!out_host && n_items)) return fail(RNB_ERR_INVALID, "null argument");
-	if (kind < 0 || kind > RNB_PRIM_DW_SLICED) return fail(RNB_ERR_INVALID, "unknown primitive kind");
+	if (kind < 0 || kind > RNB_PRIM_ENCODE_FORM) return fail(RNB_ERR_INVALID, "unknown primitive kind");
 	if (n_items == 0) return RNB_OK;
+	if (kind == RNB_PRIM_ENCODE_FORM) {
+		for (uint32_t i = 0; i < n_items; ++i) { out_host[i] = c->encode_corners; c->encode_corners = in_host[i] & 7u; }
+		return RNB_OK;
+	}
 	if (kind == RNB_PRIM_PREP_DUE) {
 		for (uint32_t i = 0; i < n_items; ++i) { out_host[2 * i] = prep_due(in_host[i]) ? 1u : 0u; out_host[2 * i + 1] = std::min(std::max(in_host[i] / 16u, 1u), 16u); }
 		return RNB_OK;
```

Result: faster. 52.69 million (median of 6 runs) (+1.2%).
